# amathislab/BUCTD

Hardware: AMD Instinct MI355X
Metric: images/sec (train) BUCTD-CoAM-W48 384x288 (higher is better)
Workload: dtype f32 (3x3 convs: operands split exactly into 3 bf16 pieces, 6 bf16 MFMAs per product, fp32 accumulate - fp32-class); 1 GPU; BUCTD-CoAM-W48 (pose_hrnet_coam, ATT_MODULES [F,T,F,F], colored condition) 384x288 CrowdPose-14kpt full train step: fwd + JointsMSE + bwd + grad all-reduce + Adam + arg-max accuracy decode; global_batch=32, batch_per_gpu=32, input=N x 6 x 384 x 288 fp32, params=115581770, parallelism=dp1, hip_streams=4, conv_math=bf16x6, step_graph=False

## Files before the change

### buctd_amd/_C.py

```python
import ctypes as C
import os

import torch

_HERE = os.path.dirname(os.path.abspath(__file__))
LIB_PATH = os.path.join(_HERE, "lib", "libbuctd_hip.so")


class ConvDesc(C.Structure):
    _fields_ = [(n, C.c_int) for n in ("N", "H", "W", "Ci", "Co", "R", "S", "stride", "pad", "Ho", "Wo")]


class BasicBlockDesc(C.Structure):
    _fields_ = ([(n, C.c_int) for n in ("N", "H", "W", "C")] +
                [(n, C.c_void_p) for n in ("x", "w1_fwd", "w2_fwd", "w1_bwd", "w2_bwd", "gamma1", "beta1", "gamma2", "beta2",
                                           "running_mean1", "running_var1", "running_mean2", "running_var2")] +
                [(n, C.c_float) for n in ("eps1", "momentum1", "eps2", "momentum2")] +
                [(n, C.c_void_p) for n in ("z1", "z2", "y", "acc", "stat")])


class BasicBlockGrads(C.Structure):
    _fields_ = ([(n, C.c_void_p) for n in ("dy", "dz2", "dres", "dy1", "dz1", "dx", "dw1", "dw2", "dgamma1", "dbeta1",
                                           "dgamma2", "dbeta2")] +
                [(n, C.c_int) for n in ("acc_w1", "acc_w2", "acc_bn1", "acc_bn2")] +
                [("bn_acc", C.c_void_p), ("wg_ws", C.c_void_p), ("wg_ws_bytes", C.c_size_t)])


class BnAccIn(C.Structure):
    _fields_ = [("acc", C.c_void_p), ("rows", C.c_long), ("eps", C.c_float), ("momentum", C.c_float),
                ("mean_out", C.c_void_p), ("invstd_out", C.c_void_p), ("running_mean", C.c_void_p),
                ("running_var", C.c_void_p)]


class C3Conv(C.Structure):
    _fields_ = ([(n, C.c_int) for n in ("N", "H", "W", "Ci", "Co")] +
                [(n, C.c_void_p) for n in ("x", "wprep", "residual")] + [("relu", C.c_int)] +
                [(n, C.c_void_p) for n in ("y", "stats_acc")] + [("in_bn", C.POINTER(BnAccIn))] +
                [(n, C.c_void_p) for n in ("in_gamma", "in_beta")] + [("in_relu", C.c_int)] +
                [(n, C.c_void_p) for n in ("bn_z", "bn_y", "bn_mean", "bn_invstd", "bn_gamma", "bn_beta", "bn_acc")])


class C3ConvEval(C.Structure):
    _fields_ = ([(n, C.c_int) for n in ("N", "H", "W", "Ci", "Co")] +
                [(n, C.c_void_p) for n in ("x", "wprep", "scale", "shift", "residual")] + [("relu", C.c_int), ("y", C.c_void_p)])


class BnApplyItem(C.Structure):
    _fields_ = [("z", C.c_void_p), ("st", BnAccIn), ("gamma", C.c_void_p), ("beta", C.c_void_p), ("residual", C.c_void_p),
                ("relu", C.c_int), ("y", C.c_void_p), ("rows", C.c_long), ("C", C.c_int)]


class BnBwdItem(C.Structure):
    _fields_ = ([(n, C.c_void_p) for n in ("dy", "y", "z", "mean", "invstd", "gamma", "beta")] +
                [("relu", C.c_int), ("rows", C.c_long), ("C", C.c_int)] +
                [(n, C.c_void_p) for n in ("dz", "dres", "dgamma", "dbeta")] +
                [("accumulate", C.c_int), ("acc", C.c_void_p), ("acc_ready", C.c_int)])


class Wg3Conv(C.Structure):
    _fields_ = ([(n, C.c_int) for n in ("N", "H", "W", "Ci", "Co")] +
                [(n, C.c_void_p) for n in ("x", "dy", "dw")] + [("accumulate", C.c_int)] +
                [(n, C.c_void_p) for n in ("x_mean", "x_invstd", "x_gamma", "x_beta")] + [("x_relu", C.c_int)] +
                [("workspace", C.c_void_p), ("workspace_bytes", C.c_size_t)])


class MhaArgs(C.Structure):
    _fields_ = ([(n, C.c_int) for n in ("B", "T", "h", "dh")] +
                [(n, C.c_void_p) for n in ("q", "k", "v")] + [(n, C.c_int) for n in ("ldq", "ldk", "ldv")] +
                [("out", C.c_void_p), ("ldo", C.c_int), ("lse", C.c_void_p), ("scale", C.c_float), ("p_drop", C.c_float),
                 ("dout", C.c_void_p), ("lddo", C.c_int)] +
                [(n, C.c_void_p) for n in ("dq", "dk", "dv")] + [(n, C.c_int) for n in ("lddq", "lddk", "lddv")])


class MatmulDesc(C.Structure):
    _fields_ = [
        ("batch", C.c_int), ("M", C.c_int), ("N", C.c_int), ("K", C.c_int),
        ("a_layout", C.c_int), ("b_layout", C.c_int),
        ("lda", C.c_int), ("ldb", C.c_int), ("ldc", C.c_int),
        ("stride_a", C.c_long), ("stride_b", C.c_long), ("stride_c", C.c_long),
        ("Kc", C.c_int), ("group_stride_a", C.c_long), ("group_stride_bk", C.c_long),
        ("Nc", C.c_int), ("group_stride_bn", C.c_long), ("group_stride_c", C.c_long),
        ("alpha", C.c_float), ("bias_axis", C.c_int),
    ]


_P = C.c_void_p
_I = C.c_int
_L = C.c_long
_F = C.c_float
_U64 = C.c_uint64
_SZ = C.c_size_t
_PD = C.POINTER(ConvDesc)
_PM = C.POINTER(MatmulDesc)
_PI = C.POINTER(C.c_int)

SIGNATURES = {
    "buctd_version": (_I, []),
    "buctd_last_error": (C.c_char_p, []),
    "buctd_conv2d_fwd": (_I, [_PD, _P, _P, _P, _P, _P, _P, _I, _P, _P, _P]),
    "buctd_conv2d_fwd_thin": (_I, [_PD]),
    "buctd_conv2d_dgrad": (_I, [_PD, _P, _P, _P, _P, _P, _P]),
    "buctd_conv2d_stats_groups": (_I, [_PD, _I, _PI, _PI]),
    "buctd_conv2d_wgrad_workspace": (_SZ, [_PD]),
    "buctd_conv2d_wgrad": (_I, [_PD, _P, _P, _P, _I, _P, _SZ, _P]),
    "buctd_conv2d_plan": (_I, [_PD, _I, _I, _PI]),
    "buctd_matmul_workspace": (_SZ, [_PM]),
    "buctd_matmul": (_I, [_PM, _P, _P, _P, _P, _P, _SZ, _P]),
    "buctd_bn_finalize": (_I, [_P, _P, _I, _I, _L, _I, _F, _F, _P, _P, _P, _P, _P]),
    "buctd_conv3x3_bf16x3_supported": (_I, [_I, _I, _I, _I, _I]),
    "buctd_conv3x3_bf16x3_stats_groups": (_I, [_I, _I, _I, _I, _I, _PI, _PI]),
    "buctd_conv3x3_bf16x3_prep_bytes": (_SZ, [_I, _I, _I]),
    "buctd_conv3x3_bf16x3_prep": (_I, [_I, _I, _P, _I, _P, _P]),
    "buctd_conv3x3_bf16x3_prep_batched": (_I, [_P, _I, _L, _P]),
    "buctd_conv3x3_bf16x3": (_I, [_I, _I, _I, _I, _I, _P, _P, _P, _P, _P, _P, _I, _P, _P, _P, _P]),
    "buctd_conv3x3_wgrad_bf16x3_supported": (_I, [_I, _I, _I, _I, _I]),
    "buctd_conv3x3_wgrad_bf16x3_workspace": (_SZ, [_I, _I, _I, _I, _I]),
    "buctd_conv3x3_wgrad_bf16x3": (_I, [_I, _I, _I, _I, _I, _P, _P, _P, _I, _P, _SZ, _P]),
    "buctd_conv3x3_bf16x6_supported": (_I, [_I, _I, _I, _I, _I]),
    "buctd_conv3x3_bf16x6_stats_groups": (_I, [_I, _I, _I, _I, _I, _PI, _PI]),
    "buctd_conv3x3_bf16x6_prep_bytes": (_SZ, [_I, _I, _I]),
    "buctd_conv3x3_bf16x6_prep": (_I, [_I, _I, _P, _I, _P, _P]),
    "buctd_conv3x3_bf16x6": (_I, [_I, _I, _I, _I, _I, _P, _P, _P, _P, _P, _P, _I, _P, _P, _P, _P]),
    "buctd_conv3x3_bf16x6_bnin": (_I, [_I, _I, _I, _I, _I, _P, _P, _P, _P, _P, _P, _I, _P, _P, _P, _P, _P, _P, _P, _I, _P]),
    "buctd_conv3x3_bf16x6_bnstat": (_I, [_I, _I, _I, _I, _I, _P, _P, _P, _P, _P, _P, _P, _P, _P, _P, _P, _P]),
    "buctd_bn_bwd_from_partials": (_I, [_P, _P, _P, _P, _P, _P, _P, _I, _L, _I, _P, _I, _P, _P, _P, _P, _I, _P, _SZ, _P]),
    "buctd_conv3x3_wgrad_bf16x6_bnin": (_I, [_I, _I, _I, _I, _I, _P, _P, _P, _I, _P, _P, _P, _P, _I, _P, _SZ, _P]),
    "buctd_conv3x3_wgrad_bf16x6_supported": (_I, [_I, _I, _I, _I, _I]),
    "buctd_conv3x3_wgrad_bf16x6_workspace": (_SZ, [_I, _I, _I, _I, _I]),
    "buctd_conv3x3_wgrad_bf16x6": (_I, [_I, _I, _I, _I, _I, _P, _P, _P, _I, _P, _SZ, _P]),
    "buctd_bn_stats": (_I, [_P, _L, _I, _P, _PI, _PI, _P]),
    "buctd_bn_stats_groups": (_I, [_L, _I, _PI, _PI]),
    "buctd_bn_apply": (_I, [_P, _P, _P, _P, _P, _P, _I, _P, _L, _I, _P]),
    "buctd_bn_bwd_workspace": (_SZ, [_L, _I]),
    "buctd_bn_bwd": (_I, [_P, _P, _P, _P, _P, _P, _P, _I, _L, _I, _P, _P, _P, _P, _I, _P, _SZ, _P]),
    "buctd_bn_fold": (_I, [_P, _P, _P, _P, _F, _I, _P, _P, _P]),
    "buctd_bn_acc_bytes": (_SZ, [_I]),
    "buctd_bn_apply_acc": (_I, [_P, C.POINTER(BnAccIn), _P, _P, _P, _I, _P, _L, _I, _P]),
    "buctd_bn_bwd_acc": (_I, [_P, _P, _P, _P, _P, _P, _P, _I, _L, _I, _P, _P, _P, _P, _I, _P, _I, _P]),
    "buctd_conv3x3_bf16x6_acc": (_I, [_I] * 5 + [_P, _P, _P, _I, _P, _P, C.POINTER(BnAccIn), _P, _P, _I, _P]),
    "buctd_conv3x3_bf16x6_bnstat_acc": (_I, [_I] * 5 + [_P] * 12),
    "buctd_gconv_x6_fwd_acc": (_I, [_I] * 6 + [_P] * 6),
    "buctd_conv3x3_bf16x6_group": (_I, [_I, C.POINTER(C3Conv), _P]),
    "buctd_conv3x3_bf16x6_group_eval": (_I, [_I, C.POINTER(C3ConvEval), _P]),
    "buctd_conv3x3_bf16x6_group_workgroups": (_I, [_I, C.POINTER(C3Conv)]),
    "buctd_conv3x3_bf16x6_plan": (_I, [_I, _I, _I, _I, _I, _I, C.POINTER(C.c_int)]),
    "buctd_conv3x3_wgrad_bf16x6_plan": (_I, [_I, _I, _I, _I, _I, C.POINTER(C.c_int)]),
    "buctd_gconv_wgrad_x6_supported": (_I, [_I] * 6),
    "buctd_gconv_wgrad_x6_workspace": (_SZ, [_I] * 6),
    "buctd_gconv_wgrad_x6": (_I, [_I] * 6 + [_P, _P, _P, _I, _P, _SZ, _P]),
    "buctd_bn_apply_acc_group": (_I, [_I, C.POINTER(BnApplyItem), _P]),
    "buctd_bn_bwd_acc_group": (_I, [_I, C.POINTER(BnBwdItem), _P]),
    "buctd_conv3x3_wgrad_bf16x6_group_workspace": (_SZ, [_I] * 6),
    "buctd_conv3x3_wgrad_bf16x6_group": (_I, [_I, C.POINTER(Wg3Conv), _P]),
    "buctd_conv3x3_wgrad_bf16x6_group_workgroups": (_I, [_I, C.POINTER(Wg3Conv)]),
    "buctd_stream_fork": (_I, [_P, _P]),
    "buctd_basic_branches_fwd_train": (_I, [_I, _I, C.POINTER(BasicBlockDesc), _P]),
    "buctd_basic_branches_bwd": (_I, [_I, _I, C.POINTER(BasicBlockDesc), C.POINTER(BasicBlockGrads), _P, _P]),
    "buctd_basic_chain_fwd_train": (_I, [_I, C.POINTER(BasicBlockDesc), _P]),
    "buctd_basic_chain_bwd": (_I, [_I, C.POINTER(BasicBlockDesc), C.POINTER(BasicBlockGrads), _P, _P]),
    "buctd_x6_image_dims": (_I, [_I, _I, _I, _P, _P]),
    "buctd_x6_image_bytes": (C.c_size_t, [_I, _I, _I]),
    "buctd_x6_image": (_I, [_P, _I, _I, _I, _L, _L, _I, _L, _L, _I, _P, _P]),
    "buctd_x6_gemm": (_I, [_I, _I, _I, _P, _P, _P, _I, _F, _P, _L, _I, _L, _P]),
    "buctd_add": (_I, [_P, _P, _P, _L, _I, _P]),
    "buctd_add_n": (_I, [C.POINTER(_P), _I, _P, _L, _P]),
    "buctd_mul": (_I, [_P, _P, _P, _L, _P]),
    "buctd_scale": (_I, [_P, _P, _F, _P, _L, _P]),
    "buctd_copy_channels": (_I, [_P, _L, _I, _I, _P, _I, _I, _I, _P]),
    "buctd_add_bcast": (_I, [_P, _P, _P, _L, _L, _P]),
    "buctd_relu_bwd": (_I, [_P, _P, _P, _L, _P]),
    "buctd_colsum_workspace": (_SZ, [_L, _I]),
    "buctd_colsum": (_I, [_P, _L, _I, _P, _I, _P, _SZ, _P]),
    "buctd_nchw_to_nhwc": (_I, [_P, _I, _I, _I, _I, _I, _I, _P, _P]),
    "buctd_nhwc_to_nchw": (_I, [_P, _I, _I, _I, _I, _P, _P]),
    "buctd_fuse_sum": (_I, [C.POINTER(_P), _PI, _I, _I, _I, _I, _I, _I, _P, _P]),
    "buctd_fuse_sum_bwd": (_I, [_P, _P, _I, _I, _I, _I, _I, _P, _P]),
    "buctd_resize_bilinear": (_I, [_P, _I, _I, _I, _I, _I, _I, _I, _I, _P, _P]),
    "buctd_maxpool3x3s2_fwd": (_I, [_P, _I, _I, _I, _I, _P, _P, _P]),
    "buctd_maxpool3x3s2_bwd": (_I, [_P, _P, _I, _I, _I, _I, _P, _P]),
    "buctd_softmax_dropout_fwd": (_I, [_P, _L, _I, _F, _F, _U64, _P, _P, _P]),
    "buctd_softmax_dropout_bwd": (_I, [_P, _P, _L, _I, _F, _F, _U64, _P, _P]),
    "buctd_softmax_dropout_fwd_dseed": (_I, [_P, _L, _I, _F, _F, _P, _P, _P, _P]),
    "buctd_softmax_dropout_bwd_dseed": (_I, [_P, _P, _L, _I, _F, _F, _P, _P, _P]),
    "buctd_dropout": (_I, [_P, _P, _L, _F, _U64, _P]),
    "buctd_dropout_dseed": (_I, [_P, _P, _L, _F, _P, _P]),
    "buctd_dropout_seed_fill": (_I, [_P, _I, _U64, _U64, _P]),
    "buctd_attn_smallqk_supported": (_I, [_I, _I, _I]),
    "buctd_attn_smallqk_fwd": (_I, [_I, _I, _I, _I, _P, _P, _P, _F, _F, _U64, _I, _P, _P, _P, _P]),
    "buctd_attn_smallqk_bwd": (_I, [_I, _I, _I, _I, _P, _P, _P, _P, _P, _P, _P, _F, _F, _U64, _I, _P, _P, _P, _P, _P]),
    "buctd_attn_smallqk_fwd_dseed": (_I, [_I, _I, _I, _I, _P, _P, _P, _F, _F, _P, _I, _P, _P, _P, _P]),
    "buctd_attn_smallqk_bwd_dseed": (_I, [_I, _I, _I, _I, _P, _P, _P, _P, _P, _P, _P, _F, _F, _P, _I, _P, _P, _P, _P, _P]),
    "buctd_layernorm_fwd": (_I, [_P, _P, _P, _L, _I, _F, _P, _P, _P, _P]),
    "buctd_add_layernorm_fwd": (_I, [_P, _P, _P, _P, _L, _I, _F, _P, _P, _P, _P, _P]),
    "buctd_layernorm_bwd_workspace": (_SZ, [_L, _I]),
    "buctd_layernorm_bwd": (_I, [_P, _P, _P, _P, _P, _L, _I, _P, _P, _P, _I, _P, _SZ, _P]),
    "buctd_joints_mse": (_I, [_P, _P, _P, _I, _I, _I, _P, _P, _F, _P, _SZ, _P]),
    "buctd_joints_ohkm_mse_workspace": (_SZ, [_I, _I]),
    "buctd_joints_ohkm_mse": (_I, [_P, _P, _P, _I, _I, _I, _I, _P, _P, _F, _P, _SZ, _P]),
    "buctd_argmax_decode": (_I, [_P, _I, _I, _I, _P, _P, _P, _P]),
    "buctd_warp_affine_norm": (_I, [_P, _I, _I, _I, _P, _P, _P, _L, _P, _P]),
    "buctd_cond_render_into": (_I, [_P, _I, _P, _I, _I, _I, _I, _I, _I, _P, _L, _P, _SZ, _P]),
    "buctd_cond_geometry": (_I, [_P, _P, _P, _P, _I, _I, _P, _P, _P, _P]),
    "buctd_synthesize_pose": (_I, [_P, _P, _P, _P, _P, _P, _I, _I, _I, C.c_ulonglong, _P, _P]),
    "buctd_mha_fwd_supported": (_I, [_I, _I]),
    "buctd_mha_fwd": (_I, [_I, _I, _I, _P, _P, _P, _I, _I, _F, _P, _P, _P]),
    "buctd_mha_fwd_bf16x6": (_I, [_I, _I, _I, _P, _P, _P, _I, _I, _F, _P, _P, _P]),
    "buctd_gconv_x6_supported": (_I, [_I] * 7),
    "buctd_gconv_x6_prep_bytes": (_SZ, [_I, _I, _I, _I]),
    "buctd_gconv_x6_prep": (_I, [_I, _I, _I, _P, _I, _P, _P]),
    "buctd_gconv_x6_prep_item_bytes": (_SZ, []),
    "buctd_gconv_x6_prep_item": (_I, [_I, _I, _I, _P, _I, _P, _P]),
    "buctd_gconv_x6_prep_batched": (_I, [_P, _I, _P]),
    "buctd_gconv_x6_stats_groups": (_I, [_I] * 6 + [_PI, _PI]),
    "buctd_gconv_x6_fwd": (_I, [_I] * 6 + [_P] * 6 + [_I, _P, _P, _P, _P]),
    "buctd_gconv_x6_dgrad": (_I, [_I] * 6 + [_P] * 4 + [_P]),
    "buctd_mha_fwd_bf16x6_workspace": (_SZ, [_I, _I, _I]),
    "buctd_mha_fwd_bf16x6_ws": (_I, [_I, _I, _I, _P, _P, _P, _I, _I, _F, _P, _P, _P, _SZ, _P]),
    "buctd_mha_train_supported": (_I, [_I, _I]),
    "buctd_mha_fwd_train": (_I, [_I, _I, _I, _P, _P, _P, _I, _I, _F, _F, _U64, _P, _P, _P]),
    "buctd_mha_bwd_workspace": (_SZ, [_I, _I]),
    "buctd_mha_bwd": (_I, [_I, _I, _I, _P, _P, _P, _I, _I, _P, _P, _P, _F, _F, _U64, _P, _P, _I, _P, _I, _P, _SZ, _P]),
    "buctd_mha_fwd_train_dseed": (_I, [_I, _I, _I, _P, _P, _P, _I, _I, _F, _F, _P, _P, _P, _P]),
    "buctd_mha_bwd_dseed": (_I, [_I, _I, _I, _P, _P, _P, _I, _I, _P, _P, _P, _F, _F, _P, _P, _P, _I, _P, _I, _P, _SZ, _P]),
    "buctd_mha_heads_fwd_supported": (_I, [_I, _I, _I]),
    "buctd_mha_heads_fwd": (_I, [C.POINTER(MhaArgs), _P]),
    "buctd_mha_heads_fwd_bf16x6": (_I, [C.POINTER(MhaArgs), _P]),
    "buctd_mha_heads_train_supported": (_I, [_I, _I, _I]),
    "buctd_mha_heads_fwd_train": (_I, [C.POINTER(MhaArgs), _U64, _P]),
    "buctd_mha_heads_bwd_workspace": (_SZ, [_I, _I, _I]),
    "buctd_mha_heads_bwd": (_I, [C.POINTER(MhaArgs), _U64, _P, _SZ, _P]),
    "buctd_mha_heads_fwd_train_dseed": (_I, [C.POINTER(MhaArgs), _P, _P]),
    "buctd_mha_heads_bwd_dseed": (_I, [C.POINTER(MhaArgs), _P, _P, _SZ, _P]),
    "buctd_nms_workspace": (_SZ, [_I]),
    "buctd_nms": (_I, [_P, _P, _P, _I, _I, _F, _P, _SZ, _P]),
    "buctd_cpu_nms": (_I, [_P, _I, _P, _F, _P, _P]),
    "buctd_argmax_decode_refined": (_I, [_P, _I, _I, _I, _P, _P, _P, _P, _P]),
    "buctd_argmax_decode_dark": (_I, [_P, _I, _I, _I, _P, _P, _P, _P, _P]),
    "buctd_gaussian_target": (_I, [_P, _P, _I, _I, _I, _I, _F, _F, _F, _P, _P, _P]),
    "buctd_cond_render_workspace": (_SZ, [_I, _I, _I, _I]),
    "buctd_cond_render": (_I, [_P, _I, _P, _I, _I, _I, _I, _I, _I, _P, _P, _SZ, _P]),
    "buctd_flipback_avg": (_I, [_P, _P, _P, _I, _I, _I, _I, _I, _P, _P]),
    "buctd_sgd_step": (_I, [_P, _P, _P, _L, _F, _F, _F, _I, _I, _F, _P]),
    "buctd_adam_step": (_I, [_P, _P, _P, _P, _L, _F, _F, _F, _F, _I, _F, _P]),
    "buctd_bf16_pack_conv": (_I, [_P, _L, _L, _L, _L, _I, _I, _I, _P, _P, _P, _P, _P, _F, _P, _P, _P]),
    "buctd_bf16_conv": (_I, [_P, _I, _I, _I, _I, _P, _P, _I, _I, _I, _I, _P, _I, _I, _P, _P, _SZ, _P]),
    "buctd_bf16_fuse_sum": (_I, [C.POINTER(_P), _PI, _I, _I, _I, _I, _I, _I, _P, _P]),
    "buctd_bf16_from_f32": (_I, [_P, _L, _P, _P]),
}

_lib = None


class BuctdHipError(RuntimeError):
    pass


def lib():
    global _lib
    if _lib is None:
        if not os.path.isfile(LIB_PATH):
            raise BuctdHipError(
                f"{LIB_PATH} is missing - build it with `make` (or __graft_entry__.build()); "
                "buctd_amd has no CPU / eager fallback")
        handle = C.CDLL(LIB_PATH, mode=C.RTLD_GLOBAL)
        for name, (res, args) in SIGNATURES.items():
            fn = getattr(handle, name)
            fn.restype = res
            fn.argtypes = args
        _lib = handle
    return _lib


def check(rc, what=""):
    if rc != 0:
        msg = lib().buctd_last_error()
        raise BuctdHipError(f"{what} failed ({rc}): {msg.decode() if msg else ''}")


_raw_stream = getattr(torch._C, "_cuda_getCurrentRawStream", None)
_raw_device = getattr(torch._C, "_cuda_getDevice", None)


def current_stream_handle():
    if _raw_stream is not None and _raw_device is not None:
        return _raw_stream(_raw_device())
    return torch.cuda.current_stream().cuda_stream


def stream_ptr():
    return current_stream_handle()


def ptr(t):
    if t is None:
        return None
    if not t.is_cuda:
        raise BuctdHipError("buctd_amd ops need tensors on the ROCm device (no CPU path)")
    return t.data_ptr()
```

### buctd_amd/csrc/block.hip

```cpp
#include "common.h"
#include "../../include/buctd_hip.h"
#include <string.h>

#define BLK_TRY(call)      \
  do {                     \
    const int rc_ = (call); \
    if (rc_) return rc_;   \
  } while (0)

static bool fwd_ptrs_ok(const buctd_basic_block& b) {
  return b.x && b.w1_fwd && b.w2_fwd && b.z1 && b.z2 && b.y && b.acc && b.stat;
}

static bool bwd_ptrs_ok(const buctd_basic_block& b, const buctd_basic_block_grads& g) {
  return b.x && b.w1_bwd && b.w2_bwd && b.z1 && b.z2 && b.y && b.stat && g.dy && g.dres && g.dy1 && g.dw1 && g.dw2 && g.bn_acc &&
         g.wg_ws && g.dz2 && g.dz1;
}

static void acc_in_of(const buctd_basic_block& b, int second, buctd_bn_acc_in* st) {
  const long rows = (long)b.N * b.H * b.W;
  const int C = b.C;
  st->acc = second ? (char*)b.acc + buctd_bn_acc_bytes(C) : b.acc;
  st->rows = rows;
  st->eps = second ? b.eps2 : b.eps1;
  st->momentum = second ? b.momentum2 : b.momentum1;
  st->mean_out = b.stat + (second ? 2 * C : 0);
  st->invstd_out = b.stat + (second ? 3 * C : C);
  st->running_mean = second ? b.running_mean2 : b.running_mean1;
  st->running_var = second ? b.running_var2 : b.running_var1;
}

static buctd_c3_conv c3_of(const buctd_basic_block& b) {
  buctd_c3_conv c;
  memset(&c, 0, sizeof(c));
  c.N = b.N; c.H = b.H; c.W = b.W; c.Ci = c.Co = b.C;
  return c;
}

static int stream_fork(hipStream_t from, hipStream_t to, const char* who) {
  if (from == to) return BUCTD_OK;
  static thread_local hipEvent_t evs[16] = {nullptr};
  int devid = 0;
  if (hipGetDevice(&devid) != hipSuccess || devid < 0 || devid >= 16) {
    buctd_set_error("%s: cannot identify the current device", who);
    return BUCTD_ELAUNCH;
  }
  hipEvent_t& ev = evs[devid];
  if (!ev && hipEventCreateWithFlags(&ev, hipEventDisableTiming) != hipSuccess) {
    buctd_set_error("%s: hipEventCreate failed", who);
    return BUCTD_ELAUNCH;
  }
  if (hipEventRecord(ev, from) != hipSuccess || hipStreamWaitEvent(to, ev, 0) != hipSuccess) {
    buctd_set_error("%s: stream fork failed", who);
    return BUCTD_ELAUNCH;
  }
  return BUCTD_OK;
}

static int block_fwd_train(const buctd_basic_block& b, void* stream) {
  const int N = b.N, H = b.H, W = b.W, C = b.C;
  void* acc1 = b.acc;
  void* acc2 = (char*)b.acc + buctd_bn_acc_bytes(C);
  buctd_bn_acc_in st1, st2;
  acc_in_of(b, 0, &st1);
  acc_in_of(b, 1, &st2);
  BLK_TRY(buctd_conv3x3_bf16x6_acc(N, H, W, C, C, b.x, b.w1_fwd, nullptr, 0, b.z1, acc1, nullptr, nullptr, nullptr, 0, stream));
  BLK_TRY(buctd_conv3x3_bf16x6_acc(N, H, W, C, C, b.z1, b.w2_fwd, nullptr, 0, b.z2, acc2, &st1, b.gamma1, b.beta1, 1, stream));
  BLK_TRY(buctd_bn_apply_acc(b.z2, &st2, b.gamma2, b.beta2, b.x, 1, b.y, st2.rows, C, stream));
  return BUCTD_OK;
}

static int block_bwd_impl(const buctd_basic_block* b, const buctd_basic_block_grads* g, const buctd_basic_block* prev,
                          const buctd_basic_block_grads* gprev, bool bn2_ready, void* stream, void* side_stream) {
  const int N = b->N, H = b->H, W = b->W, C = b->C;
  const long rows = (long)N * H * W;
  const float *mean1 = b->stat, *invstd1 = b->stat + C, *mean2 = b->stat + 2 * C, *invstd2 = b->stat + 3 * C;
  hipStream_t main_s = (hipStream_t)stream, side_s = side_stream ? (hipStream_t)side_stream : main_s;
  void* acc_bn1 = g->bn_acc;
  void* acc_bn2 = (char*)g->bn_acc + buctd_bn_acc_bytes(C);
  BLK_TRY(buctd_bn_bwd_acc(g->dy, b->y, b->z2, mean2, invstd2, b->gamma2, nullptr, 1, rows, C, g->dz2, g->dres, g->dgamma2,
                           g->dbeta2, g->acc_bn2, acc_bn2, bn2_ready ? 1 : 0, stream));
  BLK_TRY(stream_fork(main_s, side_s, "buctd_basic_chain_bwd"));
  BLK_TRY(buctd_conv3x3_wgrad_bf16x6_bnin(N, H, W, C, C, b->z1, g->dz2, g->dw2, g->acc_w2, mean1, invstd1, b->gamma1,
                                          b->beta1, 1, g->wg_ws, g->wg_ws_bytes, side_s));
  BLK_TRY(buctd_conv3x3_bf16x6_bnstat_acc(N, H, W, C, C, g->dz2, b->w2_bwd, nullptr, g->dy1, b->z1, nullptr, mean1, invstd1,
                                          b->gamma1, b->beta1, acc_bn1, stream));
  BLK_TRY(buctd_bn_bwd_acc(g->dy1, nullptr, b->z1, mean1, invstd1, b->gamma1, b->beta1, 1, rows, C, g->dz1, nullptr, g->dgamma1,
                           g->dbeta1, g->acc_bn1, acc_bn1, 1, stream));
  BLK_TRY(stream_fork(main_s, side_s, "buctd_basic_chain_bwd"));
  BLK_TRY(buctd_conv3x3_wgrad_bf16x6(N, H, W, C, C, b->x, g->dz1, g->dw1, g->acc_w1, g->wg_ws, g->wg_ws_bytes, side_s));
  if (g->dx) {
    if (prev)
      BLK_TRY(buctd_conv3x3_bf16x6_bnstat_acc(N, H, W, C, C, g->dz1, b->w1_bwd, g->dres, g->dx, prev->z2, prev->y, prev->stat + 2 * C,
                                              prev->stat + 3 * C, prev->gamma2, nullptr,
                                              (char*)gprev->bn_acc + buctd_bn_acc_bytes(C), stream));
    else
      BLK_TRY(buctd_conv3x3_bf16x6(N, H, W, C, C, g->dz1, b->w1_bwd, nullptr, nullptr, nullptr, g->dres, 0, g->dx, nullptr,
                                   nullptr, stream));
  }
  return BUCTD_OK;
}

static bool bn2_sums_chain(const buctd_basic_block* b, const buctd_basic_block_grads* g) {
  return g->dx && g->dx == g[-1].dy && g[-1].bn_acc && b[-1].y == b->x && b[-1].N == b->N && b[-1].H == b->H && b[-1].W == b->W &&
         b[-1].C == b->C;
}

extern "C" int buctd_basic_chain_fwd_train(int n, const buctd_basic_block* blocks, void* stream) {
  BUCTD_CHECK_ARG(n > 0 && blocks, "buctd_basic_chain_fwd_train: bad argument");
  for (int k = 0; k < n; ++k) BUCTD_CHECK_ARG(fwd_ptrs_ok(blocks[k]), "buctd_basic_chain_fwd_train: null pointer in block %d", k);
  for (int k = 0; k < n; ++k) BLK_TRY(block_fwd_train(blocks[k], stream));
  return BUCTD_OK;
}
extern "C" int buctd_basic_chain_bwd(int n, const buctd_basic_block* blocks, const buctd_basic_block_grads* grads, void* stream,
                                     void* side_stream) {
  BUCTD_CHECK_ARG(n > 0 && blocks && grads, "buctd_basic_chain_bwd: bad argument");
  for (int k = 0; k < n; ++k)
    BUCTD_CHECK_ARG(bwd_ptrs_ok(blocks[k], grads[k]), "buctd_basic_chain_bwd: null pointer in block %d", k);
  bool ready = false;
  for (int k = n - 1; k >= 0; --k) {
    const bool chain = k > 0 && bn2_sums_chain(blocks + k, grads + k);
    BLK_TRY(block_bwd_impl(blocks + k, grads + k, chain ? blocks + k - 1 : nullptr, chain ? grads + k - 1 : nullptr, ready, stream,
                           side_stream));
    ready = chain;
  }
  return BUCTD_OK;
}

#define BR_MAX 4

extern "C" int buctd_basic_branches_fwd_train(int nb, int n, const buctd_basic_block* blocks, void* stream) {
  BUCTD_CHECK_ARG(nb > 0 && nb <= BR_MAX && n > 0 && blocks, "buctd_basic_branches_fwd_train: 1..%d branches", BR_MAX);
  for (int i = 0; i < nb * n; ++i)
    BUCTD_CHECK_ARG(fwd_ptrs_ok(blocks[i]), "buctd_basic_branches_fwd_train: null pointer in block %d", i);
  for (int k = 0; k < n; ++k) {
    buctd_c3_conv cv[BR_MAX];
    buctd_bn_acc_in st1[BR_MAX];
    buctd_bn_apply_item ap[BR_MAX];
    for (int b = 0; b < nb; ++b) {
      const buctd_basic_block& B = blocks[b * n + k];
      buctd_c3_conv& c = cv[b] = c3_of(B);
      c.x = B.x; c.wprep = B.w1_fwd; c.y = B.z1; c.stats_acc = B.acc;
    }
    BLK_TRY(buctd_conv3x3_bf16x6_group(nb, cv, stream));
    for (int b = 0; b < nb; ++b) {
      const buctd_basic_block& B = blocks[b * n + k];
      buctd_c3_conv& c = cv[b];
      acc_in_of(B, 0, &st1[b]);
      c.x = B.z1; c.wprep = B.w2_fwd; c.y = B.z2; c.stats_acc = (char*)B.acc + buctd_bn_acc_bytes(B.C);
      c.in_bn = &st1[b]; c.in_gamma = B.gamma1; c.in_beta = B.beta1; c.in_relu = 1;
    }
    BLK_TRY(buctd_conv3x3_bf16x6_group(nb, cv, stream));
    for (int b = 0; b < nb; ++b) {
      const buctd_basic_block& B = blocks[b * n + k];
      buctd_bn_apply_item& a = ap[b];
      a.z = B.z2;
      acc_in_of(B, 1, &a.st);
      a.gamma = B.gamma2; a.beta = B.beta2; a.residual = B.x; a.relu = 1; a.y = B.y;
      a.rows = a.st.rows; a.C = B.C;
    }
    BLK_TRY(buctd_bn_apply_acc_group(nb, ap, stream));
  }
  return BUCTD_OK;
}

extern "C" int buctd_basic_branches_bwd(int nb, int n, const buctd_basic_block* blocks, const buctd_basic_block_grads* grads,
                                        void* stream, void* side_stream) {
  BUCTD_CHECK_ARG(nb > 0 && nb <= BR_MAX && n > 0 && blocks && grads, "buctd_basic_branches_bwd: 1..%d branches", BR_MAX);
  for (int i = 0; i < nb * n; ++i)
    BUCTD_CHECK_ARG(bwd_ptrs_ok(blocks[i], grads[i]), "buctd_basic_branches_bwd: null pointer in block %d", i);
  hipStream_t main_s = (hipStream_t)stream, side_s = side_stream ? (hipStream_t)side_stream : main_s;
  bool ready[BR_MAX] = {false, false, false, false};
  for (int k = n - 1; k >= 0; --k) {
    buctd_bn_bwd_item bi[BR_MAX];
    buctd_wg3_conv wg[BR_MAX];
    buctd_c3_conv cv[BR_MAX];
    bool chain[BR_MAX];
    for (int b = 0; b < nb; ++b) {
      const buctd_basic_block& B = blocks[b * n + k];
      const buctd_basic_block_grads& G = grads[b * n + k];
      const int C = B.C;
      chain[b] = k > 0 && bn2_sums_chain(&B, &G);
      bi[b] = buctd_bn_bwd_item{G.dy, B.y, B.z2, B.stat + 2 * C, B.stat + 3 * C, B.gamma2, nullptr, 1, (long)B.N * B.H * B.W, C,
                                G.dz2, G.dres, G.dgamma2, G.dbeta2, G.acc_bn2, (char*)G.bn_acc + buctd_bn_acc_bytes(C),
                                ready[b] ? 1 : 0};
    }
    BLK_TRY(buctd_bn_bwd_acc_group(nb, bi, stream));
    BLK_TRY(stream_fork(main_s, side_s, "buctd_basic_branches_bwd"));
    for (int b = 0; b < nb; ++b) {
      const buctd_basic_block& B = blocks[b * n + k];
      const buctd_basic_block_grads& G = grads[b * n + k];
      const int C = B.C;
      wg[b] = buctd_wg3_conv{B.N, B.H, B.W, C, C, B.z1, G.dz2, G.dw2, G.acc_w2, B.stat, B.stat + C, B.gamma1, B.beta1, 1,
                             G.wg_ws, G.wg_ws_bytes};
    }
    BLK_TRY(buctd_conv3x3_wgrad_bf16x6_group(nb, wg, side_s));
    for (int b = 0; b < nb; ++b) {
      const buctd_basic_block& B = blocks[b * n + k];
      const buctd_basic_block_grads& G = grads[b * n + k];
      buctd_c3_conv& c = cv[b] = c3_of(B);
      c.x = G.dz2; c.wprep = B.w2_bwd; c.y = G.dy1;
      c.bn_z = B.z1; c.bn_mean = B.stat; c.bn_invstd = B.stat + B.C; c.bn_gamma = B.gamma1; c.bn_beta = B.beta1; c.bn_acc = G.bn_acc;
    }
    BLK_TRY(buctd_conv3x3_bf16x6_group(nb, cv, stream));
    for (int b = 0; b < nb; ++b) {
      const buctd_basic_block& B = blocks[b * n + k];
      const buctd_basic_block_grads& G = grads[b * n + k];
      const int C = B.C;
      bi[b] = buctd_bn_bwd_item{G.dy1, nullptr, B.z1, B.stat, B.stat + C, B.gamma1, B.beta1, 1, (long)B.N * B.H * B.W, C,
                                G.dz1, nullptr, G.dgamma1, G.dbeta1, G.acc_bn1, G.bn_acc, 1};
    }
    BLK_TRY(buctd_bn_bwd_acc_group(nb, bi, stream));
    BLK_TRY(stream_fork(main_s, side_s, "buctd_basic_branches_bwd"));
    for (int b = 0; b < nb; ++b) {
      const buctd_basic_block& B = blocks[b * n + k];
      const buctd_basic_block_grads& G = grads[b * n + k];
      const int C = B.C;
      wg[b] = buctd_wg3_conv{B.N, B.H, B.W, C, C, B.x, G.dz1, G.dw1, G.acc_w1, nullptr, nullptr, nullptr, nullptr, 0,
                             G.wg_ws, G.wg_ws_bytes};
    }
    BLK_TRY(buctd_conv3x3_wgrad_bf16x6_group(nb, wg, side_s));
    int m = 0;
    for (int b = 0; b < nb; ++b) {
      const buctd_basic_block& B = blocks[b * n + k];
      const buctd_basic_block_grads& G = grads[b * n + k];
      const int C = B.C;
      ready[b] = chain[b];
      if (!G.dx) continue;
      buctd_c3_conv& c = cv[m++] = c3_of(B);
      c.x = G.dz1; c.wprep = B.w1_bwd; c.residual = G.dres; c.y = G.dx;
      if (chain[b]) {
        const buctd_basic_block& Bp = blocks[b * n + k - 1];
        const buctd_basic_block_grads& Gp = grads[b * n + k - 1];
        c.bn_z = Bp.z2; c.bn_y = Bp.y; c.bn_mean = Bp.stat + 2 * C; c.bn_invstd = Bp.stat + 3 * C; c.bn_gamma = Bp.gamma2;
        c.bn_acc = (char*)Gp.bn_acc + buctd_bn_acc_bytes(C);
      }
    }
    if (m) BLK_TRY(buctd_conv3x3_bf16x6_group(m, cv, stream));
  }
  return BUCTD_OK;
}

extern "C" int buctd_stream_fork(void* from, void* to) {
  return stream_fork((hipStream_t)from, (hipStream_t)to, "buctd_stream_fork");
}
```

### buctd_amd/csrc/bn.hip

```cpp
#include "common.h"
#include "../../include/buctd_hip.h"
#include "bn_acc.h"

#define STAT_ROWS 64

__global__ __launch_bounds__(256) void bn_stats_kernel(const float* __restrict__ z, long rows, int C,
                                                       float* __restrict__ part) {
  const long r0 = (long)blockIdx.x * STAT_ROWS;
  long r1 = r0 + STAT_ROWS;
  if (r1 > rows) r1 = rows;
  const int cnt = (int)(r1 - r0);
  for (int c = threadIdx.x; c < C; c += 256) {
    float s = 0.f;
    for (long r = r0; r < r1; ++r) s += z[r * C + c];
    const float mean = cnt > 0 ? s / (float)cnt : 0.f;
    float m2 = 0.f;
    for (long r = r0; r < r1; ++r) {
      const float d = z[r * C + c] - mean;
      m2 += d * d;
    }
    part[((long)blockIdx.x * C + c) * 2 + 0] = mean;
    part[((long)blockIdx.x * C + c) * 2 + 1] = m2;
  }
}
// ... 475 lines not shown
    return BUCTD_EWORKSPACE;
  }
  hipStream_t st = (hipStream_t)stream;
  float* s = (float*)workspace;
  hipLaunchKernelGGL(bn_bwd_finalize_kernel, dim3(C), dim3(256), 0, st, part, nparts, C, s, dgamma, dbeta, accumulate);
  BUCTD_CHECK_LAUNCH("buctd_bn_bwd_from_partials(finalize)");
  const long total = rows * C;
  const float inv_rows = 1.0f / (float)rows;
  if (C % 4 == 0)
    hipLaunchKernelGGL(bn_bwd_apply_kernel<true>, dim3(stream_grid(total / 4)), dim3(256), 0, st, dy, y, z, mean,
                       invstd, gamma, beta, (const float*)s, relu, total, C, inv_rows, dz, dres);
  else
    hipLaunchKernelGGL(bn_bwd_apply_kernel<false>, dim3(stream_grid(total)), dim3(256), 0, st, dy, y, z, mean, invstd,
                       gamma, beta, (const float*)s, relu, total, C, inv_rows, dz, dres);
  BUCTD_CHECK_LAUNCH("buctd_bn_bwd_from_partials(apply)");
  return BUCTD_OK;
}

extern "C" int buctd_bn_fold(const float* gamma, const float* beta, const float* running_mean,
                             const float* running_var, float eps, int C, float* scale, float* shift, void* stream) {
  BUCTD_CHECK_ARG(gamma && beta && running_mean && running_var && scale && shift && C > 0,
                  "buctd_bn_fold: bad argument");
  hipLaunchKernelGGL(bn_fold_kernel, dim3(ceil_div(C, 256)), dim3(256), 0, (hipStream_t)stream, gamma, beta,
                     running_mean, running_var, eps, C, scale, shift);
  BUCTD_CHECK_LAUNCH("buctd_bn_fold");
  return BUCTD_OK;
}


#define BWD2_MAX_BLOCKS 1024

__global__ __launch_bounds__(256) void bn_bwd_reduce2_kernel(const float* __restrict__ dy, const float* __restrict__ y,
                                                             const float* __restrict__ z, const float* __restrict__ mean,
                                                             const float* __restrict__ invstd,
                                                             const float* __restrict__ gamma, const float* __restrict__ beta,
                                                             int relu, long rows, int C, long rows_per_block,
                                                             float* __restrict__ part) {
  __shared__ f32x4 sm[2][256];
  const int c4n = C >> 2;
  const int rl = 256 / c4n;
  const int tc = threadIdx.x % c4n, tr = threadIdx.x / c4n;
  const long r0 = (long)blockIdx.x * rows_per_block;
  long r1 = r0 + rows_per_block;
  if (r1 > rows) r1 = rows;
  f32x4 s1 = (f32x4){0.f, 0.f, 0.f, 0.f}, s2 = s1;
  if (tr < rl) {
    const f32x4 mu = reinterpret_cast<const f32x4*>(mean)[tc];
    const f32x4 is = reinterpret_cast<const f32x4*>(invstd)[tc];
    f32x4 sc = is, be = is;
    const bool rebuild = relu && !y;
    if (rebuild) {
      sc = is * reinterpret_cast<const f32x4*>(gamma)[tc];
      be = reinterpret_cast<const f32x4*>(beta)[tc];
    }
    auto body = [&](f32x4 g, f32x4 zz, f32x4 yy) {
      if (relu) {
        if (rebuild) yy = (zz - mu) * sc + be;
#pragma unroll
        for (int j = 0; j < 4; ++j)
          if (!(yy[j] > 0.f)) g[j] = 0.f;
      }
      s1 += g;
      s2 += g * (zz - mu) * is;
    };
    long r = r0 + tr;
    const long step = rl;
    for (; r + 3 * step < r1; r += 4 * step) {
      f32x4 g[4], zz[4], yy[4];
#pragma unroll
      for (int u = 0; u < 4; ++u) {
        const long o = (r + u * step) * c4n + tc;
        g[u] = reinterpret_cast<const f32x4*>(dy)[o];
        zz[u] = reinterpret_cast<const f32x4*>(z)[o];
        yy[u] = (relu && y) ? reinterpret_cast<const f32x4*>(y)[o] : zz[u];
      }
#pragma unroll
      for (int u = 0; u < 4; ++u) body(g[u], zz[u], yy[u]);
    }
    for (; r < r1; r += step) {
      const long o = r * c4n + tc;
      const f32x4 zz = reinterpret_cast<const f32x4*>(z)[o];
      body(reinterpret_cast<const f32x4*>(dy)[o], zz, (relu && y) ? reinterpret_cast<const f32x4*>(y)[o] : zz);
    }
  }
  sm[0][threadIdx.x] = s1;
  sm[1][threadIdx.x] = s2;
  __syncthreads();
  if (tr == 0) {
    for (int k = 1; k < rl; ++k) {
      s1 += sm[0][k * c4n + tc];
      s2 += sm[1][k * c4n + tc];
    }
    reinterpret_cast<f32x4*>(part + ((long)blockIdx.x * 2 + 0) * C)[tc] = s1;
    reinterpret_cast<f32x4*>(part + ((long)blockIdx.x * 2 + 1) * C)[tc] = s2;
  }
}

static long bwd2_blocks(long rows, long* rows_per_block) {
  long rpb = (rows + BWD2_MAX_BLOCKS - 1) / BWD2_MAX_BLOCKS;
  if (rpb < 64) rpb = 64;
  *rows_per_block = rpb;
  return (rows + rpb - 1) / rpb;
}


static int acc_grid(long n4, int per_cu = 8) {
  long b = (n4 + 256 * 4 - 1) / (256 * 4);
  if (b > 256 * per_cu) b = 256 * per_cu;
  if (b < 1) b = 1;
  return (int)b;
}

struct BnApplyArgs {
  const float* z;
  BnAccFwd a;
  const float* gamma;
  const float* beta;
  const float* res;
  int relu;
  float* y;
  long total;
  int C;
};
__device__ __forceinline__ void bn_apply_acc_body(const BnApplyArgs& p, unsigned bid, unsigned nblk, unsigned char* lds_raw) {
  const float* __restrict__ z = p.z;
  const float* __restrict__ res = p.res;
  float* __restrict__ y = p.y;
  const BnAccFwd& a = p.a;
  const int C = p.C, relu = p.relu;
  long long* wsum = reinterpret_cast<long long*>(lds_raw);
  float* tab = reinterpret_cast<float*>(lds_raw + (size_t)BNACC_WORDS * C * sizeof(long long));
  const long n4 = p.total >> 2;
  const long step = (long)nblk * 256;
  long i = (long)bid * 256 + threadIdx.x;
  f32x4 v0 = (f32x4){0.f, 0.f, 0.f, 0.f}, v1 = v0, r0 = v0, r1 = v0;
  auto fetch = [&](long j) {
    if (j < n4) {
      v0 = reinterpret_cast<const f32x4*>(z)[j];
      if (res) r0 = reinterpret_cast<const f32x4*>(res)[j];
    }
    if (j + step < n4) {
      v1 = reinterpret_cast<const f32x4*>(z)[j + step];
      if (res) r1 = reinterpret_cast<const f32x4*>(res)[j + step];
    }
  };
  fetch(i);
  bnacc_gather_lds(a.acc, C, wsum);
  for (int c = threadIdx.x; c < C; c += 256) {
    double s1, s2;
    bnacc_read_lds(wsum, C, c, &s1, &s2);
    const BnFwdStat st = bnacc_fwd_stat_sums(s1, s2, a.rows, a.eps);
    tab[c] = st.mean;
    tab[C + c] = st.invstd * p.gamma[c];
    tab[2 * C + c] = p.beta[c];
    if (bid == 0) {
      a.mean_out[c] = st.mean;
      a.invstd_out[c] = st.invstd;
      if (a.rmean) bnacc_running(st, a.rows, a.momentum, a.rmean, a.rvar, c);
    }
  }
  __syncthreads();
  const int dc = (int)((step * 4) % C);
  int c = (int)((i * 4) % C) - dc;
  auto one = [&](long j, int cc, f32x4 v, f32x4 r) {
    const f32x4 mu = *reinterpret_cast<const f32x4*>(tab + cc);
    const f32x4 sc = *reinterpret_cast<const f32x4*>(tab + C + cc);
    const f32x4 be = *reinterpret_cast<const f32x4*>(tab + 2 * C + cc);
    f32x4 o;
#pragma unroll
    for (int j4 = 0; j4 < 4; ++j4) o[j4] = (v[j4] - mu[j4]) * sc[j4] + be[j4];
    if (res) o += r;
    if (relu) {
#pragma unroll
      for (int j4 = 0; j4 < 4; ++j4) o[j4] = fmaxf(o[j4], 0.f);
    }
    reinterpret_cast<f32x4*>(y)[j] = o;
  };
  for (; i < n4; i += 2 * step) {
    c += dc;
    if (c >= C) c -= C;
    one(i, c, v0, r0);
    c += dc;
    if (c >= C) c -= C;
    if (i + step < n4) one(i + step, c, v1, r1);
    fetch(i + 2 * step);
  }
}
__global__ __launch_bounds__(256, 8) void bn_apply_acc_kernel(BnApplyArgs p) {
  extern __shared__ __attribute__((aligned(16))) unsigned char lds_raw[];
  bn_apply_acc_body(p, blockIdx.x, gridDim.x, lds_raw);
}

#define BNG_MAX 4
template <class A>
struct BnGroup {
  A s[BNG_MAX];
  int n;
  unsigned first[BNG_MAX + 1];
};
template <class A>
__device__ __forceinline__ int bn_group_find(const BnGroup<A>& g, unsigned* bid, unsigned* nblk) {
  int k = 0;
  while (k + 1 < g.n && blockIdx.x >= g.first[k + 1]) ++k;
  *bid = blockIdx.x - g.first[k];
  *nblk = g.first[k + 1] - g.first[k];
  return k;
}
__global__ __launch_bounds__(256, 8) void bn_apply_acc_group_kernel(BnGroup<BnApplyArgs> g_) {
  extern __shared__ __attribute__((aligned(16))) unsigned char lds_raw[];
  const BnGroup<BnApplyArgs>& g = *(const BnGroup<BnApplyArgs>*)__builtin_amdgcn_kernarg_segment_ptr();
  unsigned bid, nblk;
  const int k = bn_group_find(g, &bid, &nblk);
  bn_apply_acc_body(g.s[k], bid, nblk, lds_raw);
}

#define BN_APPLY_ACC_MAXC 3720
extern "C" size_t buctd_bn_acc_bytes(int C) { return C > 0 ? bnacc_bytes(C) : 0; }

static int acc_in_check(const buctd_bn_acc_in* st, const char* who) {
  BUCTD_CHECK_ARG(st && st->acc && st->rows > 0 && st->mean_out && st->invstd_out &&
                      (st->running_mean == nullptr) == (st->running_var == nullptr),
                  "%s: statistics accumulator, rows, mean_out and invstd_out are required; running_mean/var go together", who);
  return BUCTD_OK;
}
static BnAccFwd acc_in(const buctd_bn_acc_in* st) {
  BnAccFwd a;
  a.acc = (const long long*)st->acc; a.rows = (double)st->rows; a.eps = st->eps; a.momentum = st->momentum;
  a.mean_out = st->mean_out; a.invstd_out = st->invstd_out; a.rmean = st->running_mean; a.rvar = st->running_var;
  return a;
}

extern "C" int buctd_bn_apply_acc(const float* z, const buctd_bn_acc_in* st, const float* gamma, const float* beta,
                                  const float* residual, int relu, float* y, long rows, int C, void* stream) {
  BUCTD_CHECK_ARG(z && gamma && beta && y && rows > 0 && C > 0 && C % 4 == 0 && C <= BN_APPLY_ACC_MAXC,
                  "buctd_bn_apply_acc: bad argument (C must be a multiple of 4, <= %d)", BN_APPLY_ACC_MAXC);
  const int rc = acc_in_check(st, "buctd_bn_apply_acc");
  if (rc) return rc;
  BUCTD_CHECK_ARG(st->rows == rows, "buctd_bn_apply_acc: the statistics cover %ld rows, the tensor has %ld", st->rows, rows);
  const long total = rows * C;
  const BnApplyArgs a{z, acc_in(st), gamma, beta, residual, relu, y, total, C};
  if ((size_t)(BNACC_WORDS * 8 + 3 * 4) * C > 64 * 1024) {
    static unsigned char attr_done[BUCTD_MAX_DEVICES] = {0};
    if (const int rc2 = buctd_raise_lds_limit(reinterpret_cast<const void*>(bn_apply_acc_kernel), 160 * 1024, attr_done, "buctd_bn_apply_acc"))
      return rc2;
  }
  hipLaunchKernelGGL(bn_apply_acc_kernel, dim3(acc_grid(total / 4)), dim3(256), (size_t)(BNACC_WORDS * 8 + 3 * 4) * C,
                     (hipStream_t)stream, a);
  BUCTD_CHECK_LAUNCH("buctd_bn_apply_acc");
  return BUCTD_OK;
}

extern "C" int buctd_bn_apply_acc_group(int n, const buctd_bn_apply_item* items, void* stream) {
  BUCTD_CHECK_ARG(n > 0 && n <= BNG_MAX && items, "buctd_bn_apply_acc_group: 1..%d tensors", BNG_MAX);
  BnGroup<BnApplyArgs> g;
  g.n = n;
  g.first[0] = 0;
  size_t lds = 0;
  for (int k = 0; k < n; ++k) {
    const buctd_bn_apply_item& it = items[k];
    BUCTD_CHECK_ARG(it.z && it.gamma && it.beta && it.y && it.rows > 0 && it.C > 0 && it.C % 4 == 0 && it.C <= BN_APPLY_ACC_MAXC,
                    "buctd_bn_apply_acc_group: bad argument (C must be a multiple of 4, <= %d)", BN_APPLY_ACC_MAXC);
    const int rc = acc_in_check(&it.st, "buctd_bn_apply_acc_group");
    if (rc) return rc;
    BUCTD_CHECK_ARG(it.st.rows == it.rows, "buctd_bn_apply_acc_group: the statistics cover %ld rows, the tensor has %ld",
                    it.st.rows, it.rows);
    const long total = it.rows * it.C;
    g.s[k] = BnApplyArgs{it.z, acc_in(&it.st), it.gamma, it.beta, it.residual, it.relu, it.y, total, it.C};
    g.first[k + 1] = g.first[k] + (unsigned)acc_grid(total / 4);
    const size_t l = (size_t)(BNACC_WORDS * 8 + 3 * 4) * it.C;
    if (l > lds) lds = l;
  }
  for (int k = n; k < BNG_MAX; ++k) g.first[k + 1] = g.first[n];
  if (lds > 64 * 1024) {
    static unsigned char attr_done[BUCTD_MAX_DEVICES] = {0};
    if (const int rc2 = buctd_raise_lds_limit(reinterpret_cast<const void*>(bn_apply_acc_group_kernel), 160 * 1024, attr_done,
                                              "buctd_bn_apply_acc_group"))
      return rc2;
  }
  hipLaunchKernelGGL(bn_apply_acc_group_kernel, dim3(g.first[n]), dim3(256), lds, (hipStream_t)stream, g);
  BUCTD_CHECK_LAUNCH("buctd_bn_apply_acc_group");
  return BUCTD_OK;
}

struct BnBwdArgs {
  const float* dy;
  const float* y;
  const float* z;
  const float* mean;
  const float* invstd;
  const float* gamma;
  const float* beta;
  long long* acc;
  int relu;
  long rows;
  int C;
  long rows_per_block;
  float inv_rows;
  float* dz;
  float* dres;
  float* dgamma;
  float* dbeta;
  int accumulate;
};
__device__ __forceinline__ void bn_bwd_reduce_acc_body(const BnBwdArgs& p, unsigned bid, f32x4 (&sm)[2][256]) {
  const float* __restrict__ dy = p.dy;
  const float* __restrict__ y = p.y;
  const float* __restrict__ z = p.z;
  const float* __restrict__ mean = p.mean;
  const float* __restrict__ invstd = p.invstd;
  const float* __restrict__ gamma = p.gamma;
  const float* __restrict__ beta = p.beta;
  long long* __restrict__ acc = p.acc;
  const int relu = p.relu, C = p.C;
  const long rows = p.rows, rows_per_block = p.rows_per_block;
  const int c4n = C >> 2;
  const int rl = 256 / c4n;
  const int tc = threadIdx.x % c4n, tr = threadIdx.x / c4n;
  const long r0 = (long)bid * rows_per_block;
  long r1 = r0 + rows_per_block;
  if (r1 > rows) r1 = rows;
  f32x4 s1 = (f32x4){0.f, 0.f, 0.f, 0.f}, s2 = s1;
  if (tr < rl) {
    const f32x4 mu = reinterpret_cast<const f32x4*>(mean)[tc];
    const f32x4 is = reinterpret_cast<const f32x4*>(invstd)[tc];
    f32x4 sc = is, be = is;
    const bool rebuild = relu && !y;
    if (rebuild) {
      sc = is * reinterpret_cast<const f32x4*>(gamma)[tc];
      be = reinterpret_cast<const f32x4*>(beta)[tc];
    }
    auto body = [&](f32x4 g, f32x4 zz, f32x4 yy) {
      if (relu) {
        if (rebuild) yy = (zz - mu) * sc + be;
#pragma unroll
        for (int j = 0; j < 4; ++j)
          if (!(yy[j] > 0.f)) g[j] = 0.f;
      }
      s1 += g;
      s2 += g * (zz - mu) * is;
    };
    long r = r0 + tr;
    const long step = rl;
    for (; r + 3 * step < r1; r += 4 * step) {
      f32x4 g[4], zz[4], yy[4];
#pragma unroll
      for (int u = 0; u < 4; ++u) {
        const long o = (r + u * step) * c4n + tc;
        g[u] = reinterpret_cast<const f32x4*>(dy)[o];
        zz[u] = reinterpret_cast<const f32x4*>(z)[o];
        yy[u] = (relu && y) ? reinterpret_cast<const f32x4*>(y)[o] : zz[u];
      }
#pragma unroll
      for (int u = 0; u < 4; ++u) body(g[u], zz[u], yy[u]);
    }
    for (; r < r1; r += step) {
      const long o = r * c4n + tc;
      const f32x4 zz = reinterpret_cast<const f32x4*>(z)[o];
      body(reinterpret_cast<const f32x4*>(dy)[o], zz, (relu && y) ? reinterpret_cast<const f32x4*>(y)[o] : zz);
    }
  }
  sm[0][threadIdx.x] = s1;
  sm[1][threadIdx.x] = s2;
  __syncthreads();
  if (tr == 0) {
    for (int k = 1; k < rl; ++k) {
      s1 += sm[0][k * c4n + tc];
      s2 += sm[1][k * c4n + tc];
    }
    sm[0][tc] = s1;
    sm[1][tc] = s2;
  }
  __syncthreads();
  const unsigned shard = bnacc_shard();
  for (int c = threadIdx.x; c < C; c += 256)
    bnacc_add(acc, C, shard, c, (double)reinterpret_cast<const float*>(&sm[0][0])[c], (double)reinterpret_cast<const float*>(&sm[1][0])[c]);
}
__global__ __launch_bounds__(256) void bn_bwd_reduce_acc_kernel(BnBwdArgs p) {
  __shared__ f32x4 sm[2][256];
  bn_bwd_reduce_acc_body(p, blockIdx.x, sm);
}
__global__ __launch_bounds__(256) void bn_bwd_reduce_acc_group_kernel(BnGroup<BnBwdArgs> g_) {
  __shared__ f32x4 sm[2][256];
  const BnGroup<BnBwdArgs>& g = *(const BnGroup<BnBwdArgs>*)__builtin_amdgcn_kernarg_segment_ptr();
  unsigned bid, nblk;
  const int k = bn_group_find(g, &bid, &nblk);
  bn_bwd_reduce_acc_body(g.s[k], bid, sm);
}

__device__ __forceinline__ void bn_bwd_apply_acc_body(const BnBwdArgs& p, unsigned bid, unsigned nblk, unsigned char* lds_raw) {
  const float* __restrict__ dy = p.dy;
  const float* __restrict__ y = p.y;
  const float* __restrict__ z = p.z;
  const float* __restrict__ mean = p.mean;
  const float* __restrict__ invstd = p.invstd;
  const float* __restrict__ gamma = p.gamma;
  const float* __restrict__ beta = p.beta;
  const long long* __restrict__ acc = p.acc;
  float* __restrict__ dz = p.dz;
  float* __restrict__ dres = p.dres;
  float* __restrict__ dgamma = p.dgamma;
  float* __restrict__ dbeta = p.dbeta;
  const int relu = p.relu, C = p.C, accumulate = p.accumulate;
  const long total = p.rows * C;
  const float inv_rows = p.inv_rows;
  long long* wsum = reinterpret_cast<long long*>(lds_raw);
  float* tab = reinterpret_cast<float*>(lds_raw + (size_t)BNACC_WORDS * C * sizeof(long long));
  const long n4 = total >> 2;
  const long step = (long)nblk * 256;
  const bool ld_y = relu && y;
  long i = (long)bid * 256 + threadIdx.x;
  f32x4 g0 = (f32x4){0.f, 0.f, 0.f, 0.f}, g1 = g0, z0 = g0, z1 = g0, y0 = g0, y1 = g0;
  auto fetch = [&](long j) {
    if (j < n4) {
      g0 = reinterpret_cast<const f32x4*>(dy)[j];
      z0 = reinterpret_cast<const f32x4*>(z)[j];
      if (ld_y) y0 = reinterpret_cast<const f32x4*>(y)[j];
    }
    if (j + step < n4) {
      g1 = reinterpret_cast<const f32x4*>(dy)[j + step];
      z1 = reinterpret_cast<const f32x4*>(z)[j + step];
      if (ld_y) y1 = reinterpret_cast<const f32x4*>(y)[j + step];
    }
  };
  fetch(i);
  bnacc_gather_lds(acc, C, wsum);
  for (int c = threadIdx.x; c < C; c += 256) {
    double s1, s2;
    bnacc_read_lds(wsum, C, c, &s1, &s2);
    tab[c] = mean[c];
    tab[C + c] = invstd[c];
    tab[2 * C + c] = gamma[c];
    tab[3 * C + c] = (relu && !y) ? beta[c] : 0.f;
    tab[4 * C + c] = (float)s1;
    tab[5 * C + c] = (float)s2;
    if (bid == 0) {
      if (dbeta) dbeta[c] = accumulate ? dbeta[c] + (float)s1 : (float)s1;
      if (dgamma) dgamma[c] = accumulate ? dgamma[c] + (float)s2 : (float)s2;
    }
  }
  __syncthreads();
  const int dc = (int)((step * 4) % C);
  int c = (int)((i * 4) % C) - dc;
  auto one = [&](long j, int cc, f32x4 g, f32x4 zz, f32x4 yy) {
    const f32x4 mu = *reinterpret_cast<const f32x4*>(tab + cc);
    const f32x4 is = *reinterpret_cast<const f32x4*>(tab + C + cc);
    const f32x4 ga = *reinterpret_cast<const f32x4*>(tab + 2 * C + cc);
    if (relu) {
      if (!y) {
        const f32x4 be = *reinterpret_cast<const f32x4*>(tab + 3 * C + cc);
#pragma unroll
        for (int j4 = 0; j4 < 4; ++j4) {
          const float sc = is[j4] * ga[j4];
          yy[j4] = (zz[j4] - mu[j4]) * sc + be[j4];
        }
      }
#pragma unroll
      for (int j4 = 0; j4 < 4; ++j4)
        if (!(yy[j4] > 0.f)) g[j4] = 0.f;
    }
    const f32x4 s1 = *reinterpret_cast<const f32x4*>(tab + 4 * C + cc);
    const f32x4 s2 = *reinterpret_cast<const f32x4*>(tab + 5 * C + cc);
    f32x4 o;
#pragma unroll
    for (int j4 = 0; j4 < 4; ++j4) {
      const float zh = (zz[j4] - mu[j4]) * is[j4];
      o[j4] = ga[j4] * is[j4] * (g[j4] - s1[j4] * inv_rows - zh * s2[j4] * inv_rows);
    }
    reinterpret_cast<f32x4*>(dz)[j] = o;
    if (dres) reinterpret_cast<f32x4*>(dres)[j] = g;
  };
  for (; i < n4; i += 2 * step) {
    c += dc;
    if (c >= C) c -= C;
    one(i, c, g0, z0, y0);
    c += dc;
    if (c >= C) c -= C;
    if (i + step < n4) one(i + step, c, g1, z1, y1);
    fetch(i + 2 * step);
  }
}
__global__ __launch_bounds__(256, 6) void bn_bwd_apply_acc_kernel(BnBwdArgs p) {
  extern __shared__ __attribute__((aligned(16))) unsigned char lds_raw[];
  bn_bwd_apply_acc_body(p, blockIdx.x, gridDim.x, lds_raw);
}
__global__ __launch_bounds__(256, 6) void bn_bwd_apply_acc_group_kernel(BnGroup<BnBwdArgs> g_) {
  extern __shared__ __attribute__((aligned(16))) unsigned char lds_raw[];
  const BnGroup<BnBwdArgs>& g = *(const BnGroup<BnBwdArgs>*)__builtin_amdgcn_kernarg_segment_ptr();
  unsigned bid, nblk;
  const int k = bn_group_find(g, &bid, &nblk);
  bn_bwd_apply_acc_body(g.s[k], bid, nblk, lds_raw);
}

static int bn_bwd_acc_fill(const buctd_bn_bwd_item& it, const char* who, BnBwdArgs& a, long* nb) {
  BUCTD_CHECK_ARG(it.dy && it.z && it.mean && it.invstd && it.gamma && it.dz && it.acc && it.rows > 0 && it.C > 0 && it.C % 4 == 0 &&
                      it.C / 4 <= 256,
                  "%s: bad argument (C must be a multiple of 4, <= 1024)", who);
  BUCTD_CHECK_ARG(!it.relu || it.y || it.beta, "%s: relu backward needs the forward output, or beta to rebuild its sign", who);
  a.dy = it.dy; a.y = it.y; a.z = it.z; a.mean = it.mean; a.invstd = it.invstd; a.gamma = it.gamma; a.beta = it.beta;
  a.acc = (long long*)it.acc; a.relu = it.relu; a.rows = it.rows; a.C = it.C;
  *nb = bwd2_blocks(it.rows, &a.rows_per_block);
  a.inv_rows = 1.0f / (float)it.rows;
  a.dz = it.dz; a.dres = it.dres; a.dgamma = it.dgamma; a.dbeta = it.dbeta; a.accumulate = it.accumulate;
  return BUCTD_OK;
}

extern "C" int buctd_bn_bwd_acc(const float* dy, const float* y, const float* z, const float* mean, const float* invstd,
                                const float* gamma, const float* beta, int relu, long rows, int C, float* dz, float* dres,
                                float* dgamma, float* dbeta, int accumulate, void* acc, int acc_ready, void* stream) {
  const buctd_bn_bwd_item it{dy, y, z, mean, invstd, gamma, beta, relu, rows, C, dz, dres, dgamma, dbeta, accumulate, acc, acc_ready};
  BnBwdArgs a;
  long nb;
  const int rc = bn_bwd_acc_fill(it, "buctd_bn_bwd_acc", a, &nb);
  if (rc) return rc;
  hipStream_t st = (hipStream_t)stream;
  if (!acc_ready) {
    hipLaunchKernelGGL(bn_bwd_reduce_acc_kernel, dim3((unsigned)nb), dim3(256), 0, st, a);
    BUCTD_CHECK_LAUNCH("buctd_bn_bwd_acc(reduce)");
  }
  const long total = rows * C;
  hipLaunchKernelGGL(bn_bwd_apply_acc_kernel, dim3(acc_grid(total / 4, 6)), dim3(256), (size_t)(BNACC_WORDS * 8 + 6 * 4) * C, st, a);
  BUCTD_CHECK_LAUNCH("buctd_bn_bwd_acc(apply)");
  return BUCTD_OK;
}

extern "C" int buctd_bn_bwd_acc_group(int n, const buctd_bn_bwd_item* items, void* stream) {
  BUCTD_CHECK_ARG(n > 0 && n <= BNG_MAX && items, "buctd_bn_bwd_acc_group: 1..%d tensors", BNG_MAX);
  BnGroup<BnBwdArgs> ga, gr;
  ga.n = n; gr.n = 0;
  ga.first[0] = gr.first[0] = 0;
  size_t lds = 0;
  for (int k = 0; k < n; ++k) {
    long nb;
    const int rc = bn_bwd_acc_fill(items[k], "buctd_bn_bwd_acc_group", ga.s[k], &nb);
    if (rc) return rc;
    const long total = items[k].rows * items[k].C;
    ga.first[k + 1] = ga.first[k] + (unsigned)acc_grid(total / 4, 6);
    const size_t l = (size_t)(BNACC_WORDS * 8 + 6 * 4) * items[k].C;
    if (l > lds) lds = l;
    if (!items[k].acc_ready) {
      gr.s[gr.n] = ga.s[k];
      gr.first[gr.n + 1] = gr.first[gr.n] + (unsigned)nb;
      ++gr.n;
    }
  }
  for (int k = n; k < BNG_MAX; ++k) ga.first[k + 1] = ga.first[n];
  for (int k = gr.n; k < BNG_MAX; ++k) gr.first[k + 1] = gr.first[gr.n];
  hipStream_t st = (hipStream_t)stream;
  if (gr.n) {
    hipLaunchKernelGGL(bn_bwd_reduce_acc_group_kernel, dim3(gr.first[gr.n]), dim3(256), 0, st, gr);
    BUCTD_CHECK_LAUNCH("buctd_bn_bwd_acc_group(reduce)");
  }
  hipLaunchKernelGGL(bn_bwd_apply_acc_group_kernel, dim3(ga.first[n]), dim3(256), lds, st, ga);
  BUCTD_CHECK_LAUNCH("buctd_bn_bwd_acc_group(apply)");
  return BUCTD_OK;
}
```

### buctd_amd/models/hrnet_common.py

```python
import logging
import os

import torch

from .. import nn
from .. import ops

BN_MOMENTUM = 0.1
logger = logging.getLogger(__name__)


def conv3x3(in_planes, out_planes, stride=1):
    return nn.Conv2d(in_planes, out_planes, kernel_size=3, stride=stride, padding=1, bias=False)


class BasicBlock(nn.Module):
    expansion = 1

    def __init__(self, inplanes, planes, stride=1, downsample=None):
        super().__init__()
        self.conv1 = conv3x3(inplanes, planes, stride)
        self.bn1 = nn.BatchNorm2d(planes, momentum=BN_MOMENTUM)
        self.relu = nn.ReLU(inplace=True)
        self.conv2 = conv3x3(planes, planes)
        self.bn2 = nn.BatchNorm2d(planes, momentum=BN_MOMENTUM)
        self.downsample = downsample
        self.stride = stride

    def forward(self, x):
        if self.training and x.is_cuda and torch.is_grad_enabled() and _native_block(self):
            return ops.BasicBlockFn.apply(x, *_block_params(self))
        residual = x if self.downsample is None else self.downsample(x)
        out = nn.conv_bn_act(x, self.conv1, self.bn1, relu=True)
        return nn.conv_bn_act(out, self.conv2, self.bn2, relu=True, residual=residual)


def _native_block(m):
    return (type(m) is BasicBlock and m.downsample is None and m.stride == 1 and m.conv1.bias is None and m.conv2.bias is None
            and m.bn1.training and m.bn2.training and m.bn1.track_running_stats == m.bn2.track_running_stats)


def _block_params(m):
    nn._as_channels_last_(m.conv1.weight)
    nn._as_channels_last_(m.conv2.weight)
    return m.conv1.weight, m.bn1, m.conv2.weight, m.bn2


class Bottleneck(nn.Module):
    expansion = 4

    def __init__(self, inplanes, planes, stride=1, downsample=None):
        super().__init__()
        self.conv1 = nn.Conv2d(inplanes, planes, kernel_size=1, bias=False)
        self.bn1 = nn.BatchNorm2d(planes, momentum=BN_MOMENTUM)
        self.conv2 = nn.Conv2d(planes, planes, kernel_size=3, stride=stride, padding=1, bias=False)
        self.bn2 = nn.BatchNorm2d(planes, momentum=BN_MOMENTUM)
        self.conv3 = nn.Conv2d(planes, planes * self.expansion, kernel_size=1, bias=False)
        self.bn3 = nn.BatchNorm2d(planes * self.expansion, momentum=BN_MOMENTUM)
        self.relu = nn.ReLU(inplace=True)
        self.downsample = downsample
        self.stride = stride

    def forward(self, x):
        bns = (self.bn1, self.bn2, self.bn3) + (() if self.downsample is None or len(self.downsample) < 2 else (self.downsample[1],))
        if (self.training and x.is_cuda and torch.is_grad_enabled() and ops.fused_bottleneck_on()
                and all(b.training for b in bns)
                and (self.downsample is None or type(self.downsample) is nn.ConvBN and not self.downsample._relu)):
            for c in (self.conv1, self.conv2, self.conv3) + (() if self.downsample is None else (self.downsample[0],)):
                nn._as_channels_last_(c.weight)
            return ops.BottleneckFn.apply(x, self.conv1.weight, self)
        residual = x if self.downsample is None else self.downsample(x)
        out = nn.conv_bn_act(x, self.conv1, self.bn1, relu=True)
        out = nn.conv_bn_act(out, self.conv2, self.bn2, relu=True)
        return nn.conv_bn_act(out, self.conv3, self.bn3, relu=True, residual=residual)


class BlockChain(nn.Chain):

    def forward(self, x):
        if (len(self) > 1 and self.training and x.is_cuda and torch.is_grad_enabled() and ops.native_chain_ok(tuple(x.shape))
                and all(_native_block(m) and m.bn1.track_running_stats == self[0].bn1.track_running_stats for m in self)
                and ops.bn_in_fusable(tuple(x.shape), self[0].conv1.weight)):
            return ops.BasicChainFn.apply(x, self[0].conv1.weight, [_block_params(m) for m in self])
        return super().forward(x)


blocks_dict = {"BASIC": BasicBlock, "BOTTLENECK": Bottleneck}


def make_residual_layer(block, inplanes, planes, blocks, stride=1):
    downsample = None
    if stride != 1 or inplanes != planes * block.expansion:
        downsample = nn.ConvBN(
            nn.Conv2d(inplanes, planes * block.expansion, kernel_size=1, stride=stride, bias=False),
            nn.BatchNorm2d(planes * block.expansion, momentum=BN_MOMENTUM))
    layers = [block(inplanes, planes, stride, downsample)]
    inplanes = planes * block.expansion
    for _ in range(1, blocks):
        layers.append(block(inplanes, planes))
    return BlockChain(*layers), inplanes


class HighResolutionModule(nn.Module):
    def __init__(self, num_branches, blocks, num_blocks, num_inchannels, num_channels, fuse_method,
                 multi_scale_output=True):
        super().__init__()
        self._check_branches(num_branches, blocks, num_blocks, num_inchannels, num_channels)
        self.num_inchannels = num_inchannels
        self.fuse_method = fuse_method
        self.num_branches = num_branches
        self.multi_scale_output = multi_scale_output
        self.branches = self._make_branches(num_branches, blocks, num_blocks, num_channels)
        self.fuse_layers = self._make_fuse_layers()
        self.relu = nn.ReLU(True)

    def _check_branches(self, num_branches, blocks, num_blocks, num_inchannels, num_channels):
        for what, lst in (("NUM_BLOCKS", num_blocks), ("NUM_CHANNELS", num_channels),
                          ("NUM_INCHANNELS", num_inchannels)):
            if num_branches != len(lst):
                msg = "NUM_BRANCHES({}) <> {}({})".format(num_branches, what, len(lst))
                logger.error(msg)
                raise ValueError(msg)

    def _make_branches(self, num_branches, block, num_blocks, num_channels):
        branches = []
        for i in range(num_branches):
            chain, cout = make_residual_layer(block, self.num_inchannels[i], num_channels[i], num_blocks[i])
            self.num_inchannels[i] = cout
            branches.append(chain)
        return nn.ModuleList(branches)

    def _make_fuse_layers(self):
        if self.num_branches == 1:
            return None
        ch = self.num_inchannels
        rows = []
        for i in range(self.num_branches if self.multi_scale_output else 1):
            row = []
            for j in range(self.num_branches):
                if j > i:
                    row.append(nn.ConvBN(nn.Conv2d(ch[j], ch[i], 1, 1, 0, bias=False), nn.BatchNorm2d(ch[i]),
                                         nn.Upsample(scale_factor=2 ** (j - i), mode="nearest")))
                elif j == i:
                    row.append(None)
                else:
                    steps = []
                    for k in range(i - j):
                        last = k == i - j - 1
                        cout = ch[i] if last else ch[j]
                        steps.append(nn.ConvBN(nn.Conv2d(ch[j], cout, 3, 2, 1, bias=False), nn.BatchNorm2d(cout),
                                               None if last else nn.ReLU(True)))
                    row.append(nn.Chain(*steps))
            rows.append(nn.ModuleList(row))
        return nn.ModuleList(rows)

    def get_num_inchannels(self):
        return self.num_inchannels

    def _branches_grouped(self, x):
        nb = self.num_branches
        if not (self.training and torch.is_grad_enabled() and all(type(br) is BlockChain and len(br) > 1 for br in self.branches)):
            return None
        chains = []
        for br in self.branches:
            if not all(_native_block(m) and m.bn1.track_running_stats == br[0].bn1.track_running_stats for m in br):
                return None
            chains.append([_block_params(m) for m in br])
        xs = [x[i] for i in range(nb)]
        if not ops.group_branches_ok(xs, chains):
            return None
        parts = ops.group_branch_partition(nb)
        if len(parts) == 1:
            return list(ops.BasicBranchesFn.apply(chains[0][0][0], chains, *xs))
        outs = ops.fork_join([lambda p=p: ops.BasicBranchesFn.apply(chains[p[0]][0][0], [chains[i] for i in p], *[xs[i] for i in p])
                              for p in parts], [[xs[i] for i in p] for p in parts])
        ys = [None] * nb
        for p, o in zip(parts, outs):
            for i, y in zip(p, o):
                ys[i] = y
        return ys

    def _branches_grouped_eval(self, x):
        if self.training or torch.is_grad_enabled() or not all(type(br) is BlockChain and len(br) > 0 for br in self.branches):
            return None
        chains = []
        for br in self.branches:
            if not all(type(m) is BasicBlock and m.downsample is None and m.stride == 1 and m.conv1.bias is None
                       and m.conv2.bias is None and not m.bn1.training and not m.bn2.training
                       and m.bn1.running_mean is not None and m.bn2.running_mean is not None for m in br):
                return None
            chains.append([_block_params(m) for m in br])
        xs = [x[i] for i in range(self.num_branches)]
        if not ops.eval_branches_ok(xs, chains):
            return None
        return ops.basic_branches_eval(xs, chains)

    def forward(self, x):
        if self.num_branches == 1:
            return [self.branches[0](x[0])]
        xs = self._branches_grouped(x)
        if xs is None:
            xs = self._branches_grouped_eval(x)
        if xs is None:
            xs = ops.fork_join([lambda i=i: self.branches[i](x[i]) for i in range(self.num_branches)],
                               [x[i] for i in range(self.num_branches)])
        rows = list(enumerate(self.fuse_layers))
        fan = len(rows) > 1 and torch.is_grad_enabled() and any(t.requires_grad for t in xs)
        xr = [ops.FanOut.apply(xs[j], len(rows)) if fan and xs[j].is_cuda else [xs[j]] * len(rows)
              for j in range(self.num_branches)]

        def fuse_row(i, row):
            terms, shifts = [], []
            for j in range(self.num_branches):
                if j == i:
                    terms.append(xr[j][i])
                    shifts.append(0)
                elif j > i:
                    terms.append(row[j](xr[j][i]))
                    shifts.append(j - i)
                else:
                    terms.append(row[j](xr[j][i]))
                    shifts.append(0)
            return ops.FuseSum.apply(tuple(shifts), True, *terms)

        return ops.fork_join([lambda i=i, row=row: fuse_row(i, row) for i, row in rows], [xs for _ in rows], tag=1)


def make_transition_layer(pre, cur):
    layers = []
    for i in range(len(cur)):
        if i < len(pre):
            if cur[i] != pre[i]:
                layers.append(nn.ConvBN(nn.Conv2d(pre[i], cur[i], 3, 1, 1, bias=False), nn.BatchNorm2d(cur[i]),
                                        nn.ReLU(inplace=True)))
            else:
                layers.append(None)
        else:
            steps = []
            for j in range(i + 1 - len(pre)):
                cin = pre[-1]
                cout = cur[i] if j == i - len(pre) else cin
                steps.append(nn.ConvBN(nn.Conv2d(cin, cout, 3, 2, 1, bias=False), nn.BatchNorm2d(cout),
                                       nn.ReLU(inplace=True)))
            layers.append(nn.Chain(*steps))
    return nn.ModuleList(layers)


def make_stage(layer_config, num_inchannels, multi_scale_output=True):
    block = blocks_dict[layer_config["BLOCK"]]
    modules = []
    for i in range(layer_config["NUM_MODULES"]):
        mso = multi_scale_output or i != layer_config["NUM_MODULES"] - 1
        modules.append(HighResolutionModule(layer_config["NUM_BRANCHES"], block, layer_config["NUM_BLOCKS"],
                                            num_inchannels, layer_config["NUM_CHANNELS"],
                                            layer_config["FUSE_METHOD"], mso))
        num_inchannels = modules[-1].get_num_inchannels()
    return nn.Chain(*modules), num_inchannels


class HRNetTrunk(nn.Module):

    def build_trunk(self, extra, last_stage=4):
        self.conv1 = nn.Conv2d(3, 64, kernel_size=3, stride=2, padding=1, bias=False)
        self.bn1 = nn.BatchNorm2d(64, momentum=BN_MOMENTUM)
        self.conv2 = nn.Conv2d(64, 64, kernel_size=3, stride=2, padding=1, bias=False)
        self.bn2 = nn.BatchNorm2d(64, momentum=BN_MOMENTUM)
        self.relu = nn.ReLU(inplace=True)
        self.layer1, c = make_residual_layer(Bottleneck, 64, 64, 4)
        pre = [c]
        for s in range(2, last_stage + 1):
            scfg = extra["STAGE%d" % s]
            setattr(self, "stage%d_cfg" % s, scfg)
            block = blocks_dict[scfg["BLOCK"]]
            ch = [c * block.expansion for c in scfg["NUM_CHANNELS"]]
            setattr(self, "transition%d" % (s - 1), make_transition_layer(pre, ch))
            stage, pre = make_stage(scfg, ch, multi_scale_output=(s != last_stage))
            setattr(self, "stage%d" % s, stage)
        return pre

    def stem(self, x_nhwc):
        x = nn.conv_bn_act(x_nhwc, self.conv1, self.bn1, relu=True)
        x = nn.conv_bn_act(x, self.conv2, self.bn2, relu=True)
        return self.layer1(x)

    def enter_stage(self, s, prev, first=False):
        trans = getattr(self, "transition%d" % (s - 1))
        n = getattr(self, "stage%d_cfg" % s)["NUM_BRANCHES"]
        if first:
            heads = [trans[i] if isinstance(trans[i], nn.ConvBN) else trans[i][0] if isinstance(trans[i], nn.Chain) else None
                     for i in range(n)]
            if (self.training and prev.is_cuda and torch.is_grad_enabled() and ops.fused_bottleneck_on() and n > 1
                    and all(type(h) is nn.ConvBN and h[1].training for h in heads)):
                for h in heads:
                    nn._as_channels_last_(h[0].weight)
                ys = ops.ForkConvBnFn.apply(prev, heads[0][0].weight, [(h[0], h[1], h._relu) for h in heads])
                out = []
                for i in range(n):
                    y = ys[i]
                    if isinstance(trans[i], nn.Chain):
                        for m in list(trans[i])[1:]:
                            y = m(y)
                    out.append(y)
                return out
            return [trans[i](prev) if trans[i] is not None else prev for i in range(n)]
        return [trans[i](prev[-1]) if trans[i] is not None else prev[i] for i in range(n)]


def to_device_input(x):
    if not x.is_cuda:
        x = x.cuda()
    if x.dtype != torch.float32:
        x = x.float()
    return x.contiguous()


def init_weights_hrnet(model, pretrained="", linear=False):
    logger.info("=> init weights from normal distribution")
    for m in model.modules():
        if isinstance(m, (torch.nn.Conv2d, torch.nn.ConvTranspose2d)) or (linear and isinstance(m, torch.nn.Linear)):
            torch.nn.init.normal_(m.weight, std=0.001)
            if m.bias is not None:
                torch.nn.init.constant_(m.bias, 0)
        elif isinstance(m, torch.nn.BatchNorm2d):
            torch.nn.init.constant_(m.weight, 1)
            torch.nn.init.constant_(m.bias, 0)
    if os.path.isfile(pretrained):
        state = torch.load(pretrained, map_location="cpu")
        logger.info("=> loading pretrained model {}".format(pretrained))
        keep = {k: v for k, v in state.items()
                if k.split(".")[0] in model.pretrained_layers or model.pretrained_layers[0] == "*"}
        model.load_state_dict(keep, strict=False)
    elif pretrained:
        logger.error("=> please download pre-trained models first!")
        raise ValueError("{} is not exist!".format(pretrained))
```

### buctd_amd/ops.py

```python
import ctypes as C
import math

import torch

from . import _C
from ._C import ConvDesc, MatmulDesc, check, lib, ptr, stream_ptr

_capture = {"on": False, "events": set(), "allow_seeds": False, "seed_table": None, "seed_draws": 0}
_SEED_TABLE_SLOTS = 1024


def capturing():
    return _capture["on"]


def _new_event(stream=None):
    ev = torch.cuda.Event()
    ev.record(stream) if stream is not None else ev.record()
    if _capture["on"]:
        _capture["events"].add(id(ev))
        _capture.setdefault("keep", []).append(ev)
    return ev


# ... 721 lines not shown
                      "conv3x3_wgrad_bf16x6_bnin")
                return out
            check(fn(d.N, d.H, d.W, d.Ci, d.Co, ptr(x), ptr(dy), ptr(out), int(accumulate), ptr(ws), ws.numel(),
                     stream_ptr_()), "conv3x3_wgrad (split bf16)")
            return out
    if x_bn is not None:
        raise _C.BuctdHipError("conv_wgrad: x_bn needs the bf16x6 3x3 kernel (check bn_in_fusable first)")
    kind = _gconv_kind(d) if mode == "bf16x6" else 0
    if kind:
        need = _memo(("gwg", kind, d.N, d.H, d.W, d.Ci, d.Co),
                     lambda: (int(lib().buctd_gconv_wgrad_x6_workspace(kind, d.N, d.H, d.W, d.Ci, d.Co))
                              if lib().buctd_gconv_wgrad_x6_supported(kind, d.N, d.H, d.W, d.Ci, d.Co) == 1 else -1))
        if need >= 0:
            ws = workspace_(need, x.device)
            check(lib().buctd_gconv_wgrad_x6(kind, d.N, d.H, d.W, d.Ci, d.Co, ptr(x), ptr(dy), ptr(out), int(accumulate), ptr(ws),
                                             ws.numel(), stream_ptr_()), "gconv_wgrad_x6")
            return out
    need = lib().buctd_conv2d_wgrad_workspace(C.byref(d))
    ws = workspace_(need, x.device)
    check(lib().buctd_conv2d_wgrad(C.byref(d), ptr(x), ptr(dy), ptr(out), int(accumulate), ptr(ws), ws.numel(),
                                   stream_ptr_()), "conv2d_wgrad")
    return out


_side = {"on": True, "streams": {}, "joined": True}


_SIDE_PRIO = -1


def _side_stream(device):
    idx = device.index if device.index is not None else torch.cuda.current_device()
    st = _side["streams"].get(idx)
    if st is None:
        st = torch.cuda.Stream(device=device, priority=_SIDE_PRIO)
        _side["streams"][idx] = st
    return st


def copy_stream(device):
    if not (_side["on"] and device.type == "cuda"):
        return None
    return _side_stream(device)


def side_streams(device):
    return [st for idx, st in _side["streams"].items() if idx == device.index]


def wait_side_stream(stream=None):
    for idx, st in _side["streams"].items():
        target = stream if stream is not None else torch.cuda.current_stream(torch.device("cuda", idx))
        target.wait_stream(st)
    for (idx, _), st in _branch["streams"].items():
        target = stream if stream is not None else torch.cuda.current_stream(torch.device("cuda", idx))
        if target != st:
            target.wait_stream(st)


_branch = {"on": True, "streams": {}}


_BRANCH_MAX = 2
_BRANCH_PRIO = 0


def set_stream_forks(branch, wgrad=None):
    old = (_branch["on"], _side["on"])
    _branch["on"] = bool(branch)
    _side["on"] = bool(branch if wgrad is None else wgrad)
    return old


def set_branch_max(n):
    global _BRANCH_MAX
    old, _BRANCH_MAX = _BRANCH_MAX, max(0, int(n))
    return old


def compute_streams(device):
    idx = device.index if device.index is not None else torch.cuda.current_device()
    return ([st for (d, i), st in _branch["streams"].items() if d == idx and i <= _BRANCH_MAX] +
            [st for d, st in _side["streams"].items() if d == idx])


def reserve_compute_streams(device):
    out = []
    if _branch["on"]:
        out += [_branch_stream(device, i) for i in range(1, _BRANCH_MAX + 1)]
    if _side["on"]:
        out.append(_side_stream(device))
    return out


def _branch_stream(device, i):
    i = min(i, _BRANCH_MAX)
    key = (device.index, i)
    st = _branch["streams"].get(key)
    if st is None:
        st = torch.cuda.Stream(device=device, priority=_BRANCH_PRIO)
        _branch["streams"][key] = st
    return st


def lane_stream(device, k):
    return _branch_stream(device, k + 1)


def _record(t, stream):
    if torch.is_tensor(t):
        if t.is_cuda:
            t.record_stream(stream)
    elif isinstance(t, (list, tuple)):
        for u in t:
            _record(u, stream)


def fork_join(fns, inputs, tag=0):
    dev = None
    for t in inputs:
        for u in (t if isinstance(t, (list, tuple)) else [t]):
            if torch.is_tensor(u) and u.is_cuda:
                dev = u.device
    if not _branch["on"] or dev is None or len(fns) < 2:
        return [f() for f in fns]
    main = torch.cuda.current_stream(dev)
    start = torch.cuda.Event()
    start.record(main)
    outs = [None] * len(fns)
    done = []
    outs[0] = fns[0]()
    for i in range(1, len(fns)):
        st = _branch_stream(dev, i)
        if st == main:
            outs[i] = fns[i]()
            continue
        st.wait_event(start)
        _record(inputs[i], st)
        with torch.cuda.stream(st):
            outs[i] = fns[i]()
            ev = torch.cuda.Event()
            ev.record(st)
        _record(outs[i], main)
        done.append(ev)
    for ev in done:
        main.wait_event(ev)
    return outs


def _join_side():
    _side["joined"] = True
    wait_side_stream()


def _queue_join():
    task = torch._C._current_graph_task_id() if hasattr(torch._C, "_current_graph_task_id") else None
    if task is not None and task >= 0:
        if _side.get("task") == task:
            return
        _side["task"] = task
    elif not _side["joined"]:
        return
    _side["joined"] = False
    try:
        torch.autograd.Variable._execution_engine.queue_callback(_join_side)
    except RuntimeError:
        _join_side()


def conv_wgrad_async(x, dy, w_like, stride, pad, out, accumulate, x_bn=None):
    if not (_side["on"] and x.is_cuda):
        if x.is_cuda and _branch["on"]:
            _queue_join()
        return conv_wgrad(x, dy, w_like, stride, pad, out=out, accumulate=accumulate, x_bn=x_bn)
    side = _side_stream(x.device)
    check(lib().buctd_stream_fork(stream_ptr(), side.cuda_stream), "stream_fork")
    conv_wgrad(x, dy, w_like, stride, pad, out=out, accumulate=accumulate, x_bn=x_bn, stream=side)
    x.record_stream(side)
    dy.record_stream(side)
    if x_bn is not None:
        x_bn[0].record_stream(side)
        x_bn[1].record_stream(side)
    _queue_join()
    return out


def matmul(A, B, Cout, *, batch, M, N, K, a_layout, b_layout, lda, ldb, ldc, stride_a=0, stride_b=0, stride_c=0,
           Kc=None, gsa=0, gsbk=0, Nc=None, gsbn=0, gsc=0, alpha=1.0, bias=None, bias_axis=0,
           a_off=0, b_off=0, c_off=0):
    d = MatmulDesc(batch, M, N, K, a_layout, b_layout, lda, ldb, ldc, stride_a, stride_b, stride_c,
                   K if Kc is None else Kc, gsa, gsbk, N if Nc is None else Nc, gsbn, gsc, alpha, bias_axis)
    need = lib().buctd_matmul_workspace(C.byref(d))
    ws = workspace(need, A.device) if need else None
    pa = C.c_void_p(A.data_ptr() + 4 * a_off)
    pb = C.c_void_p(B.data_ptr() + 4 * b_off)
    pc = C.c_void_p(Cout.data_ptr() + 4 * c_off)
    check(lib().buctd_matmul(C.byref(d), pa, pb, ptr(bias), pc, ptr(ws), ws.numel() if ws is not None else 0,
                             stream_ptr()), "matmul")
    return Cout


def x6_image(src, V, K, role, *, vs, ks, vg=0, vgs=0, kg=0, kgs=0, off=0, out=None):
    need = lib().buctd_x6_image_bytes(V, K, role)
    if out is None or out.numel() < need:
        out = torch.empty(need, dtype=torch.uint8, device=src.device)
    check(lib().buctd_x6_image(C.c_void_p(src.data_ptr() + 4 * off), V, K, vg, vgs, vs, kg, kgs, ks, role, ptr(out),
                               stream_ptr()), "x6_image")
    return out


def x6_gemm(a_image, b_image, Cout, M, N, K, *, ldc, Nc=0, gsc=0, bias=None, bias_axis=0, alpha=1.0, c_off=0):
    check(lib().buctd_x6_gemm(M, N, K, ptr(a_image), ptr(b_image), ptr(bias), bias_axis, alpha,
                              C.c_void_p(Cout.data_ptr() + 4 * c_off), ldc, Nc, gsc, stream_ptr()), "x6_gemm")
    return Cout


def _x6_weight_image(w, V, K, transposed):
    key = (w.data_ptr(), w._version, _weights_epoch["n"])
    cache = getattr(w, "_buctd_x6img", None)
    if cache is None or cache["key"] != key:
        cache = {"key": key}
        try:
            w._buctd_x6img = cache
        except (AttributeError, RuntimeError, TypeError):
            pass
    tag = "t" if transposed else "n"
    if tag not in cache:
        ld = w.shape[1]
        cache[tag] = x6_image(w, V, K, 0, vs=1, ks=ld) if transposed else x6_image(w, V, K, 0, vs=ld, ks=1)
        cache[tag + "_ev"] = _new_event()
        cache[tag + "_stream"] = torch.cuda.current_stream(w.device).cuda_stream
    elif torch.cuda.current_stream(w.device).cuda_stream != cache[tag + "_stream"]:
        _wait_event(torch.cuda.current_stream(w.device), cache[tag + "_ev"])
    return cache[tag]


def fc_o_x6_ok(T, rows):
    return _conv_math["mode"] == "bf16x6" and T >= 512 and rows >= 192


def bn_finalize(part, info, rows, Cn, eps, momentum, running_mean, running_var):
    mean = torch.empty(Cn, dtype=torch.float32, device=part.device)
    invstd = torch.empty(Cn, dtype=torch.float32, device=part.device)
    counts = info[2] if len(info) > 2 else None
    check(lib().buctd_bn_finalize(ptr(part), ptr(counts), info[0], info[1], rows, Cn, eps, momentum, ptr(mean), ptr(invstd),
                                  ptr(running_mean), ptr(running_var), stream_ptr()), "bn_finalize")
    return mean, invstd


class BnAccInput:

    def __init__(self, acc, rows, bn, training=True, relu=True):
        Cn = acc.Cn
        dev = bn.weight.device
        self.acc, self.rows, self.gamma, self.beta, self.relu = acc, int(rows), bn.weight, bn.bias, relu
        self.eps = bn.eps
        self.momentum = 0.1 if bn.momentum is None else bn.momentum
        stat = torch.empty((2, Cn), dtype=torch.float32, device=dev)
        self.mean, self.invstd = stat[0], stat[1]
        track = bn.track_running_stats and training
        self.rm = bn.running_mean if track else None
        self.rv = bn.running_var if track else None

    def struct(self):
        st = _C.BnAccIn()
        st.acc, st.rows, st.eps, st.momentum = self.acc.ptr, self.rows, self.eps, self.momentum
        st.mean_out, st.invstd_out = self.mean.data_ptr(), self.invstd.data_ptr()
        st.running_mean = self.rm.data_ptr() if self.rm is not None else None
        st.running_var = self.rv.data_ptr() if self.rv is not None else None
        return st


def bn_apply_acc(z, bnin, residual=None, relu=False):
    Cn = z.shape[-1]
    y = torch.empty_like(z)
    st = bnin.struct()
    check(lib().buctd_bn_apply_acc(ptr(z), C.byref(st), ptr(bnin.gamma), ptr(bnin.beta), ptr(residual), int(bool(relu)), ptr(y),
                                   z.numel() // Cn, Cn, stream_ptr()), "bn_apply_acc")
    return y


def bn_acc_ok(Cn):
    return Cn % 4 == 0 and Cn <= 1024


def bn_stats(z):
    Cn = z.shape[-1]
    rows = z.numel() // Cn
    ng, rpg = C.c_int(), C.c_int()
    check(lib().buctd_bn_stats_groups(rows, Cn, C.byref(ng), C.byref(rpg)), "bn_stats_groups")
    part = torch.empty((ng.value, Cn, 2), dtype=torch.float32, device=z.device)
    check(lib().buctd_bn_stats(ptr(z), rows, Cn, ptr(part), None, None, stream_ptr()), "bn_stats")
    return part, (ng.value, rpg.value)


def bn_apply(z, mean, invstd, gamma, beta, residual=None, relu=False):
    Cn = z.shape[-1]
    y = torch.empty_like(z)
    check(lib().buctd_bn_apply(ptr(z), ptr(mean), ptr(invstd), ptr(gamma), ptr(beta), ptr(residual), int(bool(relu)),
                               ptr(y), z.numel() // Cn, Cn, stream_ptr()), "bn_apply")
    return y


def bn_bwd(dy, y, z, mean, invstd, gamma, relu, want_dres, dgamma, dbeta, accumulate, beta=None):
    Cn = z.shape[-1]
    rows = z.numel() // Cn
    dz = torch.empty_like(z)
    dres = torch.empty_like(z) if want_dres else None
    if relu and y is None and beta is None:
        raise _C.BuctdHipError("bn_bwd: ReLU backward needs the forward output or beta")
    if bn_acc_ok(Cn):
        acc = AccRef(Cn, z.device)
        check(lib().buctd_bn_bwd_acc(ptr(dy), ptr(y) if relu else None, ptr(z), ptr(mean), ptr(invstd), ptr(gamma),
                                     ptr(beta) if (relu and y is None) else None, int(bool(relu)), rows, Cn, ptr(dz), ptr(dres),
                                     ptr(dgamma), ptr(dbeta), int(accumulate), C.c_void_p(acc.ptr), 0,
                                     stream_ptr()), "bn_bwd_acc")
        return dz, dres
    need = lib().buctd_bn_bwd_workspace(rows, Cn)
    ws = workspace(need, z.device)
    check(lib().buctd_bn_bwd(ptr(dy), ptr(y) if relu else None, ptr(z), ptr(mean), ptr(invstd), ptr(gamma),
                             ptr(beta) if (relu and y is None) else None, int(bool(relu)), rows, Cn, ptr(dz), ptr(dres), ptr(dgamma), ptr(dbeta), int(accumulate),
                             ptr(ws), ws.numel(), stream_ptr()), "bn_bwd")
    return dz, dres


def bn_fold_cached(bn, gamma, beta, eps):
    rm, rv = bn.running_mean, bn.running_var
    nbt = bn.num_batches_tracked
    key = (gamma.data_ptr(), gamma._version, beta._version, rm.data_ptr(), rm._version, rv._version, _weights_epoch["n"],
           float(eps), getattr(bn, "_pending_batches", 0), nbt._version if nbt is not None else 0)
    cache = getattr(bn, "_buctd_fold", None)
    cur = torch.cuda.current_stream(gamma.device)
    if cache is None or cache[0] != key:
        scale, shift = bn_fold(gamma, beta, rm, rv, eps)
        ev = _new_event()
        cache = (key, scale, shift, ev, cur.cuda_stream, set())
        try:
            object.__setattr__(bn, "_buctd_fold", cache)
        except (AttributeError, TypeError):
            return scale, shift
    elif cur.cuda_stream != cache[4] and cur.cuda_stream not in cache[5]:
        _wait_event(cur, cache[3])
        cache[5].add(cur.cuda_stream)
    return cache[1], cache[2]


def bn_fold(gamma, beta, rm, rv, eps):
    Cn = gamma.numel()
    scale = torch.empty(Cn, dtype=torch.float32, device=gamma.device)
    shift = torch.empty(Cn, dtype=torch.float32, device=gamma.device)
    check(lib().buctd_bn_fold(ptr(gamma), ptr(beta), ptr(rm), ptr(rv), eps, Cn, ptr(scale), ptr(shift), stream_ptr()),
          "bn_fold")
    return scale, shift


def add(a, b=None, relu=False, out=None):
    if out is None:
        out = torch.empty_like(a)
    check(lib().buctd_add(ptr(a), ptr(b), ptr(out), a.numel(), int(bool(relu)), stream_ptr()), "add")
    return out


def mul(a, b, out=None):
    if out is None:
        out = torch.empty_like(a)
    check(lib().buctd_mul(ptr(a), ptr(b), ptr(out), a.numel(), stream_ptr()), "mul")
    return out


class Mul(torch.autograd.Function):

    @staticmethod
    def forward(ctx, a, b):
        a, b = _contig(a), _contig(b)
        ctx.save_for_backward(a, b)
        return mul(a, b)

    @staticmethod
    def backward(ctx, dy):
        a, b = ctx.saved_tensors
        dy = _contig(dy)
        return mul(dy, b), mul(dy, a)


def scale(x, dev_scalar=None, alpha=1.0, out=None):
    if out is None:
        out = torch.empty_like(x)
    check(lib().buctd_scale(ptr(x), ptr(dev_scalar), alpha, ptr(out), x.numel(), stream_ptr()), "scale")
    return out


def relu_bwd(dy, y):
    dx = torch.empty_like(dy)
    check(lib().buctd_relu_bwd(ptr(dy), ptr(y), ptr(dx), dy.numel(), stream_ptr()), "relu_bwd")
    return dx


def colsum(x2d_like, Cn, out, accumulate):
    rows = x2d_like.numel() // Cn
    need = lib().buctd_colsum_workspace(rows, Cn)
    ws = workspace(need, x2d_like.device)
    check(lib().buctd_colsum(ptr(x2d_like), rows, Cn, ptr(out), int(accumulate), ptr(ws), ws.numel(), stream_ptr()),
          "colsum")
    return out


def nchw_to_nhwc(x, c0=0, cc=None):
    _f32(x, "nchw input")
    N, Ct, H, W = x.shape
    cc = Ct - c0 if cc is None else cc
    y = torch.empty((N, H, W, cc), dtype=torch.float32, device=x.device)
    check(lib().buctd_nchw_to_nhwc(ptr(x), N, Ct, c0, cc, H, W, ptr(y), stream_ptr()), "nchw_to_nhwc")
    return y


def nhwc_to_nchw(x):
    _f32(x, "nhwc input")
    N, H, W, Cn = x.shape
    y = torch.empty((N, Cn, H, W), dtype=torch.float32, device=x.device)
    check(lib().buctd_nhwc_to_nchw(ptr(x), N, Cn, H, W, ptr(y), stream_ptr()), "nhwc_to_nchw")
    return y


def fuse_sum(terms, shifts, relu=True):
    base = terms[shifts.index(0)]
    N, H, W, Cn = base.shape
    out = torch.empty_like(base)
    n = len(terms)
    arr = (C.c_void_p * n)(*[t.data_ptr() for t in terms])
    sh = (C.c_int * n)(*shifts)
    check(lib().buctd_fuse_sum(arr, sh, n, N, H, W, Cn, int(bool(relu)), ptr(out), stream_ptr()), "fuse_sum")
    return out


def fuse_sum_bwd(dy, y, shift):
    N, H, W, Cn = dy.shape
    g = torch.empty((N, H >> shift, W >> shift, Cn), dtype=torch.float32, device=dy.device)
    check(lib().buctd_fuse_sum_bwd(ptr(dy), ptr(y), shift, N, H, W, Cn, ptr(g), stream_ptr()), "fuse_sum_bwd")
    return g


def resize_bilinear_from_nchw(x, c0, cc, Ho, Wo):
    _f32(x, "resize input")
    N, Ct, H, W = x.shape
    y = torch.empty((N, Ho, Wo, cc), dtype=torch.float32, device=x.device)
    check(lib().buctd_resize_bilinear(ptr(x), N, Ct, c0, cc, H, W, Ho, Wo, ptr(y), stream_ptr()), "resize_bilinear")
    return y


def softmax_dropout_fwd(s, L, scale, p_drop, seed, inplace=True):
    rows = s.numel() // L
    p = s if inplace else torch.empty_like(s)
    pd = torch.empty_like(s) if p_drop > 0 else p
    fn, seed = _seeded("buctd_softmax_dropout_fwd", seed)
    check(fn(ptr(s), rows, L, scale, p_drop, seed, ptr(p), ptr(pd), stream_ptr()), "softmax_dropout_fwd")
    return p, pd


def softmax_dropout_bwd(dpd, p, L, scale, p_drop, seed, inplace=True):
    rows = p.numel() // L
    ds = dpd if inplace else torch.empty_like(dpd)
    fn, seed = _seeded("buctd_softmax_dropout_bwd", seed)
    check(fn(ptr(dpd), ptr(p), rows, L, scale, p_drop, seed, ptr(ds), stream_ptr()), "softmax_dropout_bwd")
    return ds


def joints_mse(pred, gt, w, want_grad, gscale=1.0):
    N, K = pred.shape[0], pred.shape[1]
    HW = pred.numel() // (N * K)
    loss = torch.empty((), dtype=torch.float32, device=pred.device)
    grad = torch.empty_like(pred) if want_grad else None
    ws = workspace(N * K * 4, pred.device)
    check(lib().buctd_joints_mse(ptr(pred), ptr(gt), ptr(w), N, K, HW, ptr(loss), ptr(grad), gscale, ptr(ws),
                                 ws.numel(), stream_ptr()), "joints_mse")
    return loss, grad


def joints_ohkm_mse(pred, gt, w, topk, want_grad, gscale=1.0):
    N, K = pred.shape[0], pred.shape[1]
    HW = pred.numel() // (N * K)
    loss = torch.empty((), dtype=torch.float32, device=pred.device)
    grad = torch.empty_like(pred) if want_grad else None
    ws = workspace(lib().buctd_joints_ohkm_mse_workspace(N, K), pred.device)
    check(lib().buctd_joints_ohkm_mse(ptr(pred), ptr(gt), ptr(w), N, K, HW, int(topk), ptr(loss), ptr(grad), gscale,
                                      ptr(ws), ws.numel(), stream_ptr()), "joints_ohkm_mse")
    return loss, grad


def argmax_decode(hm, refine=False, preds_out=None):
    N, K, H, W = hm.shape
    preds = preds_out if preds_out is not None else torch.empty((N, K, 2), dtype=torch.float32, device=hm.device)
    if preds_out is not None and not (preds_out.is_pinned() and preds_out.is_contiguous() and tuple(preds_out.shape) == (N, K, 2)
                                      and preds_out.dtype == torch.float32):
        raise _C.BuctdHipError("argmax_decode: preds_out must be a pinned contiguous fp32 [N, K, 2] host tensor")
    maxvals = torch.empty((N, K, 1), dtype=torch.float32, device=hm.device)
    idx = torch.empty((N, K), dtype=torch.int32, device=hm.device)
    if refine:
        quarter = torch.empty((N, K, 2), dtype=torch.float32, device=hm.device)
        check(lib().buctd_argmax_decode_refined(ptr(hm), N * K, H, W, preds.data_ptr(), ptr(maxvals), ptr(idx), ptr(quarter),
                                                stream_ptr()), "argmax_decode_refined")
        return preds, maxvals, idx, quarter
    check(lib().buctd_argmax_decode(ptr(hm), N * K, H, W, preds.data_ptr(), ptr(maxvals), ptr(idx), stream_ptr()),
          "argmax_decode")
    return preds, maxvals, idx


DARK_MAX_PIXELS = 8000


def dark_decode(hm):
    if hm.dim() != 4 or hm.dtype != torch.float32:
        raise _C.BuctdHipError("dark_decode: heat-maps must be a fp32 [N, K, H, W] tensor")
    hm = hm.contiguous()
    N, K, H, W = hm.shape
    preds = torch.empty((N, K, 2), dtype=torch.float32, device=hm.device)
    maxvals = torch.empty((N, K, 1), dtype=torch.float32, device=hm.device)
    idx = torch.empty((N, K), dtype=torch.int32, device=hm.device)
    offset = torch.empty((N, K, 2), dtype=torch.float32, device=hm.device)
    check(lib().buctd_argmax_decode_dark(ptr(hm), N * K, H, W, ptr(preds), ptr(maxvals), ptr(idx), ptr(offset),
                                         stream_ptr()), "argmax_decode_dark")
    return preds, maxvals, idx, offset


def scalar_to_host(src, dst):
    if not (dst.is_pinned() and dst.dtype == torch.float32 and dst.numel() == 1 and src.numel() == 1):
        raise _C.BuctdHipError("scalar_to_host: one fp32 value into a pinned host tensor")
    check(lib().buctd_copy_channels(ptr(src), 1, 1, 0, dst.data_ptr(), 1, 0, 1, stream_ptr()), "scalar_to_host")
    return dst


def gaussian_target(joints, vis, heatmap_size, image_size, sigma):
    B, K = joints.shape[0], joints.shape[1]
    Wh, Hh = int(heatmap_size[0]), int(heatmap_size[1])
    target = torch.empty((B, K, Hh, Wh), dtype=torch.float32, device=joints.device)
    weight = torch.empty((B, K, 1), dtype=torch.float32, device=joints.device)
    check(lib().buctd_gaussian_target(ptr(joints), ptr(vis), B, K, Hh, Wh, image_size[0] / heatmap_size[0],
                                      image_size[1] / heatmap_size[1], float(sigma), ptr(target), ptr(weight),
                                      stream_ptr()), "gaussian_target")
    return target, weight


def cond_render(joints, colors, H, W, truncate=False):
    B, K, js = joints.shape
    Cc = 1 if colors is None else colors.shape[1]
    cond = torch.empty((B, Cc, H, W), dtype=torch.float32, device=joints.device)
    need = lib().buctd_cond_render_workspace(B, Cc, H, W)
    ws = workspace(need, joints.device)
    check(lib().buctd_cond_render(ptr(joints), js, ptr(colors), B, K, Cc, H, W, int(bool(truncate)), ptr(cond),
                                  ptr(ws), ws.numel(), stream_ptr()), "cond_render")
    return cond


def flipback_avg(a, b, perm, shift):
    N, K, H, W = a.shape
    out = torch.empty_like(a)
    check(lib().buctd_flipback_avg(ptr(a), ptr(b), ptr(perm), N, K, H, W, int(bool(shift)), ptr(out), stream_ptr()),
          "flipback_avg")
    return out


def adam_step(p, g, m, v, lr, beta1, beta2, eps, step, gscale=1.0):
    check(lib().buctd_adam_step(ptr(p), ptr(g), ptr(m), ptr(v), p.numel(), lr, beta1, beta2, eps, step, gscale,
                                stream_ptr()), "adam_step")


def sgd_step(p, g, buf, lr, momentum, weight_decay, nesterov, first, gscale=1.0):
    check(lib().buctd_sgd_step(ptr(p), ptr(g), ptr(buf), p.numel(), lr, momentum, weight_decay, int(bool(nesterov)),
                               int(bool(first)), gscale, stream_ptr()), "sgd_step")


def layernorm_fwd(x, gamma, beta, eps):
    Cn = x.shape[-1]
    rows = x.numel() // Cn
    y = torch.empty_like(x)
    mean = torch.empty(rows, dtype=torch.float32, device=x.device)
    invstd = torch.empty(rows, dtype=torch.float32, device=x.device)
    check(lib().buctd_layernorm_fwd(ptr(x), ptr(gamma), ptr(beta), rows, Cn, eps, ptr(y), ptr(mean), ptr(invstd),
                                    stream_ptr()), "layernorm_fwd")
    return y, mean, invstd


def add_layernorm_fwd(a, b, gamma, beta, eps, keep_sum=True):
    Cn = a.shape[-1]
    rows = a.numel() // Cn
    y = torch.empty_like(a)
    s = torch.empty_like(a) if keep_sum else None
    mean = torch.empty(rows, dtype=torch.float32, device=a.device)
    invstd = torch.empty(rows, dtype=torch.float32, device=a.device)
    check(lib().buctd_add_layernorm_fwd(ptr(a), ptr(b), ptr(gamma), ptr(beta), rows, Cn, eps, ptr(s), ptr(y), ptr(mean),
                                        ptr(invstd), stream_ptr()), "add_layernorm_fwd")
    return y, mean, invstd, s


def layernorm_bwd(dy, x, mean, invstd, gamma, dgamma, dbeta, accumulate):
    Cn = x.shape[-1]
    rows = x.numel() // Cn
    dx = torch.empty_like(x)
    need = lib().buctd_layernorm_bwd_workspace(rows, Cn)
    ws = workspace(need, x.device)
    check(lib().buctd_layernorm_bwd(ptr(dy), ptr(x), ptr(mean), ptr(invstd), ptr(gamma), rows, Cn, ptr(dx),
                                    ptr(dgamma), ptr(dbeta), int(accumulate), ptr(ws), ws.numel(), stream_ptr()),
          "layernorm_bwd")
    return dx


def dropout(x, p_drop, seed):
    y = torch.empty_like(x)
    fn, seed = _seeded("buctd_dropout", seed)
    check(fn(ptr(x), ptr(y), x.numel(), p_drop, seed, stream_ptr()), "dropout")
    return y


def maxpool3x3s2_fwd(x):
    N, H, W, Cn = x.shape
    Ho, Wo = (H + 2 - 3) // 2 + 1, (W + 2 - 3) // 2 + 1
    y = torch.empty((N, Ho, Wo, Cn), dtype=torch.float32, device=x.device)
    idx = torch.empty((N, Ho, Wo, Cn), dtype=torch.int32, device=x.device)
    check(lib().buctd_maxpool3x3s2_fwd(ptr(x), N, H, W, Cn, ptr(y), ptr(idx), stream_ptr()), "maxpool_fwd")
    return y, idx


def maxpool3x3s2_bwd(dy, idx, x_shape):
    N, H, W, Cn = x_shape
    dx = torch.empty(tuple(x_shape), dtype=torch.float32, device=dy.device)
    check(lib().buctd_maxpool3x3s2_bwd(ptr(dy), ptr(idx), N, H, W, Cn, ptr(dx), stream_ptr()), "maxpool_bwd")
    return dx


def _contig(g):
    return g if g.is_contiguous() else g.contiguous()


def _count_batch(bn):
    bn.count_batch() if hasattr(bn, "count_batch") else bn.num_batches_tracked.add_(1)


class ConvBnAct(torch.autograd.Function):

    @staticmethod
    def forward(ctx, x, conv_w, conv_b, bn, residual, relu, stride, pad, training, transposed_shape):
        gamma, beta = bn.weight, bn.bias
        eps = bn.eps
        ctx.meta = (bn, conv_w, conv_b, relu, stride, pad, training, transposed_shape, tuple(x.shape))
        if training or bn.running_mean is None:
            momentum = 0.1 if bn.momentum is None else bn.momentum
            if transposed_shape is None:
                z, part, info = conv_fwd(x, conv_w, conv_b, stride, pad, stats="acc")
            else:
                z, part, info = conv_dgrad(x, conv_w, transposed_shape, stride, pad, bias=conv_b, stats="acc")
            Cn = z.shape[-1]
            rows = z.numel() // Cn
            track = bn.track_running_stats and training
            if info[0] == "acc":
                bnin = BnAccInput(part, rows, bn, training)
                y = bn_apply_acc(z, bnin, residual, relu)
                mean, invstd = bnin.mean, bnin.invstd
            else:
                mean, invstd = bn_finalize(part, info, rows, Cn, eps, momentum,
                                           bn.running_mean if track else None, bn.running_var if track else None)
                y = bn_apply(z, mean, invstd, gamma, beta, residual, relu)
            if track:
                _count_batch(bn)
            ctx.has_res = residual is not None
            ctx.save_for_backward(x, z, mean, invstd, y if (relu and ctx.has_res) else None)
            return y
        scale, shift = bn_fold_cached(bn, gamma, beta, eps)
        if transposed_shape is None:
            y = conv_fwd(x, conv_w, conv_b, stride, pad, scale=scale, shift=shift, residual=residual, relu=relu)
        else:
            z = conv_dgrad(x, conv_w, transposed_shape, stride, pad, bias=conv_b)
            Cn = z.shape[-1]
            zero = torch.zeros(Cn, dtype=torch.float32, device=z.device)
            y = bn_apply(z, zero, scale, torch.ones_like(zero), shift, residual, relu)
        ctx.save_for_backward()
        ctx.eval_mode = True
        return y

    @staticmethod
    def backward(ctx, dy):
        if getattr(ctx, "eval_mode", False):
            raise _C.BuctdHipError("backward through eval-mode BatchNorm is not on the BUCTD path")
        bn, conv_w, conv_b, relu, stride, pad, training, transposed_shape, x_shape = ctx.meta
        x, z, mean, invstd, y = ctx.saved_tensors
        dy = _contig(dy)
        dgamma, acc_g = grad_target(bn.weight)
        dbeta, acc_b = grad_target(bn.bias)
        assert acc_g == acc_b
        dz, dres = bn_bwd(dy, y, z, mean, invstd, bn.weight, relu, ctx.has_res and relu, dgamma, dbeta, acc_g, beta=bn.bias)
        if ctx.has_res and not relu:
            dres = dy
        dx = None
        if transposed_shape is None:
            if ctx.needs_input_grad[0]:
                dx = conv_dgrad(dz, conv_w, x_shape, stride, pad, residual=getattr(ctx, "dx_residual", None))
            dw, acc_w = grad_target(conv_w)
            conv_wgrad_async(x, dz, conv_w, stride, pad, dw, acc_w)
        else:
            if ctx.needs_input_grad[0]:
                dx = conv_fwd(dz, conv_w, None, stride, pad)
            dw, acc_w = grad_target(conv_w)
            conv_wgrad_async(dz, x, conv_w, stride, pad, dw, acc_w)
        if conv_b is not None:
            db, acc = grad_target(conv_b)
            colsum(dz, dz.shape[-1], db, acc)
        grad_done(bn.weight, bn.bias, conv_w, conv_b)
        return dx, None, None, None, dres, None, None, None, None, None


class _SubCtx:

    def __init__(self, needs_x=True):
        self.needs_input_grad = (needs_x,)
        self.saved_tensors = ()

    def save_for_backward(self, *tensors):
        self.saved_tensors = tensors


def _pack_subs(ctx, subs):
    flat, layout = [], []
    for c in subs:
        if c is None:
            layout.append(None)
            continue
        layout.append(tuple(t is not None for t in c.saved_tensors))
        flat.extend(t for t in c.saved_tensors if t is not None)
        c.saved_tensors = ()
    ctx.save_for_backward(*flat)
    ctx.sub_layout = layout


def _unpack_subs(ctx, subs):
    it = iter(ctx.saved_tensors)
    for c, lay in zip(subs, ctx.sub_layout):
        if c is not None:
            c.saved_tensors = tuple(next(it) if has else None for has in lay)


class BottleneckFn(torch.autograd.Function):

    @staticmethod
    def forward(ctx, x, w1, m):
        need = ctx.needs_input_grad[0]
        c1, c2, c3 = _SubCtx(need), _SubCtx(), _SubCtx()
        cd = None
        residual = x
        if m.downsample is not None:
            cd = _SubCtx(need)
            ds_conv, ds_bn = m.downsample[0], m.downsample[1]
            s, p = ds_conv._geom()
            residual = ConvBnAct.forward(cd, x, ds_conv.weight, ds_conv.bias, ds_bn, None, False, s, p, True, None)
        out = ConvBnAct.forward(c1, x, m.conv1.weight, None, m.bn1, None, True, 1, 0, True, None)
        out = ConvBnAct.forward(c2, out, m.conv2.weight, None, m.bn2, None, True, m.stride, 1, True, None)
        y = ConvBnAct.forward(c3, out, m.conv3.weight, None, m.bn3, residual, True, 1, 0, True, None)
        ctx.sub = (c1, c2, c3, cd)
        _pack_subs(ctx, ctx.sub)
        return y

    @staticmethod
    def backward(ctx, dy):
        c1, c2, c3, cd = ctx.sub
        _unpack_subs(ctx, ctx.sub)
        r3 = ConvBnAct.backward(c3, dy)
        d_out2, dres = r3[0], r3[4]
        d_out1 = ConvBnAct.backward(c2, d_out2)[0]
        dx = None
        if ctx.needs_input_grad[0]:
            if cd is not None:
                dres = ConvBnAct.backward(cd, dres)[0]
            c1.dx_residual = dres
        elif cd is not None:
            ConvBnAct.backward(cd, dres)
        dx = ConvBnAct.backward(c1, d_out1)[0]
        for c in ctx.sub:
            if c is not None:
                c.saved_tensors = ()
        return dx, None, None


class ForkConvBnFn(torch.autograd.Function):

    @staticmethod
    def forward(ctx, x, w0, groups):
        need = ctx.needs_input_grad[0]
        subs, outs = [], []
        for conv, bn, relu in groups:
            c = _SubCtx(need)
            s, p = conv._geom()
            outs.append(ConvBnAct.forward(c, x, conv.weight, conv.bias, bn, None, relu, s, p, True, None))
            subs.append(c)
        ctx.sub = subs
        _pack_subs(ctx, subs)
        return tuple(outs)

    @staticmethod
    def backward(ctx, *dys):
        subs = ctx.sub
        _unpack_subs(ctx, subs)
        dx = None
        for c, dy in zip(subs, dys):
            if dy is None:
                continue
            c.dx_residual = dx
            r = ConvBnAct.backward(c, dy)[0]
            dx = r if r is not None else dx
        for c in subs:
            c.saved_tensors = ()
        return dx, None, None


class BasicBlockFn(torch.autograd.Function):

    @staticmethod
    def forward(ctx, x, w1, bn1, w2, bn2):
        fuse = bn_in_fusable(tuple(x.shape), w2)
        veto = native_block_veto["fn"]
        if (fuse and bn_in_fusable(tuple(x.shape), w1) and bn1.track_running_stats == bn2.track_running_stats
                and not (veto is not None and veto(tuple(x.shape)))):
            ctx.native = True
            return _chain_forward(ctx, x, [(w1, bn1, w2, bn2)])
        ctx.native = False
        z1, part, info = conv_fwd(x, w1, None, 1, 1, stats="acc")
        Cn = z1.shape[-1]
        rows = z1.numel() // Cn
        y1 = None
        if info[0] == "acc":
            bnin1 = BnAccInput(part, rows, bn1, True, relu=True)
            if fuse:
                z2, part2, info2 = conv_fwd(z1, w2, None, 1, 1, stats="acc", in_bn=bnin1)
            else:
                y1 = bn_apply_acc(z1, bnin1, None, True)
                z2, part2, info2 = conv_fwd(y1, w2, None, 1, 1, stats="acc")
            bnin2 = BnAccInput(part2, rows, bn2, True)
            y = bn_apply_acc(z2, bnin2, x, True)
            mean1, invstd1, mean2, invstd2 = bnin1.mean, bnin1.invstd, bnin2.mean, bnin2.invstd
        else:
            def fin(bn, part, info):
                track = bn.track_running_stats
                return bn_finalize(part, info, rows, Cn, bn.eps, 0.1 if bn.momentum is None else bn.momentum,
                                   bn.running_mean if track else None, bn.running_var if track else None)
            mean1, invstd1 = fin(bn1, part, info)
            if fuse:
                z2, part2, info2 = conv_fwd(z1, w2, None, 1, 1, stats=True, in_bn=(mean1, invstd1, bn1.weight, bn1.bias, True))
            else:
                y1 = bn_apply(z1, mean1, invstd1, bn1.weight, bn1.bias, None, True)
                z2, part2, info2 = conv_fwd(y1, w2, None, 1, 1, stats=True)
            mean2, invstd2 = fin(bn2, part2, info2)
            y = bn_apply(z2, mean2, invstd2, bn2.weight, bn2.bias, x, True)
        for bn in (bn1, bn2):
            if bn.track_running_stats:
                _count_batch(bn)
        ctx.meta = (w1, bn1, w2, bn2, fuse)
        ctx.save_for_backward(x, z1, mean1, invstd1, None if fuse else y1, z2, mean2, invstd2, y)
        return y

    @staticmethod
    def backward(ctx, dy):
        if ctx.native:
            return _chain_backward(ctx, dy, ctx.needs_input_grad[0]), None, None, None, None
        w1, bn1, w2, bn2, fuse = ctx.meta
        x, z1, mean1, invstd1, y1, z2, mean2, invstd2, y2 = ctx.saved_tensors
        dy = _contig(dy)
        dg, acc_g = grad_target(bn2.weight)
        db, acc_b = grad_target(bn2.bias)
        assert acc_g == acc_b
        dz2, dres = bn_bwd(dy, y2, z2, mean2, invstd2, bn2.weight, True, True, dg, db, acc_g)
        dy1 = conv_dgrad(dz2, w2, tuple(z1.shape), 1, 1)
        dw, acc_w = grad_target(w2)
        if fuse:
            conv_wgrad_async(z1, dz2, w2, 1, 1, dw, acc_w, x_bn=(mean1, invstd1, bn1.weight, bn1.bias, True))
        else:
            conv_wgrad_async(y1, dz2, w2, 1, 1, dw, acc_w)
        grad_done(bn2.weight, bn2.bias, w2)
        dg, acc_g = grad_target(bn1.weight)
        db, acc_b = grad_target(bn1.bias)
        assert acc_g == acc_b
        dz1, _ = bn_bwd(dy1, None, z1, mean1, invstd1, bn1.weight, True, False, dg, db, acc_g, beta=bn1.bias)
        dx = conv_dgrad(dz1, w1, tuple(x.shape), 1, 1, residual=dres) if ctx.needs_input_grad[0] else None
        dw, acc_w = grad_target(w1)
        conv_wgrad_async(x, dz1, w1, 1, 1, dw, acc_w)
        grad_done(bn1.weight, bn1.bias, w1)
        return dx, None, None, None, None


def _block_desc(d, shape, step, xin, params, act, stat, acc=None):
    w1, bn1, w2, bn2 = params
    d.N, d.H, d.W, d.C = shape
    d.x = xin
    d.gamma1, d.beta1 = bn1.weight.data_ptr(), bn1.bias.data_ptr()
    d.gamma2, d.beta2 = bn2.weight.data_ptr(), bn2.bias.data_ptr()
    d.z1, d.z2, d.y = act, act + step, act + 2 * step
    d.stat = stat
    if acc is None:
        d.w1_bwd = _conv3x3_prepared(w1, 1).data_ptr()
        d.w2_bwd = _conv3x3_prepared(w2, 1).data_ptr()
    else:
        d.w1_fwd = _conv3x3_prepared(w1, 0).data_ptr()
        d.w2_fwd = _conv3x3_prepared(w2, 0).data_ptr()
        if bn1.track_running_stats:
            d.running_mean1, d.running_var1 = bn1.running_mean.data_ptr(), bn1.running_var.data_ptr()
            d.running_mean2, d.running_var2 = bn2.running_mean.data_ptr(), bn2.running_var.data_ptr()
            _count_batch(bn1)
            _count_batch(bn2)
        d.eps1, d.momentum1 = bn1.eps, 0.1 if bn1.momentum is None else bn1.momentum
        d.eps2, d.momentum2 = bn2.eps, 0.1 if bn2.momentum is None else bn2.momentum
        d.acc = acc
    return act + 2 * step


def _block_grads(g, tmp, step, dy, want_dx, params, bn_acc, ws, ws_bytes):
    w1, bn1, w2, bn2 = params
    g.dy = dy
    g.dz2, g.dres, g.dy1, g.dz1 = tmp, tmp + step, tmp + 2 * step, tmp + 3 * step
    g.dx = tmp + 4 * step if want_dx else 0
    dg2, acc_g2 = grad_target(bn2.weight)
    db2, acc_b2 = grad_target(bn2.bias)
    dw2, acc_w2 = grad_target(w2)
    dg1, acc_g1 = grad_target(bn1.weight)
    db1, acc_b1 = grad_target(bn1.bias)
    dw1, acc_w1 = grad_target(w1)
    assert acc_g2 == acc_b2 and acc_g1 == acc_b1
    weight_rsc(dw1)
    weight_rsc(dw2)
    g.dw1, g.dw2 = dw1.data_ptr(), dw2.data_ptr()
    g.dgamma1, g.dbeta1, g.dgamma2, g.dbeta2 = dg1.data_ptr(), db1.data_ptr(), dg2.data_ptr(), db2.data_ptr()
    g.acc_w1, g.acc_w2, g.acc_bn1, g.acc_bn2 = int(acc_w1), int(acc_w2), int(acc_g1), int(acc_g2)
    g.bn_acc = bn_acc
    g.wg_ws, g.wg_ws_bytes = ws, ws_bytes


def _native_bwd_done(side, tensors, blocks):
    if side is not None:
        for t in tensors:
            t.record_stream(side)
        _queue_join()
    elif _branch["on"]:
        _queue_join()
    for (w1, bn1, w2, bn2) in blocks:
        grad_done(bn2.weight, bn2.bias, w2)
        grad_done(bn1.weight, bn1.bias, w1)


def _chain_forward(ctx, x, blocks):
    n = len(blocks)
    shape = N, H, W, Cn = x.shape
    dev = x.device
    act = torch.empty((n, 3, N, H, W, Cn), dtype=torch.float32, device=dev)
    stat = torch.empty((n, 4, Cn), dtype=torch.float32, device=dev)
    descs = (_C.BasicBlockDesc * n)()
    step = 4 * N * H * W * Cn
    accb = acc_bytes(Cn)
    abase, pbase, sbase = act.data_ptr(), AccRef(Cn, dev, 2 * n).ptr, stat.data_ptr()
    xin = x.data_ptr()
    for k, blk in enumerate(blocks):
        xin = _block_desc(descs[k], shape, step, xin, blk, abase + 3 * step * k, sbase + k * 4 * Cn * 4, pbase + k * 2 * accb)
    check(lib().buctd_basic_chain_fwd_train(n, descs, stream_ptr()), "basic_chain_fwd_train")
    ctx.blocks = blocks
    ctx.save_for_backward(x, act, stat)
    return act[n - 1, 2]


def _chain_backward(ctx, dy, want_dx):
    blocks = ctx.blocks
    n = len(blocks)
    x, act, stat = ctx.saved_tensors
    dy = _contig(dy)
    shape = N, H, W, Cn = x.shape
    dev = x.device
    tmp = torch.empty((n, 5 if (n > 1 or want_dx) else 4, N, H, W, Cn), dtype=torch.float32, device=dev)
    step = 4 * N * H * W * Cn
    abase, sbase, tb = act.data_ptr(), stat.data_ptr(), tmp.data_ptr()
    descs = (_C.BasicBlockDesc * n)()
    grads = (_C.BasicBlockGrads * n)()
    main = torch.cuda.current_stream(dev)
    use_side = _side["on"]
    side = _side_stream(dev) if use_side else main
    accb = acc_bytes(Cn)
    bn_acc = AccRef(Cn, dev, 2 * n).ptr
    wg_ws = workspace_on(side, _wgrad3x3_workspace("bf16x6", N, H, W, Cn, Cn), dev)
    ws, ws_bytes = wg_ws.data_ptr(), wg_ws.numel()
    xin = x.data_ptr()
    for k, blk in enumerate(blocks):
        xin = _block_desc(descs[k], shape, step, xin, blk, abase + 3 * step * k, sbase + k * 4 * Cn * 4)
        up = dy.data_ptr() if k == n - 1 else tb + 5 * step * (k + 1) + 4 * step
        _block_grads(grads[k], tb + 5 * step * k, step, up, k > 0 or want_dx, blk, bn_acc + k * 2 * accb, ws, ws_bytes)
    check(lib().buctd_basic_chain_bwd(n, descs, grads, main.cuda_stream, side.cuda_stream if use_side else None),
          "basic_chain_bwd")
    _native_bwd_done(side if use_side else None, (x, act, stat, tmp, dy), reversed(blocks))
    return tmp[0, 4] if want_dx else None


class BasicChainFn(torch.autograd.Function):

    @staticmethod
    def forward(ctx, x, w_first, blocks):
        return _chain_forward(ctx, x, blocks)

    @staticmethod
    def backward(ctx, dy):
        return _chain_backward(ctx, dy, ctx.needs_input_grad[0]), None, None


_GROUP_BRANCHES = {"on": True}


def set_group_branches(on):
    old = _GROUP_BRANCHES["on"]
    _GROUP_BRANCHES["on"] = bool(on)
    return old


_GROUP_PARTS = {"n": 2}


def set_group_parts(n):
    old = _GROUP_PARTS["n"]
    _GROUP_PARTS["n"] = int(n)
    return old


def group_branch_partition(nb):
    if _GROUP_PARTS["n"] <= 1 or nb < 3:
        return [list(range(nb))]
    if nb == 3:
        return [[0], [1, 2]] if _GROUP_PARTS["n"] == 2 else [[0, 2], [1]]
    return [[0, 1], [2, 3]] if _GROUP_PARTS["n"] == 2 else [[0, 3], [1, 2]]


def group_branches_ok(xs, chains):
    if not (_GROUP_BRANCHES["on"] and 1 <= len(xs) <= 4 and len({len(c) for c in chains}) == 1):
        return False
    cfs = set()
    for x, chain in zip(xs, chains):
        if not (x.is_cuda and x.dim() == 4 and native_chain_ok(tuple(x.shape)) and bn_in_fusable(tuple(x.shape), chain[0][0])):
            return False
        Cn = x.shape[-1]
        cfs.add(3 if Cn % 48 == 0 else 2 if Cn % 32 == 0 else 0)
    return len(cfs) == 1 and 0 not in cfs


def eval_branches_ok(xs, chains):
    if not (_GROUP_BRANCHES["on"] and _conv_math["mode"] == "bf16x6" and 2 <= len(xs) <= 4 and len({len(c) for c in chains}) == 1):
        return False
    for x, chain in zip(xs, chains):
        if not (x.is_cuda and x.dim() == 4 and x.dtype == torch.float32 and x.is_contiguous()):
            return False
        for (w1, _, w2, _) in chain:
            if not (_bf16x3_ok(conv_desc(x.shape, _wshape(w1), 1, 1)) and _bf16x3_ok(conv_desc(x.shape, _wshape(w2), 1, 1))):
                return False
            if _wshape(w1)[0] != x.shape[-1] or _wshape(w2)[0] != x.shape[-1]:
                return False

    def one_kernel():
        items = (_C.C3Conv * len(xs))()
        for it, x in zip(items, xs):
            it.N, it.H, it.W, it.Ci, it.Co = x.shape[0], x.shape[1], x.shape[2], x.shape[3], x.shape[3]
            it.x = it.wprep = it.y = xs[0].data_ptr()
        return lib().buctd_conv3x3_bf16x6_group_workgroups(len(xs), items) > 0
    return _memo(("evalgrp",) + tuple(tuple(x.shape) for x in xs), one_kernel)


def basic_branches_eval(xs, chains):
    nb, n = len(xs), len(chains[0])
    cur = list(xs)
    for k in range(n):
        folded = [(bn_fold_cached(ch[k][1], ch[k][1].weight, ch[k][1].bias, ch[k][1].eps),
                   bn_fold_cached(ch[k][3], ch[k][3].weight, ch[k][3].bias, ch[k][3].eps)) for ch in chains]
        mids = [torch.empty_like(x) for x in cur]
        outs = [torch.empty_like(x) for x in cur]
        for half, dst in ((0, mids), (1, outs)):
            items = (_C.C3ConvEval * nb)()
            for b in range(nb):
                x = cur[b] if half == 0 else mids[b]
                w = chains[b][k][2 * half]
                weight_rsc(w)
                N, H, W, Cn = x.shape
                sc, sh = folded[b][half]
                it = items[b]
                it.N, it.H, it.W, it.Ci, it.Co = N, H, W, Cn, _wshape(w)[0]
                it.x, it.wprep = x.data_ptr(), _conv3x3_prepared(w, 0).data_ptr()
                it.scale, it.shift = sc.data_ptr(), sh.data_ptr()
                it.residual = cur[b].data_ptr() if half == 1 else None
                it.relu = 1
                it.y = dst[b].data_ptr()
            check(lib().buctd_conv3x3_bf16x6_group_eval(nb, items, stream_ptr()), "conv3x3_group_eval")
        cur = outs
    return cur


class BasicBranchesFn(torch.autograd.Function):

    @staticmethod
    def forward(ctx, w_first, chains, *xs):
        nb, n = len(xs), len(chains[0])
        dev = xs[0].device
        descs = (_C.BasicBlockDesc * (nb * n))()
        acts, stats = [], []
        for b, x in enumerate(xs):
            shape = N, H, W, Cn = x.shape
            act = torch.empty((n, 3, N, H, W, Cn), dtype=torch.float32, device=dev)
            stat = torch.empty((n, 4, Cn), dtype=torch.float32, device=dev)
            acts.append(act)
            stats.append(stat)
            step = 4 * N * H * W * Cn
            accb = acc_bytes(Cn)
            abase, pbase, sbase = act.data_ptr(), AccRef(Cn, dev, 2 * n).ptr, stat.data_ptr()
            xin = x.data_ptr()
            for k, blk in enumerate(chains[b]):
                xin = _block_desc(descs[b * n + k], shape, step, xin, blk, abase + 3 * step * k, sbase + k * 4 * Cn * 4,
                                  pbase + k * 2 * accb)
        check(lib().buctd_basic_branches_fwd_train(nb, n, descs, stream_ptr()), "basic_branches_fwd_train")
        ctx.chains = chains
        ctx.save_for_backward(*xs, *acts, *stats)
        return tuple(act[n - 1, 2] for act in acts)

    @staticmethod
    def backward(ctx, *dys):
        chains = ctx.chains
        nb, n = len(chains), len(chains[0])
        saved = ctx.saved_tensors
        xs, acts, stats = saved[:nb], saved[nb:2 * nb], saved[2 * nb:]
        dev = xs[0].device
        descs = (_C.BasicBlockDesc * (nb * n))()
        grads = (_C.BasicBlockGrads * (nb * n))()
        main = torch.cuda.current_stream(dev)
        use_side = _side["on"]
        side = _side_stream(dev) if use_side else main
        needs = []
        for x in xs:
            N, H, W, Cn = x.shape
            needs.append(_memo(("wg3g", nb, N, H, W, Cn), lambda: (int(lib().buctd_conv3x3_wgrad_bf16x6_group_workspace(
                nb, N, H, W, Cn, Cn)) + 255) & ~255))
        wg_ws = workspace_on(side, sum(needs), dev)
        ws_ptr = wg_ws.data_ptr()
        tmps, keep = [], []
        for b, x in enumerate(xs):
            shape = N, H, W, Cn = x.shape
            dy = dys[b]
            dy = torch.zeros_like(x) if dy is None else _contig(dy)
            keep.append(dy)
            want_dx = ctx.needs_input_grad[2 + b]
            tmp = torch.empty((n, 5, N, H, W, Cn), dtype=torch.float32, device=dev)
            tmps.append(tmp)
            step = 4 * N * H * W * Cn
            abase, sbase, tb = acts[b].data_ptr(), stats[b].data_ptr(), tmp.data_ptr()
            accb = acc_bytes(Cn)
            bn_acc = AccRef(Cn, dev, 2 * n).ptr
            xin = x.data_ptr()
            for k, blk in enumerate(chains[b]):
                xin = _block_desc(descs[b * n + k], shape, step, xin, blk, abase + 3 * step * k, sbase + k * 4 * Cn * 4)
                up = dy.data_ptr() if k == n - 1 else tb + 5 * step * (k + 1) + 4 * step
                _block_grads(grads[b * n + k], tb + 5 * step * k, step, up, k > 0 or want_dx, blk, bn_acc + k * 2 * accb,
                             ws_ptr, needs[b])
            ws_ptr += needs[b]
        check(lib().buctd_basic_branches_bwd(nb, n, descs, grads, main.cuda_stream, side.cuda_stream if use_side else None),
              "basic_branches_bwd")
        _native_bwd_done(side if use_side else None, list(xs) + list(acts) + list(stats) + tmps + keep,
                         (chains[b][k] for k in range(n - 1, -1, -1) for b in range(nb)))
        return (None, None) + tuple(tmps[b][0, 4] if ctx.needs_input_grad[2 + b] else None for b in range(nb))


class Conv(torch.autograd.Function):

    @staticmethod
    def forward(ctx, x, w, b, stride, pad, relu):
        y = conv_fwd(x, w, b, stride, pad, relu=relu)
        ctx.meta = (w, b, stride, pad, relu, tuple(x.shape))
        ctx.save_for_backward(x, y if relu else None)
        return y

    @staticmethod
    def backward(ctx, dy):
        w, b, stride, pad, relu, x_shape = ctx.meta
        x, y = ctx.saved_tensors
        dy = _contig(dy)
        if relu:
            dy = relu_bwd(dy, y)
        dx = conv_dgrad(dy, w, x_shape, stride, pad) if ctx.needs_input_grad[0] else None
        if w.requires_grad:
            dw, acc = grad_target(w)
            conv_wgrad_async(x, dy, w, stride, pad, dw, acc)
        if b is not None and b.requires_grad:
            db, acc = grad_target(b)
            colsum(dy, dy.shape[-1], db, acc)
        grad_done(w, b)
        return dx, None, None, None, None, None


class FuseSum(torch.autograd.Function):

    @staticmethod
    def forward(ctx, shifts, relu, *terms):
        out = fuse_sum(list(terms), list(shifts), relu)
        ctx.shifts, ctx.relu = shifts, relu
        ctx.save_for_backward(out if relu else None)
        return out

    @staticmethod
    def backward(ctx, dy):
        (y,) = ctx.saved_tensors
        dy = _contig(dy)
        cache = {}
        grads = []
        for j, s in enumerate(ctx.shifts):
            if not ctx.needs_input_grad[2 + j]:
                grads.append(None)
                continue
            if s not in cache:
                cache[s] = fuse_sum_bwd(dy, y, s) if s > 0 or ctx.relu else dy
            grads.append(cache[s])
        return (None, None, *grads)


class AddN(torch.autograd.Function):

    @staticmethod
    def forward(ctx, a, b, c):
        out = add(a, b)
        if c is not None:
            out = add(out, c, out=out)
        ctx.n = 3 if c is not None else 2
        return out

    @staticmethod
    def backward(ctx, dy):
        return dy, dy, (dy if ctx.n == 3 else None)


def add_n(terms):
    acc = terms[0]
    k = 1
    while k < len(terms):
        group = [acc] + list(terms[k:k + 3])
        k += 3
        out = torch.empty_like(acc)
        arr = (C.c_void_p * len(group))(*[t.data_ptr() for t in group])
        check(lib().buctd_add_n(arr, len(group), ptr(out), acc.numel(), stream_ptr()), "add_n")
        acc = out
    return acc


class FanOut(torch.autograd.Function):

    @staticmethod
    def forward(ctx, x, n):
        return tuple(x.view_as(x) for _ in range(n))

    @staticmethod
    def backward(ctx, *grads):
        gs = [_contig(g) for g in grads if g is not None]
        if not gs:
            return None, None
        return (gs[0] if len(gs) == 1 else add_n(gs)), None


class ToNCHW(torch.autograd.Function):
    @staticmethod
    def forward(ctx, x):
        return nhwc_to_nchw(x)

    @staticmethod
    def backward(ctx, dy):
        return nchw_to_nhwc(_contig(dy))


class PositionAttention(torch.autograd.Function):

    @staticmethod
    def forward(ctx, q, k, v, h, p_drop, training):
        packed = k is None
        B, Tq = q.shape[0], q.shape[1]
        ldq = q.shape[2]
        hdk = ldq // 2 if packed else ldq
        kt, k_off, ldk = (q, hdk, ldq) if packed else (k, 0, k.shape[2])
        Tk = kt.shape[1]
        dk, dv = hdk // h, v.shape[2] // h
        scale = 1.0 / math.sqrt(dk)
        p_eff = p_drop if training else 0.0
        seed = next_seed()
        S = torch.empty((B, h, Tq, Tk), dtype=torch.float32, device=q.device)
        for i in range(h):
            matmul(q, kt, S, batch=B, M=Tq, N=Tk, K=dk, a_layout=0, b_layout=0, lda=ldq, ldb=ldk, ldc=Tk,
                   stride_a=Tq * ldq, stride_b=Tk * ldk, stride_c=h * Tq * Tk, a_off=i * dk, b_off=k_off + i * dk,
                   c_off=i * Tq * Tk)
        P, Pd = softmax_dropout_fwd(S, Tk, scale, p_eff, seed)
        O = torch.empty((B, Tq, h * dv), dtype=torch.float32, device=q.device)
        for i in range(h):
            matmul(Pd, v, O, batch=B, M=Tq, N=dv, K=Tk, a_layout=0, b_layout=1, lda=Tk, ldb=h * dv, ldc=h * dv,
                   stride_a=h * Tq * Tk, stride_b=Tk * h * dv, stride_c=Tq * h * dv, a_off=i * Tq * Tk,
                   b_off=i * dv, c_off=i * dv)
        ctx.meta = (h, dk, dv, scale, p_eff, seed, packed)
        ctx.save_for_backward(q, k, v, P, Pd if p_eff > 0 else None)
        return O

    @staticmethod
    def backward(ctx, dO):
        h, dk, dv, scale, p_eff, seed, packed = ctx.meta
        q, k, v, P, Pd = ctx.saved_tensors
        if Pd is None:
            Pd = P
        dO = _contig(dO)
        B, Tq, ldq = q.shape
        hdk = h * dk
        kt, k_off, ldk = (q, hdk, ldq) if packed else (k, 0, k.shape[2])
        Tk = kt.shape[1]
        hdv = h * dv
        dq = torch.empty_like(q)
        dkk = dq if packed else torch.empty_like(k)
        dvv = torch.empty_like(v)
        dP = torch.empty_like(P)
        for i in range(h):
            matmul(Pd, dO, dvv, batch=B, M=Tk, N=dv, K=Tq, a_layout=1, b_layout=1, lda=Tk, ldb=hdv, ldc=hdv,
                   stride_a=h * Tq * Tk, stride_b=Tq * hdv, stride_c=Tk * hdv, a_off=i * Tq * Tk, b_off=i * dv,
                   c_off=i * dv)
            matmul(dO, v, dP, batch=B, M=Tq, N=Tk, K=dv, a_layout=0, b_layout=0, lda=hdv, ldb=hdv, ldc=Tk,
                   stride_a=Tq * hdv, stride_b=Tk * hdv, stride_c=h * Tq * Tk, a_off=i * dv, b_off=i * dv,
                   c_off=i * Tq * Tk)
        dS = softmax_dropout_bwd(dP, P, Tk, scale, p_eff, seed)
        for i in range(h):
            matmul(dS, kt, dq, batch=B, M=Tq, N=dk, K=Tk, a_layout=0, b_layout=1, lda=Tk, ldb=ldk, ldc=ldq,
                   stride_a=h * Tq * Tk, stride_b=Tk * ldk, stride_c=Tq * ldq, a_off=i * Tq * Tk, b_off=k_off + i * dk,
                   c_off=i * dk)
            matmul(dS, q, dkk, batch=B, M=Tk, N=dk, K=Tq, a_layout=1, b_layout=1, lda=Tk, ldb=ldq, ldc=ldk,
                   stride_a=h * Tq * Tk, stride_b=Tq * ldq, stride_c=Tk * ldk, a_off=i * Tq * Tk, b_off=i * dk,
                   c_off=k_off + i * dk)
        return dq, (None if packed else dkk), dvv, None, None, None


def _head_width(d, h):
    d, h = int(d), int(h)
    return d // h if h >= 1 and d % h == 0 else 0


def mha_fused_ok(T, d, h=1):
    return _memo(("mhafw", int(T), int(d), int(h)),
                 lambda: lib().buctd_mha_heads_fwd_supported(int(T), int(h), _head_width(d, h)) == 1)


def _mha_rows(t, T, name):
    if t.dtype != torch.float32:
        raise _C.BuctdHipError(f"{name}: fp32 expected, got {t.dtype}")
    ld = t.stride(1)
    if t.stride(2) != 1 or t.stride(0) != T * ld or ld % 4 or t.data_ptr() % 16 or ld < t.shape[2]:
        t = t.contiguous()
        ld = t.shape[2]
    return t, ld


def _mha_desc(q, k, v, h, scale):
    B, T = q.shape[0], q.shape[1]
    hd = v.shape[2]
    q, ldq = _mha_rows(q, T, "mha q")
    v, ldv = _mha_rows(v, T, "mha v")
    if k is None:
        if q.shape[2] != 2 * hd:
            raise _C.BuctdHipError("mha: the packed form holds q | k, twice the width of v")
        k, ldk, kp = q, ldq, q.data_ptr() + 4 * hd
    else:
        k, ldk = _mha_rows(k, T, "mha k")
        kp = k.data_ptr()
    if (k is not q and (q.shape[2] != hd or k.shape[2] != hd)) or k.shape[1] != T or v.shape[1] != T or hd % h:
        raise _C.BuctdHipError("mha: q, k, v must have the same token count and width (Tq == Tk, dk == dv)")
    a = _C.MhaArgs()
    a.B, a.T, a.h, a.dh = B, T, h, hd // h
    a.q, a.k, a.v = ptr(q), kp, ptr(v)
    a.ldq, a.ldk, a.ldv = ldq, ldk, ldv
    a.scale = (1.0 / math.sqrt(hd // h)) if scale is None else float(scale)
    return a, (q, k, v), B, T, hd


def mha_fwd(qk, v, scale=None, h=1, k=None):
    B, T = qk.shape[0], qk.shape[1]
    d = v.shape[2]
    if k is not None or h != 1 or lib().buctd_mha_fwd_supported(T, d) != 1:
        a, keep, B, T, d = _mha_desc(qk, k, v, int(h), scale)
        out = torch.empty((B, T, d), dtype=torch.float32, device=qk.device)
        a.out, a.ldo = ptr(out), d
        fn = lib().buctd_mha_heads_fwd_bf16x6 if _conv_math["mode"] == "bf16x6" and _MHA_X6 else lib().buctd_mha_heads_fwd
        check(fn(C.byref(a), stream_ptr()), "mha_fwd")
        return out
    _f32(qk, "mha qk")
    _f32(v, "mha v")
    two_d = qk.shape[2]
    out = torch.empty((B, T, d), dtype=torch.float32, device=qk.device)
    kptr = C.c_void_p(qk.data_ptr() + 4 * d)
    sc = (1.0 / math.sqrt(d)) if scale is None else float(scale)
    if _conv_math["mode"] == "bf16x6" and _MHA_X6:
        if _MHA_PRESPLIT:
            nb = _memo(("mhaws", B, T, d), lambda: lib().buctd_mha_fwd_bf16x6_workspace(B, T, d))
            ws = workspace(nb, qk.device)
            check(lib().buctd_mha_fwd_bf16x6_ws(B, T, d, ptr(qk), kptr, ptr(v), two_d, v.shape[2], sc, ptr(out), None,
                                                ptr(ws), ws.numel(), stream_ptr()), "mha_fwd")
            return out
        fn = lib().buctd_mha_fwd_bf16x6
    else:
        fn = lib().buctd_mha_fwd
    check(fn(B, T, d, ptr(qk), kptr, ptr(v), two_d, v.shape[2], sc, ptr(out), None, stream_ptr()), "mha_fwd")
    return out


def mha_train_ok(T, d, h=1):
    return _memo(("mhatr", int(T), int(d), int(h)),
                 lambda: lib().buctd_mha_heads_train_supported(int(T), int(h), _head_width(d, h)) == 1)


class FusedMHA(torch.autograd.Function):

    @staticmethod
    def forward(ctx, qk, v, p_drop, training, h=1, k=None):
        a, keep, B, T, d = _mha_desc(qk, k, v, int(h), None)
        p_eff = float(p_drop) if training else 0.0
        seed = next_seed()
        out = torch.empty((B, T, d), dtype=torch.float32, device=qk.device)
        lse = torch.empty((B, int(h), T), dtype=torch.float32, device=qk.device)
        a.out, a.ldo, a.lse, a.p_drop = ptr(out), d, ptr(lse), p_eff
        fn, s = _seeded("buctd_mha_heads_fwd_train", seed)
        check(fn(C.byref(a), s, stream_ptr()), "mha_fwd_train")
        ctx.meta = (int(h), p_eff, seed, k is None)
        ctx.save_for_backward(*keep, out, lse)
        return out

    @staticmethod
    def backward(ctx, dout):
        h, p_eff, seed, packed = ctx.meta
        q, k, v, out, lse = ctx.saved_tensors
        a, _, B, T, d = _mha_desc(q, None if packed else k, v, h, None)
        dout, lddo = _mha_rows(dout, T, "mha dout")
        dq = torch.empty(q.shape, dtype=torch.float32, device=q.device)
        dk = dq if packed else torch.empty(k.shape, dtype=torch.float32, device=q.device)
        dv = torch.empty(v.shape, dtype=torch.float32, device=q.device)
        a.out, a.ldo, a.lse, a.p_drop = ptr(out), d, ptr(lse), p_eff
        a.dout, a.lddo = ptr(dout), lddo
        a.dq, a.dk, a.dv = ptr(dq), (dq.data_ptr() + 4 * d if packed else ptr(dk)), ptr(dv)
        a.lddq, a.lddk, a.lddv = dq.shape[2], dk.shape[2], dv.shape[2]
        ws = workspace(_memo(("mhabw", B, h, T), lambda: lib().buctd_mha_heads_bwd_workspace(B, h, T)), q.device)
        fn, s = _seeded("buctd_mha_heads_bwd", seed)
        check(fn(C.byref(a), s, ptr(ws), ws.numel(), stream_ptr()), "mha_bwd")
        return dq, dv, None, None, None, (None if packed else dk)


def attn_smallqk_ok(T, d_in, C, h=1):
    if h != 1 or d_in + 1 > 20:
        return False
    R4 = _smallqk_r4(d_in)
    return bool(lib().buctd_attn_smallqk_supported(T, R4, C))


def _smallqk_r4(d_in):
    r = d_in + 1
    return 4 if r <= 4 else 8 if r <= 8 else 16 if r <= 16 else 20


class SmallQKAttention(torch.autograd.Function):

    @staticmethod
    def forward(ctx, yq, wq, bq, k, v, p_drop, training):
        B, T, d = yq.shape
        Cn = k.shape[2]
        R4 = _smallqk_r4(d)
        dev = yq.device
        qp = torch.zeros((B, T, R4), dtype=torch.float32, device=dev)
        qp[:, :, :d] = yq
        qp[:, :, d] = 1.0
        w4t = torch.zeros((R4, Cn), dtype=torch.float32, device=dev)
        w4t[:d] = wq.detach().t()
        w4t[d] = bq.detach()
        k = _contig(k)
        v = _contig(v)
        kp = torch.empty((B, T, R4), dtype=torch.float32, device=dev)
        matmul(k, w4t, kp, batch=1, M=B * T, N=R4, K=Cn, a_layout=0, b_layout=0, lda=Cn, ldb=Cn, ldc=R4)
        scale = 1.0 / math.sqrt(Cn)
        p_eff = float(p_drop) if training else 0.0
        seed = next_seed()
        out = torch.empty((B, T, Cn), dtype=torch.float32, device=dev)
        m = torch.empty((B, T), dtype=torch.float32, device=dev)
        linv = torch.empty((B, T), dtype=torch.float32, device=dev)
        b3 = {"bf16x3": 1, "bf16x6": 2}.get(_conv_math["mode"], 0)
        fn, s = _seeded("buctd_attn_smallqk_fwd", seed)
        check(fn(B, T, R4, Cn, ptr(qp), ptr(kp), ptr(v), scale, p_eff, s, b3, ptr(out), ptr(m), ptr(linv), stream_ptr()),
              "attn_smallqk_fwd")
        ctx.meta = (d, R4, scale, p_eff, seed, b3)
        ctx.save_for_backward(qp, kp, k, v, out, m, linv, w4t, wq, bq)
        return out

    @staticmethod
    def backward(ctx, dout):
        d, R4, scale, p_eff, seed, b3 = ctx.meta
        qp, kp, k, v, out, m, linv, w4t, wq, bq = ctx.saved_tensors
        dout = _contig(dout)
        B, T, Cn = v.shape
        dev = v.device
        dqp = torch.empty_like(qp)
        dkp = torch.empty_like(kp)
        dv = torch.empty_like(v)
        dvec = torch.empty((B, T), dtype=torch.float32, device=dev)
        fn, s = _seeded("buctd_attn_smallqk_bwd", seed)
        check(fn(B, T, R4, Cn, ptr(qp), ptr(kp), ptr(v), ptr(out), ptr(dout), ptr(m), ptr(linv), scale, p_eff, s, b3, ptr(dqp),
                 ptr(dkp), ptr(dv), ptr(dvec), stream_ptr()), "attn_smallqk_bwd")
        dk = torch.empty_like(k)
        matmul(dkp, w4t, dk, batch=1, M=B * T, N=Cn, K=R4, a_layout=0, b_layout=1, lda=R4, ldb=Cn, ldc=Cn)
        dw4t = torch.empty_like(w4t)
        matmul(dkp, k, dw4t, batch=1, M=R4, N=Cn, K=B * T, a_layout=1, b_layout=1, lda=R4, ldb=Cn, ldc=Cn)
        dyq = dqp[:, :, :d].contiguous() if ctx.needs_input_grad[0] else None
        gw, acc = grad_target(wq)
        if acc:
            gw.add_(dw4t[:d].t())
        else:
            gw.copy_(dw4t[:d].t())
        grad_done(wq)
        gb, acc = grad_target(bq)
        if acc:
            gb.add_(dw4t[d])
        else:
            gb.copy_(dw4t[d])
        grad_done(bq)
        return dyq, None, None, dk, dv, None, None


class ChannelAttention(torch.autograd.Function):

    @staticmethod
    def forward(ctx, qn, yn, fc_w, fc_b, h, p_drop, training):
        B, T, Cn = yn.shape
        dk = T // h
        scale = 1.0 / math.sqrt(dk)
        p_eff = p_drop if training else 0.0
        seed = next_seed()
        Lg = torch.empty((B, h, Cn, Cn), dtype=torch.float32, device=yn.device)
        for i in range(h):
            matmul(qn, yn, Lg, batch=B, M=Cn, N=Cn, K=dk, a_layout=1, b_layout=1, lda=Cn, ldb=Cn, ldc=Cn,
                   stride_a=T * Cn, stride_b=T * Cn, stride_c=h * Cn * Cn, a_off=i * dk * Cn, b_off=i * dk * Cn,
                   c_off=i * Cn * Cn)
        A, Ad = softmax_dropout_fwd(Lg, Cn, scale, p_eff, seed)
        on = torch.empty((B, T, Cn), dtype=torch.float32, device=yn.device)
        for i in range(h):
            matmul(yn, Ad, on, batch=B, M=dk, N=Cn, K=Cn, a_layout=0, b_layout=0, lda=Cn, ldb=Cn, ldc=Cn,
                   stride_a=T * Cn, stride_b=h * Cn * Cn, stride_c=T * Cn, a_off=i * dk * Cn, b_off=i * Cn * Cn,
                   c_off=i * dk * Cn)
        out = torch.empty_like(on)
        if fc_o_x6_ok(T, B * Cn):
            x6_gemm(_x6_weight_image(fc_w, T, T, False),
                    x6_image(on, B * Cn, T, 1, vg=Cn, vgs=T * Cn, vs=1, ks=Cn), out, T, B * Cn, T, ldc=Cn, Nc=Cn,
                    gsc=T * Cn, bias=fc_b, bias_axis=1)
        else:
            matmul(fc_w, on, out, batch=1, M=T, N=B * Cn, K=T, a_layout=0, b_layout=1, lda=T, ldb=Cn, ldc=Cn,
                   Nc=Cn, gsbn=T * Cn, gsc=T * Cn, bias=fc_b, bias_axis=1)
        ctx.meta = (fc_w, fc_b, h, dk, scale, p_eff, seed)
        ctx.save_for_backward(qn, yn, A, Ad if p_eff > 0 else None, on)
        return out

    @staticmethod
    def backward(ctx, dout):
        fc_w, fc_b, h, dk, scale, p_eff, seed = ctx.meta
        qn, yn, A, Ad, on = ctx.saved_tensors
        if Ad is None:
            Ad = A
# ... 83 lines not shown
```

### include/buctd_hip.h

```cpp
#ifndef BUCTD_HIP_H
#define BUCTD_HIP_H
#include <stddef.h>
#include <stdint.h>

#ifdef __cplusplus
extern "C" {
#endif

int buctd_version(void);
const char* buctd_last_error(void);

typedef struct {
  int N, H, W, Ci;
  int Co, R, S;
  int stride, pad;
  int Ho, Wo;
} buctd_conv_desc;

int buctd_conv2d_fwd_thin(const buctd_conv_desc* d);
int buctd_conv2d_fwd(const buctd_conv_desc* d, const float* x, const float* w, const float* bias,
                     const float* scale, const float* shift, const float* residual, int relu, float* y,
                     float* stats_partials, void* stream);
int buctd_conv2d_dgrad(const buctd_conv_desc* d, const float* dy, const float* w, const float* bias, float* dx,
                       float* stats_partials, void* stream);
int buctd_conv2d_stats_groups(const buctd_conv_desc* d, int transposed, int* ngroups, int* rows_per_group);
size_t buctd_conv2d_wgrad_workspace(const buctd_conv_desc* d);
int buctd_conv2d_wgrad(const buctd_conv_desc* d, const float* x, const float* dy, float* dw, int accumulate,
                       void* workspace, size_t workspace_bytes, void* stream);
#define BUCTD_CONV_BIAS 1
#define BUCTD_CONV_SCALE 2
#define BUCTD_CONV_RESIDUAL 4
#define BUCTD_CONV_RELU 8
#define BUCTD_CONV_STATS 16
#define BUCTD_CONV_PLAN_INTS 11
int buctd_conv2d_plan(const buctd_conv_desc* d, int direction, int flags, int* out);

int buctd_conv3x3_bf16x6_supported(int N, int H, int W, int Ci, int Co);
int buctd_conv3x3_bf16x6_stats_groups(int N, int H, int W, int Ci, int Co, int* ngroups, int* rows_per_group);
size_t buctd_conv3x3_bf16x6_prep_bytes(int Ci, int Co, int flip);
int buctd_conv3x3_bf16x6_prep(int Ci, int Co, const float* w, int flip, void* wprep, void* stream);
int buctd_conv3x3_bf16x6(int N, int H, int W, int Ci, int Co, const float* x, const void* wprep, const float* bias,
                         const float* scale, const float* shift, const float* residual, int relu, float* y,
                         float* stats_partials, int* stats_counts, void* stream);
int buctd_conv3x3_bf16x6_bnin(int N, int H, int W, int Ci, int Co, const float* x, const void* wprep, const float* bias,
                              const float* scale, const float* shift, const float* residual, int relu, float* y,
                              float* stats_partials, int* stats_counts, const float* in_mean, const float* in_invstd,
                              const float* in_gamma, const float* in_beta, int in_relu, void* stream);
int buctd_conv3x3_bf16x6_bnstat(int N, int H, int W, int Ci, int Co, const float* x, const void* wprep, const float* residual,
                                float* y, const float* bn_z, const float* bn_y, const float* bn_mean, const float* bn_invstd,
                                const float* bn_gamma, const float* bn_beta, float* bn_part, void* stream);
struct buctd_bn_acc_in_;
int buctd_conv3x3_bf16x6_acc(int N, int H, int W, int Ci, int Co, const float* x, const void* wprep, const float* residual,
                             int relu, float* y, void* stats_acc, const struct buctd_bn_acc_in_* in_bn, const float* in_gamma,
                             const float* in_beta, int in_relu, void* stream);
int buctd_conv3x3_bf16x6_bnstat_acc(int N, int H, int W, int Ci, int Co, const float* x, const void* wprep,
                                    const float* residual, float* y, const float* bn_z, const float* bn_y,
                                    const float* bn_mean, const float* bn_invstd, const float* bn_gamma, const float* bn_beta,
                                    void* bn_acc, void* stream);
typedef struct {
  int N, H, W, Ci, Co;
  const float* x;
  const void* wprep;
  const float* residual;
  int relu;
  float* y;
  void* stats_acc;
  const struct buctd_bn_acc_in_* in_bn;
  const float *in_gamma, *in_beta;
  int in_relu;
  const float *bn_z, *bn_y, *bn_mean, *bn_invstd, *bn_gamma, *bn_beta;
  void* bn_acc;
} buctd_c3_conv;
int buctd_conv3x3_bf16x6_group(int n, const buctd_c3_conv* convs, void* stream);
typedef struct {
  int N, H, W, Ci, Co;
  const float* x;
  const void* wprep;
  const float *scale, *shift;
  const float* residual;
  int relu;
  float* y;
} buctd_c3_conv_eval;
int buctd_conv3x3_bf16x6_group_eval(int n, const buctd_c3_conv_eval* convs, void* stream);
int buctd_conv3x3_bf16x6_group_workgroups(int n, const buctd_c3_conv* convs);
int buctd_conv3x3_bf16x6_plan(int N, int H, int W, int Ci, int Co, int option_set, int* out);
int buctd_conv3x3_bf16x3_supported(int N, int H, int W, int Ci, int Co);
int buctd_conv3x3_bf16x3_stats_groups(int N, int H, int W, int Ci, int Co, int* ngroups, int* rows_per_group);
size_t buctd_conv3x3_bf16x3_prep_bytes(int Ci, int Co, int flip);
int buctd_conv3x3_bf16x3_prep(int Ci, int Co, const float* w, int flip, void* wprep, void* stream);
typedef struct {
  const float* w;
  void* wprep;
  int Ci, Co, flip, reserved;
  long piece_begin;
} buctd_c3_prep_item;
int buctd_conv3x3_bf16x3_prep_batched(const buctd_c3_prep_item* items_device, int n, long total_pieces, void* stream);
int buctd_conv3x3_bf16x3(int N, int H, int W, int Ci, int Co, const float* x, const void* wprep, const float* bias,
                         const float* scale, const float* shift, const float* residual, int relu, float* y,
                         float* stats_partials, int* stats_counts, void* stream);

int buctd_conv3x3_wgrad_bf16x6_supported(int N, int H, int W, int Ci, int Co);
int buctd_conv3x3_wgrad_bf16x6_plan(int N, int H, int W, int Ci, int Co, int* out);
size_t buctd_conv3x3_wgrad_bf16x6_workspace(int N, int H, int W, int Ci, int Co);
int buctd_conv3x3_wgrad_bf16x6(int N, int H, int W, int Ci, int Co, const float* x, const float* dy, float* dw,
                               int accumulate, void* workspace, size_t workspace_bytes, void* stream);
int buctd_conv3x3_wgrad_bf16x6_bnin(int N, int H, int W, int Ci, int Co, const float* x, const float* dy, float* dw,
                                    int accumulate, const float* x_mean, const float* x_invstd, const float* x_gamma,
                                    const float* x_beta, int x_relu, void* workspace, size_t workspace_bytes,
                                    void* stream);
typedef struct {
  int N, H, W, Ci, Co;
  const float *x, *dy;
  float* dw;
  int accumulate;
  const float *x_mean, *x_invstd, *x_gamma, *x_beta;
  int x_relu;
  void* workspace;
  size_t workspace_bytes;
} buctd_wg3_conv;
size_t buctd_conv3x3_wgrad_bf16x6_group_workspace(int n, int N, int H, int W, int Ci, int Co);
int buctd_conv3x3_wgrad_bf16x6_group(int n, const buctd_wg3_conv* convs, void* stream);
int buctd_conv3x3_wgrad_bf16x6_group_workgroups(int n, const buctd_wg3_conv* convs);
int buctd_conv3x3_wgrad_bf16x3_supported(int N, int H, int W, int Ci, int Co);
size_t buctd_conv3x3_wgrad_bf16x3_workspace(int N, int H, int W, int Ci, int Co);
int buctd_conv3x3_wgrad_bf16x3(int N, int H, int W, int Ci, int Co, const float* x, const float* dy, float* dw,
                               int accumulate, void* workspace, size_t workspace_bytes, void* stream);

typedef struct {
  int batch, M, N, K;
  int a_layout;
  int b_layout;
  int lda, ldb, ldc;
  long stride_a, stride_b, stride_c;
  int Kc; long group_stride_a, group_stride_bk;
  int Nc; long group_stride_bn, group_stride_c;
  float alpha;
  int bias_axis;
} buctd_matmul_desc;
size_t buctd_matmul_workspace(const buctd_matmul_desc* d);
int buctd_matmul(const buctd_matmul_desc* d, const float* A, const float* B, const float* bias, float* C,
                 void* workspace, size_t workspace_bytes, void* stream);

int buctd_bn_finalize(const float* partials, const int* group_counts, int ngroups, int rows_per_group, long rows,
                      int C, float eps, float momentum, float* mean, float* invstd, float* running_mean,
                      float* running_var, void* stream);
int buctd_bn_stats(const float* z, long rows, int C, float* partials, int* ngroups, int* rows_per_group,
                   void* stream);
int buctd_bn_stats_groups(long rows, int C, int* ngroups, int* rows_per_group);
int buctd_bn_apply(const float* z, const float* mean, const float* invstd, const float* gamma, const float* beta,
                   const float* residual, int relu, float* y, long rows, int C, void* stream);
size_t buctd_bn_bwd_workspace(long rows, int C);
int buctd_bn_bwd(const float* dy, const float* y, const float* z, const float* mean, const float* invstd,
                 const float* gamma, const float* beta, int relu, long rows, int C, float* dz, float* dres,
                 float* dgamma, float* dbeta, int accumulate, void* workspace, size_t workspace_bytes, void* stream);
int buctd_bn_bwd_from_partials(const float* dy, const float* y, const float* z, const float* mean, const float* invstd,
                               const float* gamma, const float* beta, int relu, long rows, int C, const float* part,
                               int nparts, float* dz, float* dres, float* dgamma, float* dbeta, int accumulate,
                               void* workspace, size_t workspace_bytes, void* stream);
size_t buctd_bn_acc_bytes(int C);
typedef struct buctd_bn_acc_in_ {
  const void* acc;
  long rows;
  float eps, momentum;
  float *mean_out, *invstd_out;
  float *running_mean, *running_var;
} buctd_bn_acc_in;
int buctd_bn_apply_acc(const float* z, const buctd_bn_acc_in* st, const float* gamma, const float* beta,
                       const float* residual, int relu, float* y, long rows, int C, void* stream);
int buctd_bn_bwd_acc(const float* dy, const float* y, const float* z, const float* mean, const float* invstd,
                     const float* gamma, const float* beta, int relu, long rows, int C, float* dz, float* dres,
                     float* dgamma, float* dbeta, int accumulate, void* acc, int acc_ready, void* stream);
typedef struct {
  const float* z;
  buctd_bn_acc_in st;
  const float *gamma, *beta, *residual;
  int relu;
  float* y;
  long rows;
  int C;
} buctd_bn_apply_item;
int buctd_bn_apply_acc_group(int n, const buctd_bn_apply_item* items, void* stream);
typedef struct {
  const float *dy, *y, *z, *mean, *invstd, *gamma, *beta;
  int relu;
  long rows;
  int C;
  float *dz, *dres, *dgamma, *dbeta;
  int accumulate;
  void* acc;
  int acc_ready;
} buctd_bn_bwd_item;
int buctd_bn_bwd_acc_group(int n, const buctd_bn_bwd_item* items, void* stream);
int buctd_bn_fold(const float* gamma, const float* beta, const float* running_mean, const float* running_var,
                  float eps, int C, float* scale, float* shift, void* stream);

int buctd_add(const float* a, const float* b, float* out, long n, int relu, void* stream);
int buctd_add_n(const float* const* terms, int n, float* out, long count, void* stream);
int buctd_mul(const float* a, const float* b, float* out, long n, void* stream);
int buctd_scale(const float* x, const float* dev_scalar, float alpha, float* out, long n, void* stream);
int buctd_copy_channels(const float* src, long rows, int Cs, int cs0, float* dst, int Cd, int cd0, int Cc,
                        void* stream);
int buctd_add_bcast(const float* a, const float* v, float* out, long batch, long n, void* stream);
int buctd_relu_bwd(const float* dy, const float* y, float* dx, long n, void* stream);
size_t buctd_colsum_workspace(long rows, int C);
int buctd_colsum(const float* x, long rows, int C, float* out, int accumulate, void* workspace,
                 size_t workspace_bytes, void* stream);
int buctd_nchw_to_nhwc(const float* x, int N, int Ctot, int c0, int Cc, int H, int W, float* y, void* stream);
int buctd_nhwc_to_nchw(const float* x, int N, int C, int H, int W, float* y, void* stream);
int buctd_fuse_sum(const float* const* terms, const int* shifts, int nterms, int N, int H, int W, int C, int relu,
                   float* out, void* stream);
int buctd_fuse_sum_bwd(const float* dy, const float* y, int shift, int N, int H, int W, int C, float* g,
                       void* stream);
int buctd_resize_bilinear(const float* x, int N, int Ctot, int c0, int Cc, int H, int W, int Ho, int Wo, float* y,
                          void* stream);
int buctd_maxpool3x3s2_fwd(const float* x, int N, int H, int W, int C, float* y, int32_t* idx, void* stream);
int buctd_maxpool3x3s2_bwd(const float* dy, const int32_t* idx, int N, int H, int W, int C, float* dx,
                           void* stream);

int buctd_softmax_dropout_fwd(const float* s, long rows, int L, float scale, float p_drop, uint64_t seed, float* p,
                              float* pd, void* stream);
int buctd_softmax_dropout_bwd(const float* dpd, const float* p, long rows, int L, float scale, float p_drop,
                              uint64_t seed, float* ds, void* stream);
int buctd_softmax_dropout_fwd_dseed(const float* s, long rows, int L, float scale, float p_drop, const uint64_t* seed,
                                    float* p, float* pd, void* stream);
int buctd_softmax_dropout_bwd_dseed(const float* dpd, const float* p, long rows, int L, float scale, float p_drop,
                                    const uint64_t* seed, float* ds, void* stream);
int buctd_attn_smallqk_supported(int T, int R4, int C);
int buctd_attn_smallqk_fwd(int B, int T, int R4, int C, const float* q, const float* k, const float* v, float scale,
                           float p_drop, uint64_t seed, int bf16x3, float* out, float* m, float* linv, void* stream);
int buctd_attn_smallqk_bwd(int B, int T, int R4, int C, const float* q, const float* k, const float* v,
                           const float* o, const float* dout, const float* m, const float* linv, float scale,
                           float p_drop, uint64_t seed, int bf16x3, float* dq, float* dk, float* dv,
                           float* dvec_workspace, void* stream);
int buctd_attn_smallqk_fwd_dseed(int B, int T, int R4, int C, const float* q, const float* k, const float* v, float scale,
                                 float p_drop, const uint64_t* seed, int bf16x3, float* out, float* m, float* linv,
                                 void* stream);
int buctd_attn_smallqk_bwd_dseed(int B, int T, int R4, int C, const float* q, const float* k, const float* v,
                                 const float* o, const float* dout, const float* m, const float* linv, float scale,
                                 float p_drop, const uint64_t* seed, int bf16x3, float* dq, float* dk, float* dv,
                                 float* dvec_workspace, void* stream);
int buctd_dropout(const float* x, float* y, long n, float p_drop, uint64_t seed, void* stream);
int buctd_dropout_dseed(const float* x, float* y, long n, float p_drop, const uint64_t* seed, void* stream);
int buctd_dropout_seed_fill(uint64_t* table, int n, uint64_t base, uint64_t counter0, void* stream);
int buctd_layernorm_fwd(const float* x, const float* gamma, const float* beta, long rows, int C, float eps, float* y,
                        float* mean, float* invstd, void* stream);
int buctd_add_layernorm_fwd(const float* a, const float* b, const float* gamma, const float* beta, long rows, int C, float eps,
                            float* sum_out, float* y, float* mean, float* invstd, void* stream);
size_t buctd_layernorm_bwd_workspace(long rows, int C);
int buctd_layernorm_bwd(const float* dy, const float* x, const float* mean, const float* invstd, const float* gamma,
                        long rows, int C, float* dx, float* dgamma, float* dbeta, int accumulate, void* workspace,
                        size_t workspace_bytes, void* stream);

int buctd_joints_mse(const float* pred, const float* gt, const float* w, int N, int K, int HW, float* loss,
                     float* grad, float gscale, void* workspace, size_t workspace_bytes, void* stream);
#define BUCTD_OHKM_MAX_JOINTS 64
size_t buctd_joints_ohkm_mse_workspace(int N, int K);
int buctd_joints_ohkm_mse(const float* pred, const float* gt, const float* w, int N, int K, int HW, int topk, float* loss,
                          float* grad, float gscale, void* workspace, size_t workspace_bytes, void* stream);
int buctd_argmax_decode(const float* hm, int rows, int H, int W, float* preds, float* maxvals, int32_t* idx,
                        void* stream);
int buctd_argmax_decode_refined(const float* hm, int rows, int H, int W, float* preds, float* maxvals, int32_t* idx,
                                float* quarter, void* stream);
#define BUCTD_DARK_MAX_PIXELS 8000
int buctd_argmax_decode_dark(const float* hm, int rows, int H, int W, float* preds, float* maxvals, int32_t* idx,
                             float* offset, void* stream);
int buctd_gaussian_target(const float* joints, const float* vis, int B, int K, int Hh, int Wh, float stride_x,
                          float stride_y, float sigma, float* target, float* weight, void* stream);
size_t buctd_cond_render_workspace(int B, int Cc, int H, int W);
int buctd_cond_render(const float* joints, int js, const float* colors, int B, int K, int Cc, int H, int W,
                      int truncate, float* cond, void* workspace, size_t workspace_bytes, void* stream);
int buctd_flipback_avg(const float* a, const float* b, const int32_t* perm, int N, int K, int H, int W, int shift,
                       float* out, void* stream);

int buctd_gconv_x6_supported(int kind, int N, int H, int W, int Ci, int Co, int dir);
size_t buctd_gconv_x6_prep_bytes(int kind, int Ci, int Co, int dir);
int buctd_gconv_x6_prep(int kind, int Ci, int Co, const float* w, int dir, void* wprep, void* stream);
size_t buctd_gconv_x6_prep_item_bytes(void);
int buctd_gconv_x6_prep_item(int kind, int Ci, int Co, const float* w, int dir, void* wprep, void* item_host);
int buctd_gconv_x6_prep_batched(const void* items_device, int n, void* stream);
int buctd_gconv_x6_stats_groups(int kind, int N, int H, int W, int Ci, int Co, int* ngroups, int* rows_per_group);
int buctd_gconv_x6_fwd(int kind, int N, int H, int W, int Ci, int Co, const float* x, const void* wprep, const float* bias,
                       const float* scale, const float* shift, const float* residual, int relu, float* y,
                       float* stats_partials, int* stats_counts, void* stream);
int buctd_gconv_x6_fwd_acc(int kind, int N, int H, int W, int Ci, int Co, const float* x, const void* wprep, const float* bias,
                           float* y, void* stats_acc, void* stream);
int buctd_gconv_x6_dgrad(int kind, int N, int H, int W, int Ci, int Co, const float* dy, const void* wprep,
                         const float* residual, float* dx, void* stream);
int buctd_gconv_wgrad_x6_supported(int kind, int N, int H, int W, int Ci, int Co);
size_t buctd_gconv_wgrad_x6_workspace(int kind, int N, int H, int W, int Ci, int Co);
int buctd_gconv_wgrad_x6(int kind, int N, int H, int W, int Ci, int Co, const float* x, const float* dy, float* dw,
                         int accumulate, void* workspace, size_t workspace_bytes, void* stream);

typedef struct {
  int N, H, W, C;
  const float* x;
  const void *w1_fwd, *w2_fwd;
  const void *w1_bwd, *w2_bwd;
  const float *gamma1, *beta1, *gamma2, *beta2;
  float *running_mean1, *running_var1, *running_mean2, *running_var2;
  float eps1, momentum1, eps2, momentum2;
  float *z1, *z2, *y;
  void* acc;
  float* stat;
} buctd_basic_block;
typedef struct {
  const float* dy;
  float *dz2, *dres, *dy1, *dz1;
  float* dx;
  float *dw1, *dw2, *dgamma1, *dbeta1, *dgamma2, *dbeta2;
  int acc_w1, acc_w2, acc_bn1, acc_bn2;
  void* bn_acc;
  void* wg_ws; size_t wg_ws_bytes;
} buctd_basic_block_grads;
int buctd_basic_chain_fwd_train(int n, const buctd_basic_block* blocks, void* stream);
int buctd_basic_chain_bwd(int n, const buctd_basic_block* blocks, const buctd_basic_block_grads* grads, void* stream,
                          void* side_stream);

int buctd_basic_branches_fwd_train(int nb, int n, const buctd_basic_block* blocks, void* stream);
int buctd_basic_branches_bwd(int nb, int n, const buctd_basic_block* blocks, const buctd_basic_block_grads* grads, void* stream,
                             void* side_stream);

int buctd_stream_fork(void* from, void* to);

int buctd_x6_image_dims(int V, int K, int role, int* Vpad, int* Kpad);
size_t buctd_x6_image_bytes(int V, int K, int role);
int buctd_x6_image(const float* src, int V, int K, int vg, long vgs, long vs, int kg, long kgs, long ks, int role,
                   void* image, void* stream);
int buctd_x6_gemm(int M, int N, int K, const void* a_image, const void* b_image, const float* bias, int bias_axis,
                  float alpha, float* C, long ldc, int Nc, long gsc, void* stream);

int buctd_adam_step(float* p, const float* g, float* m, float* v, long n, float lr, float beta1, float beta2,
                    float eps, int step, float gscale, void* stream);
int buctd_sgd_step(float* p, const float* g, float* momentum_buf, long n, float lr, float momentum, float weight_decay,
                   int nesterov, int first_step, float gscale, void* stream);

int buctd_mha_fwd_supported(int T, int d);
int buctd_mha_fwd(int B, int T, int d, const float* q, const float* k, const float* v, int ldqk, int ldv, float scale,
                  float* out, float* lse, void* stream);
int buctd_mha_fwd_bf16x6(int B, int T, int d, const float* q, const float* k, const float* v, int ldqk, int ldv,
                         float scale, float* out, float* lse, void* stream);
size_t buctd_mha_fwd_bf16x6_workspace(int B, int T, int d);
int buctd_mha_fwd_bf16x6_ws(int B, int T, int d, const float* q, const float* k, const float* v, int ldqk, int ldv,
                            float scale, float* out, float* lse, void* workspace, size_t workspace_bytes, void* stream);
int buctd_mha_train_supported(int T, int d);
int buctd_mha_fwd_train(int B, int T, int d, const float* q, const float* k, const float* v, int ldqk, int ldv, float scale,
                        float p_drop, uint64_t seed, float* out, float* lse, void* stream);
size_t buctd_mha_bwd_workspace(int B, int T);
int buctd_mha_bwd(int B, int T, int d, const float* q, const float* k, const float* v, int ldqk, int ldv, const float* out,
                  const float* dout, const float* lse, float scale, float p_drop, uint64_t seed, float* dq, float* dk,
                  int lddqk, float* dv, int lddv, void* workspace, size_t workspace_bytes, void* stream);
int buctd_mha_fwd_train_dseed(int B, int T, int d, const float* q, const float* k, const float* v, int ldqk, int ldv,
                              float scale, float p_drop, const uint64_t* seed, float* out, float* lse, void* stream);
int buctd_mha_bwd_dseed(int B, int T, int d, const float* q, const float* k, const float* v, int ldqk, int ldv,
                        const float* out, const float* dout, const float* lse, float scale, float p_drop,
                        const uint64_t* seed, float* dq, float* dk, int lddqk, float* dv, int lddv, void* workspace,
                        size_t workspace_bytes, void* stream);

typedef struct buctd_mha_args {
  int B, T, h, dh;
  const float* q; const float* k; const float* v;
  int ldq, ldk, ldv;
  float* out; int ldo;
  float* lse;
  float scale, p_drop;
  const float* dout; int lddo;
  float* dq; float* dk; float* dv;
  int lddq, lddk, lddv;
} buctd_mha_args;
int buctd_mha_heads_fwd_supported(int T, int h, int dh);
int buctd_mha_heads_fwd(const buctd_mha_args* a, void* stream);
int buctd_mha_heads_fwd_bf16x6(const buctd_mha_args* a, void* stream);
int buctd_mha_heads_train_supported(int T, int h, int dh);
int buctd_mha_heads_fwd_train(const buctd_mha_args* a, uint64_t seed, void* stream);
size_t buctd_mha_heads_bwd_workspace(int B, int h, int T);
int buctd_mha_heads_bwd(const buctd_mha_args* a, uint64_t seed, void* workspace, size_t workspace_bytes, void* stream);
int buctd_mha_heads_fwd_train_dseed(const buctd_mha_args* a, const uint64_t* seed, void* stream);
int buctd_mha_heads_bwd_dseed(const buctd_mha_args* a, const uint64_t* seed, void* workspace, size_t workspace_bytes,
                              void* stream);

typedef struct {
  const unsigned char* src;
  int H, W;
  int flip;
  int rx, ry, rw, rh;
  double m[6];
} buctd_warp_item;
int buctd_warp_affine_norm(const buctd_warp_item* items_device, int B, int dst_h, int dst_w, const float* mean3,
                           const float* std3, float* out, long out_batch_stride, unsigned char* crop_u8, void* stream);
int buctd_cond_render_into(const float* joints, int js, const float* colors, int B, int K, int Cc, int H, int W,
                           int truncate, float* cond, long cond_batch_stride, void* workspace, size_t workspace_bytes,
                           void* stream);
int buctd_cond_geometry(const double* synth, const double* cond_vis, const buctd_warp_item* items_device,
                        const int* pair_device, int B, int K, double* out_joints, double* out_vis, float* out_trunc,
                        void* stream);

typedef struct {
  double sigmas[32];
  int pair[32];
  int jitter_cls[32], miss_cls[32], inv_cls[32], swap_cls[32];
  double jitter_p[2][3];
  double miss_p[3][3];
  double inv_p[3];
  double swap_p[2][3];
  double out_vis;
} buctd_synth_tables;
int buctd_synthesize_pose(const buctd_synth_tables* tables, const double* joints, const double* estimated,
                          const double* near_joints, const double* area, const int* num_overlap, int B, int K, int M,
                          unsigned long long seed, double* out, void* stream);

size_t buctd_nms_workspace(int boxes_num);
int buctd_nms(int* keep_out, int* num_out, const float* boxes, int boxes_num, int boxes_dim, float thresh,
              void* workspace, size_t workspace_bytes, void* stream);
int buctd_cpu_nms(const float* dets, int n, const int* order, float thresh, int* keep_out, int* num_out);

int buctd_bf16_pack_conv(const float* w, long s_co, long s_ci, long s_r, long s_s, int Co, int Ci, int R,
                         const float* conv_bias, const float* gamma, const float* beta, const float* running_mean,
                         const float* running_var, float eps, uint16_t* wimg, float* bias_out, void* stream);
int buctd_bf16_conv(const uint16_t* x, int N, int H, int W, int Ci, const uint16_t* wimg, const float* bias, int Co,
                    int R, int stride, int pad, const uint16_t* residual, int relu, int out_f32_nchw, void* y,
                    void* workspace, size_t workspace_bytes, void* stream);
int buctd_bf16_fuse_sum(const uint16_t* const* terms, const int* shifts, int nterms, int N, int H, int W, int C,
                        int relu, uint16_t* out, void* stream);
int buctd_bf16_from_f32(const float* x, long n, uint16_t* y, void* stream);

#ifdef __cplusplus
}
#endif
#endif
```

Measured before the change: 513.8 images/s.

## Fuse BN backward reductions into fan-in add and fuse-sum backward kernels

Gradient producers in backward (the add_n of fanned-out gradients and the HRNet fuse-layer sum backward) now also accumulate the BN-backward reduction sums (sum of dy and sum of dy*xhat) for the downstream BN layers that fed those tensors. Forward outputs carry a sink descriptor, and the consuming BN or block-chain backward receives a pre-filled accumulator, so it skips its own reduction pass over dy and z. This removes a separate full read of the gradient and activation per BN. The cost is more plumbing through autograd (tensor attributes, ready flags) and extra z reads inside the fused kernels, which could use more registers.

```diff
diff --git a/buctd_amd/_C.py b/buctd_amd/_C.py
--- a/buctd_amd/_C.py
+++ b/buctd_amd/_C.py
@@ -23,7 +23,7 @@
     _fields_ = ([(n, C.c_void_p) for n in ("dy", "dz2", "dres", "dy1", "dz1", "dx", "dw1", "dw2", "dgamma1", "dbeta1",
                                            "dgamma2", "dbeta2")] +
                 [(n, C.c_int) for n in ("acc_w1", "acc_w2", "acc_bn1", "acc_bn2")] +
-                [("bn_acc", C.c_void_p), ("wg_ws", C.c_void_p), ("wg_ws_bytes", C.c_size_t)])
+                [("bn_acc", C.c_void_p), ("wg_ws", C.c_void_p), ("wg_ws_bytes", C.c_size_t), ("bn2_ready", C.c_int)])
 
 
 class BnAccIn(C.Structure):
@@ -55,6 +55,15 @@
                 [("relu", C.c_int), ("rows", C.c_long), ("C", C.c_int)] +
                 [(n, C.c_void_p) for n in ("dz", "dres", "dgamma", "dbeta")] +
                 [("accumulate", C.c_int), ("acc", C.c_void_p), ("acc_ready", C.c_int)])
+
+
+class BnSink(C.Structure):
+    _fields_ = [(n, C.c_void_p) for n in ("z", "mean", "invstd", "acc")]
+
+
+class AddNBnSumsItem(C.Structure):
+    _fields_ = [("terms", C.c_void_p * 4), ("n", C.c_int), ("out", C.c_void_p), ("y", C.c_void_p), ("sink", BnSink),
+                ("rows", C.c_long), ("C", C.c_int)]
 
 
 class Wg3Conv(C.Structure):
@@ -150,6 +159,9 @@
     "buctd_gconv_wgrad_x6": (_I, [_I] * 6 + [_P, _P, _P, _I, _P, _SZ, _P]),
     "buctd_bn_apply_acc_group": (_I, [_I, C.POINTER(BnApplyItem), _P]),
     "buctd_bn_bwd_acc_group": (_I, [_I, C.POINTER(BnBwdItem), _P]),
+    "buctd_add_n_bn_sums": (_I, [C.POINTER(AddNBnSumsItem), _P]),
+    "buctd_add_n_bn_sums_group": (_I, [_I, C.POINTER(AddNBnSumsItem), _P]),
+    "buctd_fuse_sum_bwd_bn_sums": (_I, [_P, _P, _I, _I, _I, _I, _I, _P, _I, C.POINTER(BnSink), _P]),
     "buctd_conv3x3_wgrad_bf16x6_group_workspace": (_SZ, [_I] * 6),
     "buctd_conv3x3_wgrad_bf16x6_group": (_I, [_I, C.POINTER(Wg3Conv), _P]),
     "buctd_conv3x3_wgrad_bf16x6_group_workgroups": (_I, [_I, C.POINTER(Wg3Conv)]),
diff --git a/buctd_amd/csrc/block.hip b/buctd_amd/csrc/block.hip
--- a/buctd_amd/csrc/block.hip
+++ b/buctd_amd/csrc/block.hip
@@ -117,7 +117,7 @@
   BUCTD_CHECK_ARG(n > 0 && blocks && grads, "buctd_basic_chain_bwd: bad argument");
   for (int k = 0; k < n; ++k)
     BUCTD_CHECK_ARG(bwd_ptrs_ok(blocks[k], grads[k]), "buctd_basic_chain_bwd: null pointer in block %d", k);
-  bool ready = false;
+  bool ready = grads[n - 1].bn2_ready != 0;
   for (int k = n - 1; k >= 0; --k) {
     const bool chain = k > 0 && bn2_sums_chain(blocks + k, grads + k);
     BLK_TRY(block_bwd_impl(blocks + k, grads + k, chain ? blocks + k - 1 : nullptr, chain ? grads + k - 1 : nullptr, ready, stream,
@@ -171,6 +171,7 @@
     BUCTD_CHECK_ARG(bwd_ptrs_ok(blocks[i], grads[i]), "buctd_basic_branches_bwd: null pointer in block %d", i);
   hipStream_t main_s = (hipStream_t)stream, side_s = side_stream ? (hipStream_t)side_stream : main_s;
   bool ready[BR_MAX] = {false, false, false, false};
+  for (int b = 0; b < nb; ++b) ready[b] = grads[b * n + n - 1].bn2_ready != 0;
   for (int k = n - 1; k >= 0; --k) {
     buctd_bn_bwd_item bi[BR_MAX];
     buctd_wg3_conv wg[BR_MAX];
diff --git a/buctd_amd/csrc/bn.hip b/buctd_amd/csrc/bn.hip
--- a/buctd_amd/csrc/bn.hip
+++ b/buctd_amd/csrc/bn.hip
@@ -801,78 +801,160 @@
   float* dbeta;
   int accumulate;
 };
-__device__ __forceinline__ void bn_bwd_reduce_acc_body(const BnBwdArgs& p, unsigned bid, f32x4 (&sm)[2][256]) {
-  const float* __restrict__ dy = p.dy;
-  const float* __restrict__ y = p.y;
-  const float* __restrict__ z = p.z;
-  const float* __restrict__ mean = p.mean;
-  const float* __restrict__ invstd = p.invstd;
-  const float* __restrict__ gamma = p.gamma;
-  const float* __restrict__ beta = p.beta;
-  long long* __restrict__ acc = p.acc;
-  const int relu = p.relu, C = p.C;
-  const long rows = p.rows, rows_per_block = p.rows_per_block;
+struct BnSrcDy {
+  static constexpr int UNROLL = 4;
+  const float* dy;
+  __device__ __forceinline__ f32x4 get(long, int, long o) const { return reinterpret_cast<const f32x4*>(dy)[o]; }
+  __device__ __forceinline__ void put(long, f32x4) const {}
+};
+struct BnSrcAddN {
+  static constexpr int UNROLL = 4;
+  const float* a[4];
+  int n;
+  float* out;
+  __device__ __forceinline__ f32x4 get(long, int, long o) const {
+    f32x4 s = reinterpret_cast<const f32x4*>(a[0])[o] + reinterpret_cast<const f32x4*>(a[1])[o];
+    if (n > 2) s += reinterpret_cast<const f32x4*>(a[2])[o];
+    if (n > 3) s += reinterpret_cast<const f32x4*>(a[3])[o];
+    return s;
+  }
+  __device__ __forceinline__ void put(long o, f32x4 g) const { reinterpret_cast<f32x4*>(out)[o] = g; }
+};
+template <int SHIFT>
+struct BnSrcFuse {
+  static constexpr int UNROLL = SHIFT == 0 ? 4 : 1;
+  const float* dy;
+  const float* y;
+  float* g;
+  int H, W, C4;
+  __device__ __forceinline__ f32x4 get(long r, int c4, long) const {
+    constexpr int f = 1 << SHIFT;
+    const int hs = H >> SHIFT, ws = W >> SHIFT;
+    const int w = (int)(r % ws);
+    const long t = r / ws;
+    const int h = (int)(t % hs);
+    const long n = t / hs;
+    f32x4 acc = (f32x4){0.f, 0.f, 0.f, 0.f};
+#pragma unroll
+    for (int dh = 0; dh < f; ++dh)
+#pragma unroll
+      for (int dw = 0; dw < f; ++dw) {
+        const long o = ((n * H + h * f + dh) * W + w * f + dw) * C4 + c4;
+        f32x4 d = reinterpret_cast<const f32x4*>(dy)[o];
+        if (y) {
+          const f32x4 yy = reinterpret_cast<const f32x4*>(y)[o];
+#pragma unroll
+          for (int j = 0; j < 4; ++j)
+            if (!(yy[j] > 0.f)) d[j] = 0.f;
+        }
+        acc += d;
+      }
+    return acc;
+  }
+  __device__ __forceinline__ void put(long o, f32x4 v) const { reinterpret_cast<f32x4*>(g)[o] = v; }
+};
+
+struct BnSink {
+  const float* z;
+  const float* mean;
+  const float* invstd;
+  long long* acc;
+};
+#define BN_SINKS_MAX 3
+
+template <class Src, int NS>
+__device__ __forceinline__ void bn_sums_body(const Src& src, const float* __restrict__ y, const float* __restrict__ gamma,
+                                             const float* __restrict__ beta, int relu, const BnSink* sk, long rows, int C,
+                                             long rows_per_block, unsigned bid, f32x4 (*sm)[256]) {
+  constexpr int U = Src::UNROLL;
   const int c4n = C >> 2;
   const int rl = 256 / c4n;
   const int tc = threadIdx.x % c4n, tr = threadIdx.x / c4n;
   const long r0 = (long)bid * rows_per_block;
   long r1 = r0 + rows_per_block;
   if (r1 > rows) r1 = rows;
-  f32x4 s1 = (f32x4){0.f, 0.f, 0.f, 0.f}, s2 = s1;
+  const f32x4 zero = (f32x4){0.f, 0.f, 0.f, 0.f};
+  f32x4 s1 = zero, s2[NS];
+#pragma unroll
+  for (int k = 0; k < NS; ++k) s2[k] = zero;
   if (tr < rl) {
-    const f32x4 mu = reinterpret_cast<const f32x4*>(mean)[tc];
-    const f32x4 is = reinterpret_cast<const f32x4*>(invstd)[tc];
-    f32x4 sc = is, be = is;
+    f32x4 mu[NS], is[NS];
+#pragma unroll
+    for (int k = 0; k < NS; ++k) {
+      mu[k] = reinterpret_cast<const f32x4*>(sk[k].mean)[tc];
+      is[k] = reinterpret_cast<const f32x4*>(sk[k].invstd)[tc];
+    }
+    f32x4 sc = is[0], be = is[0];
     const bool rebuild = relu && !y;
     if (rebuild) {
-      sc = is * reinterpret_cast<const f32x4*>(gamma)[tc];
+      sc = is[0] * reinterpret_cast<const f32x4*>(gamma)[tc];
       be = reinterpret_cast<const f32x4*>(beta)[tc];
     }
-    auto body = [&](f32x4 g, f32x4 zz, f32x4 yy) {
+    auto body = [&](f32x4 g, const f32x4* zz, f32x4 yy) {
       if (relu) {
-        if (rebuild) yy = (zz - mu) * sc + be;
+        if (rebuild) yy = (zz[0] - mu[0]) * sc + be;
 #pragma unroll
         for (int j = 0; j < 4; ++j)
           if (!(yy[j] > 0.f)) g[j] = 0.f;
       }
       s1 += g;
-      s2 += g * (zz - mu) * is;
+#pragma unroll
+      for (int k = 0; k < NS; ++k) s2[k] += g * (zz[k] - mu[k]) * is[k];
     };
     long r = r0 + tr;
     const long step = rl;
-    for (; r + 3 * step < r1; r += 4 * step) {
-      f32x4 g[4], zz[4], yy[4];
-#pragma unroll
-      for (int u = 0; u < 4; ++u) {
+    for (; r + (U - 1) * step < r1; r += U * step) {
+      f32x4 g[U], zz[U][NS], yy[U];
+#pragma unroll
+      for (int u = 0; u < U; ++u) {
         const long o = (r + u * step) * c4n + tc;
-        g[u] = reinterpret_cast<const f32x4*>(dy)[o];
-        zz[u] = reinterpret_cast<const f32x4*>(z)[o];
-        yy[u] = (relu && y) ? reinterpret_cast<const f32x4*>(y)[o] : zz[u];
-      }
-#pragma unroll
-      for (int u = 0; u < 4; ++u) body(g[u], zz[u], yy[u]);
+        g[u] = src.get(r + u * step, tc, o);
+#pragma unroll
+        for (int k = 0; k < NS; ++k) zz[u][k] = reinterpret_cast<const f32x4*>(sk[k].z)[o];
+        yy[u] = (relu && y) ? reinterpret_cast<const f32x4*>(y)[o] : zz[u][0];
+      }
+#pragma unroll
+      for (int u = 0; u < U; ++u) {
+        src.put((r + u * step) * c4n + tc, g[u]);
+        body(g[u], zz[u], yy[u]);
+      }
     }
     for (; r < r1; r += step) {
       const long o = r * c4n + tc;
-      const f32x4 zz = reinterpret_cast<const f32x4*>(z)[o];
-      body(reinterpret_cast<const f32x4*>(dy)[o], zz, (relu && y) ? reinterpret_cast<const f32x4*>(y)[o] : zz);
+      f32x4 zz[NS];
+#pragma unroll
+      for (int k = 0; k < NS; ++k) zz[k] = reinterpret_cast<const f32x4*>(sk[k].z)[o];
+      const f32x4 g = src.get(r, tc, o);
+      const f32x4 yy = (relu && y) ? reinterpret_cast<const f32x4*>(y)[o] : zz[0];
+      src.put(o, g);
+      body(g, zz, yy);
     }
   }
   sm[0][threadIdx.x] = s1;
-  sm[1][threadIdx.x] = s2;
+#pragma unroll
+  for (int k = 0; k < NS; ++k) sm[1 + k][threadIdx.x] = s2[k];
   __syncthreads();
   if (tr == 0) {
     for (int k = 1; k < rl; ++k) {
       s1 += sm[0][k * c4n + tc];
-      s2 += sm[1][k * c4n + tc];
+#pragma unroll
+      for (int q = 0; q < NS; ++q) s2[q] += sm[1 + q][k * c4n + tc];
     }
     sm[0][tc] = s1;
-    sm[1][tc] = s2;
+#pragma unroll
+    for (int q = 0; q < NS; ++q) sm[1 + q][tc] = s2[q];
   }
   __syncthreads();
   const unsigned shard = bnacc_shard();
-  for (int c = threadIdx.x; c < C; c += 256)
-    bnacc_add(acc, C, shard, c, (double)reinterpret_cast<const float*>(&sm[0][0])[c], (double)reinterpret_cast<const float*>(&sm[1][0])[c]);
+  for (int c = threadIdx.x; c < C; c += 256) {
+    const double v1 = (double)reinterpret_cast<const float*>(&sm[0][0])[c];
+#pragma unroll
+    for (int q = 0; q < NS; ++q) bnacc_add(sk[q].acc, C, shard, c, v1, (double)reinterpret_cast<const float*>(&sm[1 + q][0])[c]);
+  }
+}
+__device__ __forceinline__ void bn_bwd_reduce_acc_body(const BnBwdArgs& p, unsigned bid, f32x4 (&sm)[2][256]) {
+  const BnSink sk{p.z, p.mean, p.invstd, p.acc};
+  bn_sums_body<BnSrcDy, 1>(BnSrcDy{p.dy}, p.y, p.gamma, p.beta, p.relu, &sk, p.rows, p.C, p.rows_per_block, bid, sm);
 }
 __global__ __launch_bounds__(256) void bn_bwd_reduce_acc_kernel(BnBwdArgs p) {
   __shared__ f32x4 sm[2][256];
@@ -1053,3 +1135,125 @@
   BUCTD_CHECK_LAUNCH("buctd_bn_bwd_acc_group(apply)");
   return BUCTD_OK;
 }
+
+struct BnAddSumsArgs {
+  BnSrcAddN src;
+  const float* y;
+  BnSink sk;
+  long rows;
+  int C;
+  long rows_per_block;
+};
+__global__ __launch_bounds__(256) void add_n_bn_sums_kernel(BnAddSumsArgs p) {
+  __shared__ f32x4 sm[2][256];
+  bn_sums_body<BnSrcAddN, 1>(p.src, p.y, nullptr, nullptr, p.y != nullptr, &p.sk, p.rows, p.C, p.rows_per_block, blockIdx.x, sm);
+}
+__global__ __launch_bounds__(256) void add_n_bn_sums_group_kernel(BnGroup<BnAddSumsArgs> g_) {
+  __shared__ f32x4 sm[2][256];
+  const BnGroup<BnAddSumsArgs>& g = *(const BnGroup<BnAddSumsArgs>*)__builtin_amdgcn_kernarg_segment_ptr();
+  unsigned bid, nblk;
+  const int k = bn_group_find(g, &bid, &nblk);
+  const BnAddSumsArgs& p = g.s[k];
+  bn_sums_body<BnSrcAddN, 1>(p.src, p.y, nullptr, nullptr, p.y != nullptr, &p.sk, p.rows, p.C, p.rows_per_block, bid, sm);
+}
+
+template <int SHIFT, int NS>
+struct BnFuseSumsArgs {
+  BnSrcFuse<SHIFT> src;
+  BnSink sk[NS];
+  long rows;
+  int C;
+  long rows_per_block;
+};
+template <int SHIFT, int NS>
+__global__ __launch_bounds__(256) void fuse_sum_bwd_bn_sums_kernel(BnFuseSumsArgs<SHIFT, NS> p) {
+  __shared__ f32x4 sm[1 + NS][256];
+  bn_sums_body<BnSrcFuse<SHIFT>, NS>(p.src, nullptr, nullptr, nullptr, 0, p.sk, p.rows, p.C, p.rows_per_block, blockIdx.x, sm);
+}
+
+static int add_sums_fill(const buctd_add_n_bn_sums_item& it, const char* who, BnAddSumsArgs& a, long* nb) {
+  BUCTD_CHECK_ARG(it.n >= 2 && it.n <= 4 && it.out && it.rows > 0 && it.C > 0 && it.C % 4 == 0 && it.C / 4 <= 256,
+                  "%s: 2..4 terms, C a multiple of 4, <= 1024", who);
+  BUCTD_CHECK_ARG(it.sink.z && it.sink.mean && it.sink.invstd && it.sink.acc, "%s: incomplete sink", who);
+  for (int k = 0; k < 4; ++k) {
+    a.src.a[k] = k < it.n ? it.terms[k] : nullptr;
+    BUCTD_CHECK_ARG(k >= it.n || it.terms[k], "%s: null term", who);
+  }
+  a.src.n = it.n;
+  a.src.out = it.out;
+  a.y = it.y;
+  a.sk = BnSink{it.sink.z, it.sink.mean, it.sink.invstd, (long long*)it.sink.acc};
+  a.rows = it.rows;
+  a.C = it.C;
+  *nb = bwd2_blocks(it.rows, &a.rows_per_block);
+  return BUCTD_OK;
+}
+
+extern "C" int buctd_add_n_bn_sums(const buctd_add_n_bn_sums_item* item, void* stream) {
+  BUCTD_CHECK_ARG(item, "buctd_add_n_bn_sums: bad argument");
+  BnAddSumsArgs a;
+  long nb;
+  const int rc = add_sums_fill(*item, "buctd_add_n_bn_sums", a, &nb);
+  if (rc) return rc;
+  hipLaunchKernelGGL(add_n_bn_sums_kernel, dim3((unsigned)nb), dim3(256), 0, (hipStream_t)stream, a);
+  BUCTD_CHECK_LAUNCH("buctd_add_n_bn_sums");
+  return BUCTD_OK;
+}
+
+extern "C" int buctd_add_n_bn_sums_group(int n, const buctd_add_n_bn_sums_item* items, void* stream) {
+  BUCTD_CHECK_ARG(n > 0 && n <= BNG_MAX && items, "buctd_add_n_bn_sums_group: 1..%d tensors", BNG_MAX);
+  BnGroup<BnAddSumsArgs> g;
+  g.n = n;
+  g.first[0] = 0;
+  for (int k = 0; k < n; ++k) {
+    long nb;
+    const int rc = add_sums_fill(items[k], "buctd_add_n_bn_sums_group", g.s[k], &nb);
+    if (rc) return rc;
+    g.first[k + 1] = g.first[k] + (unsigned)nb;
+  }
+  for (int k = n; k < BNG_MAX; ++k) {
+    g.s[k] = g.s[0];
+    g.first[k + 1] = g.first[n];
+  }
+  hipLaunchKernelGGL(add_n_bn_sums_group_kernel, dim3(g.first[n]), dim3(256), 0, (hipStream_t)stream, g);
+  BUCTD_CHECK_LAUNCH("buctd_add_n_bn_sums_group");
+  return BUCTD_OK;
+}
+
+template <int SHIFT, int NS>
+static void fuse_sums_launch(const float* dy, const float* y, int H, int W, int C, float* g, const buctd_bn_sink* sinks, long rows,
+                             hipStream_t st) {
+  BnFuseSumsArgs<SHIFT, NS> a;
+  a.src = BnSrcFuse<SHIFT>{dy, y, g, H, W, C / 4};
+  for (int k = 0; k < NS; ++k) a.sk[k] = BnSink{sinks[k].z, sinks[k].mean, sinks[k].invstd, (long long*)sinks[k].acc};
+  a.rows = rows;
+  a.C = C;
+  const long nb = bwd2_blocks(rows, &a.rows_per_block);
+  hipLaunchKernelGGL((fuse_sum_bwd_bn_sums_kernel<SHIFT, NS>), dim3((unsigned)nb), dim3(256), 0, st, a);
+}
+template <int SHIFT>
+static void fuse_sums_launch_ns(int ns, const float* dy, const float* y, int H, int W, int C, float* g, const buctd_bn_sink* sinks,
+                                long rows, hipStream_t st) {
+  if (ns == 1) fuse_sums_launch<SHIFT, 1>(dy, y, H, W, C, g, sinks, rows, st);
+  else if (ns == 2) fuse_sums_launch<SHIFT, 2>(dy, y, H, W, C, g, sinks, rows, st);
+  else fuse_sums_launch<SHIFT, 3>(dy, y, H, W, C, g, sinks, rows, st);
+}
+
+extern "C" int buctd_fuse_sum_bwd_bn_sums(const float* dy, const float* y, int shift, int N, int H, int W, int C, float* g,
+                                          int nsinks, const buctd_bn_sink* sinks, void* stream) {
+  BUCTD_CHECK_ARG(dy && g && shift >= 0 && shift <= 3 && N > 0 && H > 0 && W > 0 && C > 0 && C % 4 == 0 && C / 4 <= 256,
+                  "buctd_fuse_sum_bwd_bn_sums: bad argument (shift <= 3, C a multiple of 4, <= 1024)");
+  BUCTD_CHECK_ARG((H >> shift) << shift == H && (W >> shift) << shift == W,
+                  "buctd_fuse_sum_bwd_bn_sums: H/W not divisible by 2^shift");
+  BUCTD_CHECK_ARG(nsinks >= 1 && nsinks <= BN_SINKS_MAX && sinks, "buctd_fuse_sum_bwd_bn_sums: 1..%d sinks", BN_SINKS_MAX);
+  for (int k = 0; k < nsinks; ++k)
+    BUCTD_CHECK_ARG(sinks[k].z && sinks[k].mean && sinks[k].invstd && sinks[k].acc, "buctd_fuse_sum_bwd_bn_sums: incomplete sink %d", k);
+  const long rows = (long)N * (H >> shift) * (W >> shift);
+  hipStream_t st = (hipStream_t)stream;
+  if (shift == 0) fuse_sums_launch_ns<0>(nsinks, dy, y, H, W, C, g, sinks, rows, st);
+  else if (shift == 1) fuse_sums_launch_ns<1>(nsinks, dy, y, H, W, C, g, sinks, rows, st);
+  else if (shift == 2) fuse_sums_launch_ns<2>(nsinks, dy, y, H, W, C, g, sinks, rows, st);
+  else fuse_sums_launch_ns<3>(nsinks, dy, y, H, W, C, g, sinks, rows, st);
+  BUCTD_CHECK_LAUNCH("buctd_fuse_sum_bwd_bn_sums");
+  return BUCTD_OK;
+}
diff --git a/buctd_amd/models/hrnet_common.py b/buctd_amd/models/hrnet_common.py
--- a/buctd_amd/models/hrnet_common.py
+++ b/buctd_amd/models/hrnet_common.py
@@ -157,7 +157,7 @@
     def get_num_inchannels(self):
         return self.num_inchannels
 
-    def _branches_grouped(self, x):
+    def _branches_grouped(self, x, fan=0):
         nb = self.num_branches
         if not (self.training and torch.is_grad_enabled() and all(type(br) is BlockChain and len(br) > 1 for br in self.branches)):
             return None
@@ -170,10 +170,16 @@
         if not ops.group_branches_ok(xs, chains):
             return None
         parts = ops.group_branch_partition(nb)
+
+        def run(p):
+            ys = ops.BasicBranchesFn.apply(chains[p[0]][0][0], [chains[i] for i in p], *[xs[i] for i in p])
+            if fan > 1:
+                al = ops.FanOutGroup.apply(fan, *ys)
+                return [al[k * fan:(k + 1) * fan] for k in range(len(ys))]
+            return list(ys)
         if len(parts) == 1:
-            return list(ops.BasicBranchesFn.apply(chains[0][0][0], chains, *xs))
-        outs = ops.fork_join([lambda p=p: ops.BasicBranchesFn.apply(chains[p[0]][0][0], [chains[i] for i in p], *[xs[i] for i in p])
-                              for p in parts], [[xs[i] for i in p] for p in parts])
+            return run(parts[0])
+        outs = ops.fork_join([lambda p=p: run(p) for p in parts], [[xs[i] for i in p] for p in parts])
         ys = [None] * nb
         for p, o in zip(parts, outs):
             for i, y in zip(p, o):
@@ -198,16 +204,21 @@
     def forward(self, x):
         if self.num_branches == 1:
             return [self.branches[0](x[0])]
-        xs = self._branches_grouped(x)
-        if xs is None:
+        rows = list(enumerate(self.fuse_layers))
+        fan = len(rows) if len(rows) > 1 and torch.is_grad_enabled() else 0
+        xr = self._branches_grouped(x, fan)
+        if xr is not None and not fan:
+            xr = [[y] * len(rows) for y in xr]
+        if xr is None:
             xs = self._branches_grouped_eval(x)
-        if xs is None:
-            xs = ops.fork_join([lambda i=i: self.branches[i](x[i]) for i in range(self.num_branches)],
+            if xs is not None:
+                xr = [[y] * len(rows) for y in xs]
+        if xr is None:
+            def branch(i):
+                y = self.branches[i](x[i])
+                return ops.FanOut.apply(y, fan) if fan and y.is_cuda and y.requires_grad else [y] * len(rows)
+            xr = ops.fork_join([lambda i=i: branch(i) for i in range(self.num_branches)],
                                [x[i] for i in range(self.num_branches)])
-        rows = list(enumerate(self.fuse_layers))
-        fan = len(rows) > 1 and torch.is_grad_enabled() and any(t.requires_grad for t in xs)
-        xr = [ops.FanOut.apply(xs[j], len(rows)) if fan and xs[j].is_cuda else [xs[j]] * len(rows)
-              for j in range(self.num_branches)]
 
         def fuse_row(i, row):
             terms, shifts = [], []
@@ -223,7 +234,8 @@
                     shifts.append(0)
             return ops.FuseSum.apply(tuple(shifts), True, *terms)
 
-        return ops.fork_join([lambda i=i, row=row: fuse_row(i, row) for i, row in rows], [xs for _ in rows], tag=1)
+        return ops.fork_join([lambda i=i, row=row: fuse_row(i, row) for i, row in rows],
+                             [[xr[j][i] for j in range(self.num_branches)] for i, _ in rows], tag=1)
 
 
 def make_transition_layer(pre, cur):
diff --git a/buctd_amd/ops.py b/buctd_amd/ops.py
--- a/buctd_amd/ops.py
+++ b/buctd_amd/ops.py
@@ -1047,7 +1047,7 @@
     return y
 
 
-def bn_bwd(dy, y, z, mean, invstd, gamma, relu, want_dres, dgamma, dbeta, accumulate, beta=None):
+def bn_bwd(dy, y, z, mean, invstd, gamma, relu, want_dres, dgamma, dbeta, accumulate, beta=None, acc=None):
     Cn = z.shape[-1]
     rows = z.numel() // Cn
     dz = torch.empty_like(z)
@@ -1055,10 +1055,12 @@
     if relu and y is None and beta is None:
         raise _C.BuctdHipError("bn_bwd: ReLU backward needs the forward output or beta")
     if bn_acc_ok(Cn):
-        acc = AccRef(Cn, z.device)
+        ready = acc is not None
+        if not ready:
+            acc = AccRef(Cn, z.device)
         check(lib().buctd_bn_bwd_acc(ptr(dy), ptr(y) if relu else None, ptr(z), ptr(mean), ptr(invstd), ptr(gamma),
                                      ptr(beta) if (relu and y is None) else None, int(bool(relu)), rows, Cn, ptr(dz), ptr(dres),
-                                     ptr(dgamma), ptr(dbeta), int(accumulate), C.c_void_p(acc.ptr), 0,
+                                     ptr(dgamma), ptr(dbeta), int(accumulate), C.c_void_p(acc.ptr), int(ready),
                                      stream_ptr()), "bn_bwd_acc")
         return dz, dres
     need = lib().buctd_bn_bwd_workspace(rows, Cn)
@@ -1067,6 +1069,82 @@
                              ptr(beta) if (relu and y is None) else None, int(bool(relu)), rows, Cn, ptr(dz), ptr(dres), ptr(dgamma), ptr(dbeta), int(accumulate),
                              ptr(ws), ws.numel(), stream_ptr()), "bn_bwd")
     return dz, dres
+
+
+_BN_SUMS = {"on": True}
+
+
+def set_bn_sums_producers(on):
+    old = _BN_SUMS["on"]
+    _BN_SUMS["on"] = bool(on)
+    return old
+
+
+class BnSumsSink:
+    __slots__ = ("z", "y", "mean", "invstd", "n_acc", "acc_index", "filled_for")
+
+    def __init__(self, z, y, mean, invstd, n_acc=1, acc_index=0):
+        self.z, self.y, self.mean, self.invstd, self.n_acc, self.acc_index = z, y, mean, invstd, n_acc, acc_index
+        self.filled_for = None
+
+
+def _sink_usable(sink, src, shape):
+    return (_BN_SUMS["on"] and sink is not None and src.is_cuda and src.dtype == torch.float32 and sink.z.shape == shape
+            and sink.z.is_contiguous() and bn_acc_ok(shape[-1]))
+
+
+def _sink_struct(st, sink, g):
+    Cn = g.shape[-1]
+    acc = AccRef(Cn, g.device, sink.n_acc)
+    st.z, st.mean, st.invstd = sink.z.data_ptr(), sink.mean.data_ptr(), sink.invstd.data_ptr()
+    st.acc = acc.ptr + sink.acc_index * acc_bytes(Cn)
+    return (g, g._version, _C.current_stream_handle(), acc)
+
+
+def bn_sums_take(sink, dy):
+    if sink is None:
+        return None
+    rec, sink.filled_for = sink.filled_for, None
+    if rec is None:
+        return None
+    g, version, stream, acc = rec
+    if (dy.data_ptr() == g.data_ptr() and dy.shape == g.shape and dy.stride() == g.stride() and dy.dtype == g.dtype
+            and dy._version == version and _C.current_stream_handle() == stream):
+        return acc
+    return None
+
+
+def add_n_bn_sums(groups):
+    items = (_C.AddNBnSumsItem * len(groups))()
+    outs, recs = [], []
+    for it, (terms, sink) in zip(items, groups):
+        out = torch.empty_like(terms[0])
+        Cn = out.shape[-1]
+        for k, t in enumerate(terms):
+            it.terms[k] = t.data_ptr()
+        it.n, it.out, it.y = len(terms), out.data_ptr(), ptr(sink.y)
+        it.rows, it.C = out.numel() // Cn, Cn
+        recs.append(_sink_struct(it.sink, sink, out))
+        outs.append(out)
+    if len(groups) == 1:
+        check(lib().buctd_add_n_bn_sums(items, stream_ptr()), "add_n_bn_sums")
+    else:
+        check(lib().buctd_add_n_bn_sums_group(len(groups), items, stream_ptr()), "add_n_bn_sums_group")
+    for (_, sink), rec in zip(groups, recs):
+        sink.filled_for = rec
+    return outs
+
+
+def fuse_sum_bwd_bn_sums(dy, y, shift, sinks):
+    N, H, W, Cn = dy.shape
+    g = torch.empty((N, H >> shift, W >> shift, Cn), dtype=torch.float32, device=dy.device)
+    arr = (_C.BnSink * len(sinks))()
+    recs = [_sink_struct(st, sink, g) for st, sink in zip(arr, sinks)]
+    check(lib().buctd_fuse_sum_bwd_bn_sums(ptr(dy), ptr(y), shift, N, H, W, Cn, ptr(g), len(sinks), arr, stream_ptr()),
+          "fuse_sum_bwd_bn_sums")
+    for sink, rec in zip(sinks, recs):
+        sink.filled_for = rec
+    return g
 
 
 def bn_fold_cached(bn, gamma, beta, eps):
@@ -1407,6 +1485,8 @@
             if track:
                 _count_batch(bn)
             ctx.has_res = residual is not None
+            if not relu and residual is None and bn_acc_ok(Cn):
+                y._bn_sink = ctx.sink = BnSumsSink(z, None, mean, invstd)
             ctx.save_for_backward(x, z, mean, invstd, y if (relu and ctx.has_res) else None)
             return y
         scale, shift = bn_fold_cached(bn, gamma, beta, eps)
@@ -1431,7 +1511,8 @@
         dgamma, acc_g = grad_target(bn.weight)
         dbeta, acc_b = grad_target(bn.bias)
         assert acc_g == acc_b
-        dz, dres = bn_bwd(dy, y, z, mean, invstd, bn.weight, relu, ctx.has_res and relu, dgamma, dbeta, acc_g, beta=bn.bias)
+        dz, dres = bn_bwd(dy, y, z, mean, invstd, bn.weight, relu, ctx.has_res and relu, dgamma, dbeta, acc_g, beta=bn.bias,
+                          acc=bn_sums_take(getattr(ctx, "sink", None), dy))
         if ctx.has_res and not relu:
             dres = dy
         dx = None
@@ -1686,6 +1767,10 @@
         grad_done(bn1.weight, bn1.bias, w1)
 
 
+def _last_bn2_sink(act, stat, n):
+    return BnSumsSink(act[n - 1, 1], act[n - 1, 2], stat[n - 1, 2], stat[n - 1, 3], n_acc=2 * n, acc_index=2 * n - 1)
+
+
 def _chain_forward(ctx, x, blocks):
     n = len(blocks)
     shape = N, H, W, Cn = x.shape
@@ -1702,7 +1787,9 @@
     check(lib().buctd_basic_chain_fwd_train(n, descs, stream_ptr()), "basic_chain_fwd_train")
     ctx.blocks = blocks
     ctx.save_for_backward(x, act, stat)
-    return act[n - 1, 2]
+    out = act[n - 1, 2]
+    out._bn_sink = ctx.sink = _last_bn2_sink(act, stat, n)
+    return out
 
 
 def _chain_backward(ctx, dy, want_dx):
@@ -1721,7 +1808,8 @@
     use_side = _side["on"]
     side = _side_stream(dev) if use_side else main
     accb = acc_bytes(Cn)
-    bn_acc = AccRef(Cn, dev, 2 * n).ptr
+    filled = bn_sums_take(getattr(ctx, "sink", None), dy)
+    bn_acc = (filled if filled is not None else AccRef(Cn, dev, 2 * n)).ptr
     wg_ws = workspace_on(side, _wgrad3x3_workspace("bf16x6", N, H, W, Cn, Cn), dev)
     ws, ws_bytes = wg_ws.data_ptr(), wg_ws.numel()
     xin = x.data_ptr()
@@ -1729,6 +1817,7 @@
         xin = _block_desc(descs[k], shape, step, xin, blk, abase + 3 * step * k, sbase + k * 4 * Cn * 4)
         up = dy.data_ptr() if k == n - 1 else tb + 5 * step * (k + 1) + 4 * step
         _block_grads(grads[k], tb + 5 * step * k, step, up, k > 0 or want_dx, blk, bn_acc + k * 2 * accb, ws, ws_bytes)
+    grads[n - 1].bn2_ready = int(filled is not None)
     check(lib().buctd_basic_chain_bwd(n, descs, grads, main.cuda_stream, side.cuda_stream if use_side else None),
           "basic_chain_bwd")
     _native_bwd_done(side if use_side else None, (x, act, stat, tmp, dy), reversed(blocks))
@@ -1857,7 +1946,11 @@
         check(lib().buctd_basic_branches_fwd_train(nb, n, descs, stream_ptr()), "basic_branches_fwd_train")
         ctx.chains = chains
         ctx.save_for_backward(*xs, *acts, *stats)
-        return tuple(act[n - 1, 2] for act in acts)
+        outs = tuple(act[n - 1, 2] for act in acts)
+        ctx.sinks = [_last_bn2_sink(act, stat, n) for act, stat in zip(acts, stats)]
+        for out, sink in zip(outs, ctx.sinks):
+            out._bn_sink = sink
+        return outs
 
     @staticmethod
     def backward(ctx, *dys):
@@ -1890,13 +1983,15 @@
             step = 4 * N * H * W * Cn
             abase, sbase, tb = acts[b].data_ptr(), stats[b].data_ptr(), tmp.data_ptr()
             accb = acc_bytes(Cn)
-            bn_acc = AccRef(Cn, dev, 2 * n).ptr
+            filled = bn_sums_take(ctx.sinks[b], dy) if dys[b] is not None else None
+            bn_acc = (filled if filled is not None else AccRef(Cn, dev, 2 * n)).ptr
             xin = x.data_ptr()
             for k, blk in enumerate(chains[b]):
                 xin = _block_desc(descs[b * n + k], shape, step, xin, blk, abase + 3 * step * k, sbase + k * 4 * Cn * 4)
                 up = dy.data_ptr() if k == n - 1 else tb + 5 * step * (k + 1) + 4 * step
                 _block_grads(grads[b * n + k], tb + 5 * step * k, step, up, k > 0 or want_dx, blk, bn_acc + k * 2 * accb,
                              ws_ptr, needs[b])
+            grads[b * n + n - 1].bn2_ready = int(filled is not None)
             ws_ptr += needs[b]
         check(lib().buctd_basic_branches_bwd(nb, n, descs, grads, main.cuda_stream, side.cuda_stream if use_side else None),
               "basic_branches_bwd")
@@ -1938,6 +2033,7 @@
     def forward(ctx, shifts, relu, *terms):
         out = fuse_sum(list(terms), list(shifts), relu)
         ctx.shifts, ctx.relu = shifts, relu
+        ctx.sinks = tuple(s if s is not None and s.y is None else None for s in (getattr(t, "_bn_sink", None) for t in terms))
         ctx.save_for_backward(out if relu else None)
         return out
 
@@ -1952,7 +2048,17 @@
                 grads.append(None)
                 continue
             if s not in cache:
-                cache[s] = fuse_sum_bwd(dy, y, s) if s > 0 or ctx.relu else dy
+                if s > 0 or ctx.relu:
+                    N, H, W, Cn = dy.shape
+                    shape = (N, H >> s, W >> s, Cn)
+                    sinks = []
+                    for k, sk in enumerate(ctx.sinks):
+                        if (ctx.shifts[k] == s and s <= 3 and ctx.needs_input_grad[2 + k] and _sink_usable(sk, dy, shape)
+                                and len(sinks) < 3 and not any(sk is q for q in sinks)):
+                            sinks.append(sk)
+                    cache[s] = fuse_sum_bwd_bn_sums(dy, y, s, sinks) if sinks else fuse_sum_bwd(dy, y, s)
+                else:
+                    cache[s] = dy
             grads.append(cache[s])
         return (None, None, *grads)
 
@@ -1989,14 +2095,46 @@
 
     @staticmethod
     def forward(ctx, x, n):
+        ctx.sink = getattr(x, "_bn_sink", None)
         return tuple(x.view_as(x) for _ in range(n))
 
     @staticmethod
     def backward(ctx, *grads):
+        return _fan_in([(grads, ctx.sink)])[0], None
+
+
+def _fan_in(branches):
+    outs = [None] * len(branches)
+    fused = []
+    for b, (grads, sink) in enumerate(branches):
         gs = [_contig(g) for g in grads if g is not None]
         if not gs:
-            return None, None
-        return (gs[0] if len(gs) == 1 else add_n(gs)), None
+            continue
+        if len(gs) == 1:
+            outs[b] = gs[0]
+        elif len(gs) <= 4 and all(_sink_usable(sink, g, g.shape) for g in gs):
+            fused.append((b, gs, sink))
+        else:
+            outs[b] = add_n(gs)
+    for k in range(0, len(fused), 4):
+        part = fused[k:k + 4]
+        for (b, _, _), out in zip(part, add_n_bn_sums([(gs, sink) for _, gs, sink in part])):
+            outs[b] = out
+    return outs
+
+
+class FanOutGroup(torch.autograd.Function):
+
+    @staticmethod
+    def forward(ctx, n, *xs):
+        ctx.n = n
+        ctx.sinks = [getattr(x, "_bn_sink", None) for x in xs]
+        return tuple(x.view_as(x) for x in xs for _ in range(n))
+
+    @staticmethod
+    def backward(ctx, *grads):
+        n = ctx.n
+        return (None, *_fan_in([(grads[b * n:(b + 1) * n], sink) for b, sink in enumerate(ctx.sinks)]))
 
 
 class ToNCHW(torch.autograd.Function):
diff --git a/include/buctd_hip.h b/include/buctd_hip.h
--- a/include/buctd_hip.h
+++ b/include/buctd_hip.h
@@ -191,6 +191,23 @@
   int acc_ready;
 } buctd_bn_bwd_item;
 int buctd_bn_bwd_acc_group(int n, const buctd_bn_bwd_item* items, void* stream);
+typedef struct {
+  const float *z, *mean, *invstd;
+  void* acc;
+} buctd_bn_sink;
+typedef struct {
+  const float* terms[4];
+  int n;
+  float* out;
+  const float* y;
+  buctd_bn_sink sink;
+  long rows;
+  int C;
+} buctd_add_n_bn_sums_item;
+int buctd_add_n_bn_sums(const buctd_add_n_bn_sums_item* item, void* stream);
+int buctd_add_n_bn_sums_group(int n, const buctd_add_n_bn_sums_item* items, void* stream);
+int buctd_fuse_sum_bwd_bn_sums(const float* dy, const float* y, int shift, int N, int H, int W, int C, float* g, int nsinks,
+                               const buctd_bn_sink* sinks, void* stream);
 int buctd_bn_fold(const float* gamma, const float* beta, const float* running_mean, const float* running_var,
                   float eps, int C, float* scale, float* shift, void* stream);
 
@@ -311,6 +328,7 @@
   int acc_w1, acc_w2, acc_bn1, acc_bn2;
   void* bn_acc;
   void* wg_ws; size_t wg_ws_bytes;
+  int bn2_ready;
 } buctd_basic_block_grads;
 int buctd_basic_chain_fwd_train(int n, const buctd_basic_block* blocks, void* stream);
 int buctd_basic_chain_bwd(int n, const buctd_basic_block* blocks, const buctd_basic_block_grads* grads, void* stream,
```

Result: no change. 512.1 images/s (-0.3%).
